# twke18/SPML

Measured on AMD Instinct MI355X. Metric: images/sec (513x513) + k-means iters/sec, higher is better.
Workload: dtype f32

## Files before the change

include/spml_hip.h:

```cpp
#ifndef SPML_HIP_H_
#define SPML_HIP_H_

#include <stddef.h>
#include <stdint.h>

#ifdef __cplusplus
extern "C" {
#endif

typedef enum spml_status {
  SPML_OK = 0,
  SPML_ERR_INVALID_ARG = -1,
  SPML_ERR_UNSUPPORTED = -2,
  SPML_ERR_WORKSPACE = -3,
  SPML_ERR_LAUNCH = -4
} spml_status;

const char* spml_status_string(int status);

#define SPML_ABI_VERSION 8
int spml_abi_version(void);

int spml_set_deterministic(int on);
int spml_get_deterministic(void);

int spml_build_experiment(void);

int spml_normalize_concat_loc_f32(const float* emb, int N, int C, int H, int W,
                                  const float* loc, const int64_t* row_map,
                                  float* out_emb, float* out_loc, void* stream);

int spml_normalize_concat_loc_bwd_f32(const float* emb, int N, int C, int H,
                                      int W, const float* loc,
                                      const int64_t* row_map,
                                      const float* d_out_emb,
                                      const float* d_out_loc, float* d_emb,
                                      void* stream);

int spml_normalize_concat_local_f32(const float* emb, int N, int C, int H, int W,
                                    const float* local, int L,
                                    const int64_t* row_map, float* out_emb,
                                    float* out_loc, void* stream);

int spml_normalize_concat_local_bwd_f32(const float* emb, int N, int C, int H,
                                        int W, const float* local, int L,
                                        const int64_t* row_map,
                                        const float* d_out_emb,
                                        const float* d_out_loc, float* d_emb,
                                        void* stream);

int spml_normalize_concat_local_nhwc_supported(int C, int L);
int spml_normalize_concat_local_nhwc_f32(const float* emb, int N, int C, int H, int W,
                                         const float* local, int L,
                                         const int64_t* row_map, float* out_emb,
                                         float* out_loc, void* stream);
int spml_normalize_concat_local_nhwc_bwd_f32(const float* emb, int N, int C, int H,
                                             int W, const float* local, int L,
                                             const int64_t* row_map,
                                             const float* d_out_emb,
                                             const float* d_out_loc, float* d_emb,
                                             void* stream);

int spml_normalize_rows_f32(const float* x, int64_t rows, int D, float* y,
                            void* stream);
int spml_normalize_rows_bwd_f32(const float* x, const float* dy, int64_t rows,
                                int D, float* dx, void* stream);

size_t spml_relabel_unique_workspace_bytes(int64_t P);
int spml_relabel_unique_i64(const int64_t* keys, int64_t P, int64_t* inv, int64_t* uniq,
                            int64_t uniq_capacity, int64_t* count, void* workspace,
                            size_t workspace_bytes, void* stream);

int spml_kmeans_init_grid_i64(int H, int W, int Ky, int Kx, int64_t* out,
                              void* stream);

#define SPML_KMEANS_DEFAULT 0
#define SPML_KMEANS_FORCE_GENERIC 1
#define SPML_KMEANS_FORCE_V2 4
#define SPML_KMEANS_SEPARATE_PRECONVERT 16
#define SPML_KMEANS_NO_PRECONVERT 8
#define SPML_KMEANS_NO_SCREEN 64
#define SPML_KMEANS_WS_PRECONVERTED 32
#define SPML_KMEANS_PASS_ONLY 256

#define SPML_KMEANS_NO_PASS64 512

#define SPML_KMEANS_TWO_KERNEL_FINALIZE 1024

#define SPML_KMEANS_NO_V4K 2048

size_t spml_kmeans_workspace_bytes(int64_t P, int D, int K, int n_img,
                                   int64_t max_seg_len);

int spml_clock_probe(uint64_t* out, int spin_us, void* stream);

int spml_maxpool3x3s2_nhwc_f32(const float* x, int n, int H, int W, int C, float* y, void* stream);

int spml_kmeans_run_f32(const float* x, int64_t P, int D,
                        const int64_t* seg_offsets, int n_img,
                        int64_t max_seg_len, int K, const int64_t* labels_init,
                        int iterations, int64_t* labels_out,
                        float* centroids_out, int flags, void* ws,
                        size_t ws_bytes, void* stream);

int spml_kmeans_assign_f32(const float* x, int64_t P, int D,
                           const int64_t* seg_offsets, int n_img,
                           int64_t max_seg_len, int K, const float* centroids,
                           int64_t* labels_out, int flags, void* ws,
                           size_t ws_bytes, void* stream);

int spml_kmeans_fused_pass_f32(const float* x, int64_t P, int D,
                               const int64_t* seg_offsets, int n_img,
                               int64_t max_seg_len, int K,
                               const float* centroids_in, int64_t* labels_out,
                               float* centroid_sums_out, int flags, void* ws,
                               size_t ws_bytes, void* stream);

int spml_kmeans_preconvert_f32(const float* x, int64_t P, int D,
                               const int64_t* seg_offsets, int n_img,
                               int64_t max_seg_len, int K, void* ws,
                               size_t ws_bytes, void* stream);

const char* spml_kmeans_path_name(int64_t P, int D, int K, int n_img,
                                  int64_t max_seg_len, int iterations,
                                  int given_centroids, int flags);

int spml_kmeans_profile_layout(int64_t P, int D, int K, int n_img,
                               int64_t max_seg_len, int iterations,
                               int* n_passes, int* workgroups_per_pass);

int spml_kmeans_run_profiled_f32(const float* x, int64_t P, int D,
                                 const int64_t* seg_offsets, int n_img,
                                 int64_t max_seg_len, int K,
                                 const int64_t* labels_init, int iterations,
                                 int64_t* labels_out, int flags, void* ws,
                                 size_t ws_bytes, uint64_t* pass_clocks,
                                 size_t pass_clocks_len, void* stream);

int spml_segment_sum_normalize_f32(const float* x, const int64_t* ids,
                                   int64_t P, int D, int64_t M, float* sums,
                                   float* protos, void* stream);

size_t spml_segment_sum_det_workspace_bytes(int64_t M, int D);
int spml_segment_sum_normalize_det_f32(const float* x, const int64_t* ids,
                                       int64_t P, int D, int64_t M,
                                       float* sums, float* protos, void* ws,
                                       size_t ws_bytes, void* stream);

int spml_segment_sum_normalize_bwd_f32(const float* d_protos,
                                       const float* sums, const int64_t* ids,
                                       int64_t P, int D, int64_t M,
                                       float* d_sums_scratch, float* dx,
                                       int accumulate, void* stream);

#define SPML_NLL_LABEL 0
#define SPML_NLL_TAGSET 1
#define SPML_NLL_PLAIN 2
#define SPML_NLL_CODE32 4

size_t spml_segsort_nll_workspace_bytes(int64_t P, int64_t M, int D);

int spml_segsort_nll_fwd_f32(const float* emb, const int64_t* own,
                             const int64_t* px_code, int64_t P,
                             const float* protos, const int64_t* pr_code,
                             int64_t M, int D, float kappa, int mode,
                             float* nll, float* stats, void* ws,
                             size_t ws_bytes, void* stream);

int spml_segsort_nll_bwd_f32(const float* emb, const int64_t* own,
                             const int64_t* px_code, int64_t P,
                             const float* protos, const int64_t* pr_code,
                             int64_t M, int D, float kappa, int mode,
                             const float* stats, const float* d_nll,
                             float* d_emb, float* d_protos, int64_t m_grad,
                             void* ws, size_t ws_bytes, void* stream);

size_t spml_topk_workspace_bytes(int64_t Q, int64_t M, int D, int k);

int spml_topk_affinity_f32(const float* q, int64_t Q, const float* protos,
                           int64_t M, int D, int k, const int64_t* q_group,
                           const int64_t* pr_group, const uint8_t* pr_valid,
                           float masked_value, int64_t* idx, float* val,
                           void* ws, size_t ws_bytes, void* stream);

int spml_window_accumulate_f32(const float* patch, int C, int h, int w,
                               float* acc, float* counts, int H, int W, int sh,
                               int sw, void* stream);

size_t spml_affinity_workspace_bytes(int B, int C, int64_t n);

int spml_affinity_transition_f32(const float* emb, int B, int C, int64_t n,
                                 float scale, int power, float* trans, void* ws,
                                 size_t ws_bytes, void* stream);

size_t spml_bn_workspace_bytes(int64_t R, int C);

int spml_bn_act_fwd_f32(const float* x, const float* residual, int64_t R, int C,
                        const float* gamma, const float* beta,
                        float* running_mean, float* running_var, float momentum,
                        float eps, int relu, float* y, float* mean, float* invstd,
                        void* ws, size_t ws_bytes, void* stream);

int spml_bn_act_bwd_f32(const float* dy, const float* y, const float* x, int64_t R,
                        int C, const float* mean, const float* invstd,
                        const float* gamma, float* d_gamma, float* d_beta,
                        float* dx, float* d_residual, void* ws, size_t ws_bytes,
                        void* stream);

int spml_bn_stats_f32(const float* x, int64_t R, int C, float* mean, float* m2,
                      void* ws, size_t ws_bytes, void* stream);

int spml_bn_act_apply_f32(const float* x, const float* residual, int64_t R, int C,
                          const float* mean, const float* invstd,
                          const float* gamma, const float* beta, int relu,
                          float* y, void* stream);

int spml_bn_act_bwd_reduce_f32(const float* dy, const float* y, const float* x,
                               int64_t R, int C, const float* mean,
                               const float* invstd, float* sum_dz,
                               float* sum_dz_xhat, void* ws, size_t ws_bytes,
                               void* stream);

int spml_bn_act_bwd_apply_f32(const float* dy, const float* y, const float* x,
                              int64_t R, int C, const float* mean,
                              const float* invstd, const float* gamma,
                              const float* sum_dz, const float* sum_dz_xhat,
                              double count, const float* count_dev, float* dx,
                              float* d_residual, void* stream);


int spml_hl8_from_f32(const float* x, int64_t rows, int C, float* bound,
                      int compute_bound, void* out, void* stream);

int spml_hl8_weight_transposed_f32(const float* w, int Cout, int taps, int Cin,
                                   const float* bound, void* out, void* stream);

int spml_conv_hl8_supported(int K, int N, int taps);

int spml_conv_hl8_f32(const void* a, const float* a_bound, const void* b,
                      const float* b_bound, const float* addend,
                      const unsigned char* addend_mask, float* out,
                      int n_img, int H, int W, int K, int N, int taps, int dilation,
                      void* stream);

int spml_conv_hl8_stats_layout(int n_img, int H, int W, int K, int N, int taps,
                               int* chunks, int* chunk_rows);
int spml_conv_hl8_stats_f32(const void* a, const float* a_bound, const void* b,
                            const float* b_bound, float* out, float* chunk_stats,
                            float* zero_me, int n_img, int H, int W, int K, int N,
                            int taps, int dilation, void* stream);

int spml_conv_wgrad_hl8_supported(int K, int N, int taps);
size_t spml_conv_wgrad_workspace_bytes(int n_img, int H, int W, int K, int N, int taps);
int spml_conv_wgrad_hl8_f32(const void* dy, const float* dy_bound, const void* x,
                            const float* x_bound, float* dw, int n_img, int H, int W,
                            int K, int N, int taps, int dilation, void* ws,
                            size_t ws_bytes, void* stream);

int spml_conv_wgrad_pyramid_hl8_supported(int K, int N, int branches);
int spml_conv_tap_gather_f32(const float* z, const float* bias, float* out, int n_img, int H,
                             int W, int N, int branches, const int* dilations, void* stream);
size_t spml_conv_wgrad_pyramid_workspace_bytes(int n_img, int H, int W, int K, int N,
                                               int branches);
int spml_conv_wgrad_pyramid_hl8_f32(const void* dy, const float* dy_bound, const void* x,
                                    const float* x_bound, float* dw, int n_img, int H, int W,
                                    int K, int N, int branches, const int* dilations,
                                    void* ws, size_t ws_bytes, void* stream);

int spml_bn_stats_ext_f32(const float* x, int64_t R, int C, float* mean, float* m2,
                          float* cmax, float* cmin, void* ws, size_t ws_bytes,
                          void* stream);

int spml_bn_stats_ext_chunks_f32(const float* chunk_stats, int chunks, int chunk_rows,
                                 int64_t R, int C, float* mean, float* m2, float* cmax,
                                 float* cmin, void* stream);

int spml_bn_finalize_f32(const float* mean, const float* m2, int C, double count,
                         float eps, float momentum, float* running_mean,
                         float* running_var, float* invstd, void* stream);

int spml_bn_act_apply_hl8_f32(const float* x, const float* residual,
                              const float* residual_bound, int64_t R, int C,
                              const float* mean, const float* invstd,
                              const float* gamma, const float* beta,
                              const float* cmax, const float* cmin, int relu,
                              float* y, void* y_hl8, float* y_bound,
                              unsigned char* relu_mask, void* stream);

int spml_bn_act_bwd_reduce_ext_f32(const float* dy, const float* y,
                                   const unsigned char* relu_mask,
                                   const float* x, int64_t R, int C, const float* mean,
                                   const float* invstd, float* sum_dz,
                                   float* sum_dz_xhat, float* max_dz, void* ws,
                                   size_t ws_bytes, void* stream);

int spml_bn_act_bwd_apply_hl8_f32(const float* dy, const float* y,
                                  const unsigned char* relu_mask,
                                  const float* x, int64_t R, int C, const float* mean,
                                  const float* invstd, const float* gamma,
                                  const float* sum_dz, const float* sum_dz_xhat,
                                  const float* max_dz, const float* cmax,
                                  const float* cmin, double count,
                                  const float* count_dev, float* dx, void* dx_hl8,
                                  float* dx_bound, float* d_residual, void* stream);

int spml_bn_fwd_hl8_f32(const float* x, const float* residual, const float* residual_bound,
                        int64_t R, int C, const float* gamma, const float* beta,
                        float* running_mean, float* running_var, float momentum, float eps,
                        int relu, float* y, void* y_hl8, float* y_bound,
                        unsigned char* relu_mask, float* mean, float* invstd, float* cmax,
                        float* cmin, void* ws, size_t ws_bytes, void* stream);

int spml_bn_fwd_hl8_chunks_f32(const float* x, const float* chunk_stats, int chunks,
                               int chunk_rows, const float* residual,
                               const float* residual_bound, int64_t R, int C,
                               const float* gamma, const float* beta, float* running_mean,
                               float* running_var, float momentum, float eps, int relu,
                               float* y, void* y_hl8, float* y_bound,
                               unsigned char* relu_mask, float* mean, float* invstd,
                               float* cmax, float* cmin, void* stream);

int spml_bn_bwd_hl8_f32(const float* dy, const float* y, const unsigned char* relu_mask,
                        const float* x, int64_t R, int C, const float* mean,
                        const float* invstd, const float* gamma, const float* cmax,
                        const float* cmin, float* d_gamma, float* d_beta, float* dx,
                        void* dx_hl8, float* dx_bound, float* d_residual, void* ws,
                        size_t ws_bytes, void* stream);

int spml_conv_hl8_pyramid_f32(const void* a, const float* a_bound, const void* b,
// ... 80 lines not shown
```

spml_amd/_ffi.py:

```python
import ctypes
import os
import threading
from ctypes import c_char_p, c_double, c_float, c_int, c_int64, c_size_t, c_void_p

import torch

_HERE = os.path.dirname(os.path.abspath(__file__))
LIB_PATH = os.environ.get('SPML_HIP_LIB') or os.path.join(_HERE, 'lib', 'libspml_hip.so')

_lib = None
_lock = threading.Lock()

_P = c_void_p
_SIGNATURES = {
    'spml_status_string': (c_char_p, [c_int]),
    'spml_abi_version': (c_int, []),
    'spml_normalize_concat_loc_f32': (c_int, [_P, c_int, c_int, c_int, c_int, _P, _P, _P, _P, _P]),
    'spml_normalize_concat_loc_bwd_f32': (c_int, [_P, c_int, c_int, c_int, c_int, _P, _P, _P, _P, _P, _P]),
    'spml_normalize_concat_local_f32': (c_int, [_P, c_int, c_int, c_int, c_int, _P, c_int, _P, _P, _P, _P]),
    'spml_normalize_concat_local_nhwc_supported': (c_int, [c_int, c_int]),
    'spml_normalize_concat_local_nhwc_f32': (c_int, [_P, c_int, c_int, c_int, c_int, _P, c_int, _P, _P, _P, _P]),
    'spml_normalize_concat_local_nhwc_bwd_f32': (c_int, [_P, c_int, c_int, c_int, c_int, _P, c_int, _P, _P, _P,
                                                         _P, _P]),
    'spml_normalize_concat_local_bwd_f32': (c_int, [_P, c_int, c_int, c_int, c_int, _P, c_int, _P, _P, _P,
                                                    _P, _P]),
    'spml_normalize_rows_f32': (c_int, [_P, c_int64, c_int, _P, _P]),
    'spml_normalize_rows_bwd_f32': (c_int, [_P, _P, c_int64, c_int, _P, _P]),
    'spml_kmeans_init_grid_i64': (c_int, [c_int, c_int, c_int, c_int, _P, _P]),
    'spml_relabel_unique_workspace_bytes': (c_size_t, [c_int64]),
    'spml_relabel_unique_i64': (c_int, [_P, c_int64, _P, _P, c_int64, _P, _P, c_size_t, _P]),
    'spml_kmeans_workspace_bytes': (c_size_t, [c_int64, c_int, c_int, c_int, c_int64]),
    'spml_kmeans_run_f32': (c_int, [_P, c_int64, c_int, _P, c_int, c_int64, c_int, _P, c_int, _P, _P,
                                    c_int, _P, c_size_t, _P]),
    'spml_kmeans_assign_f32': (c_int, [_P, c_int64, c_int, _P, c_int, c_int64, c_int, _P, _P, c_int,
                                       _P, c_size_t, _P]),
    'spml_kmeans_fused_pass_f32': (c_int, [_P, c_int64, c_int, _P, c_int, c_int64, c_int, _P, _P, _P,
                                           c_int, _P, c_size_t, _P]),
    'spml_kmeans_preconvert_f32': (c_int, [_P, c_int64, c_int, _P, c_int, c_int64, c_int, _P, c_size_t,
                                           _P]),
    'spml_kmeans_path_name': (c_char_p, [c_int64, c_int, c_int, c_int, c_int64, c_int, c_int, c_int]),
    'spml_kmeans_profile_layout': (c_int, [c_int64, c_int, c_int, c_int, c_int64, c_int, _P, _P]),
    'spml_kmeans_run_profiled_f32': (c_int, [_P, c_int64, c_int, _P, c_int, c_int64, c_int, _P, c_int,
                                             _P, c_int, _P, c_size_t, _P, c_size_t, _P]),
    'spml_segment_sum_normalize_f32': (c_int, [_P, _P, c_int64, c_int, c_int64, _P, _P, _P]),
    'spml_segment_sum_normalize_bwd_f32': (c_int, [_P, _P, _P, c_int64, c_int, c_int64, _P, _P, c_int, _P]),
    'spml_segment_sum_det_workspace_bytes': (c_size_t, [c_int64, c_int]),
    'spml_segment_sum_normalize_det_f32': (c_int, [_P, _P, c_int64, c_int, c_int64, _P, _P, _P, c_size_t, _P]),
    'spml_set_deterministic': (c_int, [c_int]),
    'spml_get_deterministic': (c_int, []),
    'spml_build_experiment': (c_int, []),
    'spml_segsort_nll_workspace_bytes': (c_size_t, [c_int64, c_int64, c_int]),
    'spml_segsort_nll_fwd_f32': (c_int, [_P, _P, _P, c_int64, _P, _P, c_int64, c_int, c_float, c_int,
                                         _P, _P, _P, c_size_t, _P]),
    'spml_segsort_nll_bwd_f32': (c_int, [_P, _P, _P, c_int64, _P, _P, c_int64, c_int, c_float, c_int,
                                         _P, _P, _P, _P, c_int64, _P, c_size_t, _P]),
    'spml_topk_workspace_bytes': (c_size_t, [c_int64, c_int64, c_int, c_int]),
    'spml_topk_affinity_f32': (c_int, [_P, c_int64, _P, c_int64, c_int, c_int, _P, _P, _P, c_float,
                                       _P, _P, _P, c_size_t, _P]),
    'spml_affinity_workspace_bytes': (c_size_t, [c_int, c_int, c_int64]),
    'spml_affinity_transition_f32': (c_int, [_P, c_int, c_int, c_int64, c_float, c_int, _P, _P, c_size_t,
                                             _P]),
    'spml_bn_workspace_bytes': (c_size_t, [c_int64, c_int]),
    'spml_bn_act_fwd_f32': (c_int, [_P, _P, c_int64, c_int, _P, _P, _P, _P, c_float, c_float, c_int, _P, _P, _P,
                                    _P, c_size_t, _P]),
    'spml_bn_act_bwd_f32': (c_int, [_P, _P, _P, c_int64, c_int, _P, _P, _P, _P, _P, _P, _P, _P, c_size_t, _P]),
    'spml_hl8_from_f32': (c_int, [_P, c_int64, c_int, _P, c_int, _P, _P]),
    'spml_hl8_weight_transposed_f32': (c_int, [_P, c_int, c_int, c_int, _P, _P, _P]),
    'spml_conv_hl8_supported': (c_int, [c_int, c_int, c_int]),
    'spml_conv_hl8_f32': (c_int, [_P, _P, _P, _P, _P, _P, _P, c_int, c_int, c_int, c_int, c_int, c_int, c_int, _P]),
    'spml_conv_hl8_stats_layout': (c_int, [c_int, c_int, c_int, c_int, c_int, c_int, _P, _P]),
    'spml_conv_hl8_stats_f32': (c_int, [_P, _P, _P, _P, _P, _P, _P, c_int, c_int, c_int, c_int, c_int, c_int, c_int, _P]),
    'spml_bn_fwd_hl8_chunks_f32': (c_int, [_P, _P, c_int, c_int, _P, _P, c_int64, c_int, _P, _P, _P, _P, c_float, c_float,
                                           c_int, _P, _P, _P, _P, _P, _P, _P, _P, _P]),
    'spml_conv_wgrad_hl8_supported': (c_int, [c_int, c_int, c_int]),
    'spml_conv_wgrad_workspace_bytes': (c_size_t, [c_int, c_int, c_int, c_int, c_int, c_int]),
    'spml_conv_wgrad_hl8_f32': (c_int, [_P, _P, _P, _P, _P, c_int, c_int, c_int, c_int, c_int, c_int, c_int, _P,
                                        c_size_t, _P]),
    'spml_conv_wgrad_pyramid_hl8_supported': (c_int, [c_int, c_int, c_int]),
    'spml_conv_tap_gather_f32': (c_int, [_P, _P, _P, c_int, c_int, c_int, c_int, c_int, _P, _P]),
    'spml_conv_wgrad_pyramid_workspace_bytes': (c_size_t, [c_int, c_int, c_int, c_int, c_int, c_int]),
    'spml_conv_wgrad_pyramid_hl8_f32': (c_int, [_P, _P, _P, _P, _P, c_int, c_int, c_int, c_int, c_int, c_int, _P, _P,
                                                c_size_t, _P]),
    'spml_bn_stats_ext_f32': (c_int, [_P, c_int64, c_int, _P, _P, _P, _P, _P, c_size_t, _P]),
    'spml_bn_stats_ext_chunks_f32': (c_int, [_P, c_int, c_int, c_int64, c_int, _P, _P, _P, _P, _P]),
    'spml_bn_finalize_f32': (c_int, [_P, _P, c_int, c_double, c_float, c_float, _P, _P, _P, _P]),
    'spml_bn_act_apply_hl8_f32': (c_int, [_P, _P, _P, c_int64, c_int, _P, _P, _P, _P, _P, _P, c_int, _P, _P, _P, _P,
                                          _P]),
    'spml_bn_act_bwd_reduce_ext_f32': (c_int, [_P, _P, _P, _P, c_int64, c_int, _P, _P, _P, _P, _P, _P, c_size_t, _P]),
    'spml_bn_act_bwd_apply_hl8_f32': (c_int, [_P, _P, _P, _P, c_int64, c_int, _P, _P, _P, _P, _P, _P, _P, _P,
                                              c_double, _P, _P, _P, _P, _P, _P]),
    'spml_bn_fwd_hl8_f32': (c_int, [_P, _P, _P, c_int64, c_int, _P, _P, _P, _P, c_float, c_float, c_int, _P, _P, _P, _P,
                                    _P, _P, _P, _P, _P, c_size_t, _P]),
    'spml_bn_bwd_hl8_f32': (c_int, [_P, _P, _P, _P, c_int64, c_int, _P, _P, _P, _P, _P, _P, _P, _P, _P, _P, _P, _P,
                                    c_size_t, _P]),
    'spml_conv_hl8_pyramid_f32': (c_int, [_P, _P, _P, _P, _P, _P, _P, c_int, c_int, c_int, c_int, c_int, c_int, _P,
                                          _P]),
    'spml_hl8_weight_transposed_into_f32': (c_int, [_P, c_int, c_int, c_int, _P, _P, c_int, c_int, _P]),
    'spml_absmax_bound_f32': (c_int, [_P, c_int64, _P, c_int, _P]),
    'spml_hl8_weight_set_f32': (c_int, [_P, _P, _P, _P, c_int, _P, _P, _P, _P]),
    'spml_bn_finalize_ranks_f32': (c_int, [_P, c_int, c_int, c_float, c_float, _P, _P, _P, _P, _P, _P]),
    'spml_conv_hl8_affine_f32': (c_int, [_P, _P, _P, _P, _P, _P, c_int, _P, _P, c_int, c_int, c_int, c_int, c_int,
                                         c_int, c_int, _P]),
    'spml_upsample_ce_supported': (c_int, [c_int]),
    'spml_upsample_ce_workspace_bytes': (c_size_t, [c_int, c_int, c_int]),
    'spml_upsample_ce_fwd_f32': (c_int, [_P, _P, c_int, c_int, c_int, c_int, c_int, c_int, c_int64, _P, _P, _P,
                                         c_size_t, _P]),
    'spml_upsample_ce_bwd_f32': (c_int, [_P, _P, _P, c_int, c_int, c_int, c_int, c_int, c_int, c_int64, _P, _P, _P]),
    'spml_upsample_ce_bwd_path_name': (c_char_p, [c_int, c_int, c_int, c_int, c_int, c_int]),
    'spml_bn_stats_f32': (c_int, [_P, c_int64, c_int, _P, _P, _P, c_size_t, _P]),
    'spml_bn_act_apply_f32': (c_int, [_P, _P, c_int64, c_int, _P, _P, _P, _P, c_int, _P, _P]),
    'spml_bn_act_bwd_reduce_f32': (c_int, [_P, _P, _P, c_int64, c_int, _P, _P, _P, _P, _P, c_size_t, _P]),
    'spml_bn_act_bwd_apply_f32': (c_int, [_P, _P, _P, c_int64, c_int, _P, _P, _P, _P, _P, c_double, _P, _P, _P,
                                          _P]),
    'spml_clock_probe': (c_int, [_P, c_int, _P]),
    'spml_maxpool3x3s2_nhwc_f32': (c_int, [_P, c_int, c_int, c_int, c_int, _P, _P]),
    'spml_window_accumulate_f32': (c_int, [_P, c_int, c_int, c_int, _P, _P, c_int, c_int, c_int, c_int,
                                           _P]),
    'spml_unit_hl8_from_nchw_f32': (c_int, [_P, c_int, c_int, c_int, c_int, _P, _P]),
    'spml_class_head_supported': (c_int, [c_int, c_int]),
    'spml_class_head_accumulate_f32': (c_int, [_P, c_int, c_int, c_int, _P, _P, c_int, _P, c_int, c_int, c_int, c_int,
                                               _P]),
    'spml_argmax_channels_i64': (c_int, [_P, c_int, c_int, c_int, c_int, c_int, _P, _P]),
    'spml_iou_counts_i64': (c_int, [_P, _P, c_int64, c_int, _P, _P]),
    'spml_resample_unit_f32': (c_int, [_P, c_int, c_int, c_int, c_int64, c_int64, c_int64, c_int, c_int, c_int, c_int,
                                       c_int, _P, c_int, c_int, _P]),
    'spml_resample_classes_accumulate_f32': (c_int, [_P, c_int, c_int, c_int, c_int64, c_int64, c_int64, c_int, c_int,
                                                     c_int, c_int, c_int, c_int, _P, _P]),
    'spml_cam_finalize_f32': (c_int, [_P, c_int, c_int64, c_int, c_int, _P, c_int, c_float, _P, _P]),
    'spml_upsample_argmax_i64': (c_int, [_P, c_int, c_int, c_int, c_int, c_int, _P, _P]),
    'spml_view_probs_accumulate_f32': (c_int, [_P, c_int, c_int, c_int, _P, _P, c_int, c_int, c_int, c_int, c_int, _P,
                                               _P]),
    'spml_view_votes_workspace_bytes': (c_size_t, [c_int, c_int]),
    'spml_view_votes_accumulate_f32': (c_int, [_P, c_int, c_int, _P, c_int, c_int, c_int, c_int, c_int, c_int, _P, _P,
                                               c_size_t, _P]),
}

EXPORTS = tuple(_SIGNATURES)


class SpmlHipError(RuntimeError):
  pass


ABI_VERSION = 8


def lib():
  global _lib
  if _lib is None:
    with _lock:
      if _lib is None:
        if not os.path.exists(LIB_PATH):
          raise SpmlHipError(
              'libspml_hip.so not found at %s -- build it with `python -m spml_amd._build` '
              '(there is no CPU fallback for the HIP path)' % LIB_PATH)
        handle = ctypes.CDLL(LIB_PATH)
        for name, (res, args) in _SIGNATURES.items():
          try:
            fn = getattr(handle, name)
          except AttributeError:
            raise SpmlHipError('libspml_hip.so does not export %s (stale build? run '
                               '`python -m spml_amd._build --force`)' % name)
          fn.restype = res
          fn.argtypes = args
        got = handle.spml_abi_version()
        if got != ABI_VERSION:
          raise SpmlHipError('libspml_hip.so has ABI version %d, this wrapper was written against %d (stale build? '
                             'run `python -m spml_amd._build --force`)' % (got, ABI_VERSION))
        exp = handle.spml_build_experiment()
        want = (int(os.environ.get('SPML_CONV_EXP') or 0) & 0xffff) | ((int(os.environ.get('SPML_P64_EXP') or 0) & 0xffff) << 16)
        if exp != want:
          raise SpmlHipError('libspml_hip.so is a profiling build (SPML_CONV_EXP=%d, SPML_P64_EXP=%d: kernels that skip work '
                             'and overwrite outputs) but this process asks for (%d, %d) -- rebuild with '
                             '`python -m spml_amd._build`' % (exp & 0xffff, exp >> 16, want & 0xffff, want >> 16))
        if os.environ.get('SPML_DETERMINISTIC', '0') not in ('', '0'):
          handle.spml_set_deterministic(1)
        _lib = handle
  return _lib


def set_deterministic(on):
  return bool(lib().spml_set_deterministic(1 if on else 0))


def deterministic():
  return bool(lib().spml_get_deterministic())


def check(rc, what):
  if rc != 0:
    raise SpmlHipError('%s failed: %s (status %d)' % (
        what, lib().spml_status_string(rc).decode(), rc))


def stream_ptr():
  return c_void_p(torch.cuda.current_stream().cuda_stream)


def ptr(t, dtype=None, allow_none=False):
  if t is None:
    if allow_none:
      return c_void_p(0)
    raise SpmlHipError('missing tensor argument')
  if not t.is_cuda:
    raise SpmlHipError('the HIP path needs GPU tensors (got %s); there is no CPU fallback'
                       % t.device)
  if t.device.index != torch.cuda.current_device():
    raise SpmlHipError('tensor lives on %s but the current device is cuda:%d -- wrap the call in '
# ... 135 lines not shown
  nbytes = lib().spml_kmeans_workspace_bytes(p, d, k, n_img, max_seg_len)
  ws = workspace(nbytes, x.device)
  check(lib().spml_kmeans_run_f32(
      ptr(x, torch.float32), p, d, ptr(seg_offsets, torch.int64), n_img, int(max_seg_len), k,
      ptr(labels_init, torch.int64), int(iterations), ptr(labels), ptr(cent, None, True),
      int(flags), ptr(ws), ws.numel(), stream_ptr()), 'spml_kmeans_run_f32')
  _note_kmeans(p, d, k, n_img, max_seg_len, iterations, 0, flags)
  return (labels, cent) if want_centroids else labels


def kmeans_run_profiled(x, seg_offsets, max_seg_len, k, labels_init, iterations, flags=0):
  import ctypes
  p, d = x.shape
  n_img = seg_offsets.shape[0] - 1
  n_pass, wgs = ctypes.c_int(0), ctypes.c_int(0)
  check(lib().spml_kmeans_profile_layout(p, d, k, n_img, int(max_seg_len), int(iterations),
                                         ctypes.byref(n_pass), ctypes.byref(wgs)),
        'spml_kmeans_profile_layout')
  clocks = torch.zeros((n_pass.value, wgs.value, 2), dtype=torch.int64, device=x.device)
  labels = torch.empty((p,), dtype=torch.int64, device=x.device)
  ws = workspace(lib().spml_kmeans_workspace_bytes(p, d, k, n_img, max_seg_len), x.device)
  check(lib().spml_kmeans_run_profiled_f32(
      ptr(x, torch.float32), p, d, ptr(seg_offsets, torch.int64), n_img, int(max_seg_len), k,
      ptr(labels_init, torch.int64), int(iterations), ptr(labels), int(flags), ptr(ws), ws.numel(),
      ptr(clocks), clocks.numel(), stream_ptr()), 'spml_kmeans_run_profiled_f32')
  _note_kmeans(p, d, k, n_img, max_seg_len, iterations, 0, flags)
  c = clocks.cpu()
  start = torch.where(c[:, :, 0] == 0, torch.full_like(c[:, :, 0], torch.iinfo(torch.int64).max), c[:, :, 0])
  dur = (c[:, :, 1].max(dim=1).values - start.min(dim=1).values).double() * 0.01
  return labels, dur


def kmeans_assign(x, seg_offsets, max_seg_len, centroids, flags=0):
  p, d = x.shape
  n_img = seg_offsets.shape[0] - 1
  k = centroids.shape[-2]
  labels = torch.empty((p,), dtype=torch.int64, device=x.device)
  nbytes = lib().spml_kmeans_workspace_bytes(p, d, k, n_img, max_seg_len)
  ws = workspace(nbytes, x.device)
  check(lib().spml_kmeans_assign_f32(
      ptr(x, torch.float32), p, d, ptr(seg_offsets, torch.int64), n_img, int(max_seg_len), k,
      ptr(centroids, torch.float32), ptr(labels), int(flags), ptr(ws), ws.numel(),
      stream_ptr()), 'spml_kmeans_assign_f32')
  _note_kmeans(p, d, k, n_img, max_seg_len, 1, 1, flags)
  return labels


def kmeans_workspace(x, seg_offsets, max_seg_len, k):
  p, d = x.shape
  return workspace(lib().spml_kmeans_workspace_bytes(p, d, k, seg_offsets.shape[0] - 1, max_seg_len),
                   x.device)


def kmeans_preconvert(x, seg_offsets, max_seg_len, k, ws):
  p, d = x.shape
  check(lib().spml_kmeans_preconvert_f32(
      ptr(x, torch.float32), p, d, ptr(seg_offsets, torch.int64), seg_offsets.shape[0] - 1,
      int(max_seg_len), int(k), ptr(ws), ws.numel(), stream_ptr()), 'spml_kmeans_preconvert_f32')


def kmeans_fused_pass(x, seg_offsets, max_seg_len, centroids, ws=None, preconverted=False, flags=0,
                      out=None):
  p, d = x.shape
  n_img = seg_offsets.shape[0] - 1
  k = centroids.shape[-2]
  if ws is None:
    ws = kmeans_workspace(x, seg_offsets, max_seg_len, k)
  if out is None:
    out = (torch.empty((p,), dtype=torch.int64, device=x.device),
           torch.empty((n_img, k, d), dtype=torch.float32, device=x.device))
  labels, sums = out
  flags = int(flags) | (32 if preconverted else 0)
  check(lib().spml_kmeans_fused_pass_f32(
      ptr(x, torch.float32), p, d, ptr(seg_offsets, torch.int64), n_img, int(max_seg_len), k,
      ptr(centroids, torch.float32), ptr(labels, torch.int64), ptr(sums, torch.float32), flags,
      ptr(ws), ws.numel(), stream_ptr()), 'spml_kmeans_fused_pass_f32')
  _note_kmeans(p, d, k, n_img, max_seg_len, 1, 1, flags)
  return labels, sums


def clock_probe(device, spin_us, stream):
  out = torch.zeros((2,), dtype=torch.int64, device=device)
  stream.wait_stream(torch.cuda.current_stream(device))
  check(lib().spml_clock_probe(ptr(out), int(spin_us), c_void_p(stream.cuda_stream)), 'spml_clock_probe')
  return out


def maxpool3x3s2_nhwc(x):
  n, c, h, w = x.shape
  oh, ow = (h - 1) // 2 + 1, (w - 1) // 2 + 1
  y = torch.empty((n, c, oh, ow), dtype=torch.float32, device=x.device, memory_format=torch.channels_last)
  check(lib().spml_maxpool3x3s2_nhwc_f32(_ptr_any(x), n, h, w, c, _ptr_any(y), stream_ptr()), 'spml_maxpool3x3s2_nhwc_f32')
  return y


def segment_sum_normalize(x, ids, m):
  p, d = x.shape
  sums = torch.empty((m, d), dtype=torch.float32, device=x.device)
  protos = torch.empty((m, d), dtype=torch.float32, device=x.device)
  if deterministic():
    nbytes = lib().spml_segment_sum_det_workspace_bytes(int(m), d)
    ws = workspace(nbytes, x.device)
    check(lib().spml_segment_sum_normalize_det_f32(ptr(x, torch.float32), ptr(ids, torch.int64), p, d, int(m),
                                                   ptr(sums), ptr(protos), ptr(ws), ws.numel(), stream_ptr()),
          'spml_segment_sum_normalize_det_f32')
    return protos, sums
  check(lib().spml_segment_sum_normalize_f32(ptr(x, torch.float32), ptr(ids, torch.int64), p, d,
                                             int(m), ptr(sums), ptr(protos), stream_ptr()),
        'spml_segment_sum_normalize_f32')
  return protos, sums


def segment_sum_normalize_bwd(d_protos, sums, ids, p, accumulate=0, dx=None):
  m, d = sums.shape
  scratch = torch.empty_like(sums)
  if accumulate:
    if dx is None or tuple(dx.shape) != (p, d):
      raise SpmlHipError('accumulate needs a dx of shape (%d, %d) to add into' % (p, d))
  else:
    dx = torch.empty((p, d), dtype=torch.float32, device=sums.device)
  check(lib().spml_segment_sum_normalize_bwd_f32(
      ptr(d_protos, torch.float32), ptr(sums, torch.float32), ptr(ids, torch.int64), p, d, m,
      ptr(scratch), ptr(dx, torch.float32), 1 if accumulate else 0, stream_ptr()), 'spml_segment_sum_normalize_bwd_f32')
  return dx


def segsort_nll_fwd(emb, own, px_code, protos, pr_code, kappa, mode):
  p, d = emb.shape
  m = protos.shape[0]
  nll = torch.empty((p,), dtype=torch.float32, device=emb.device)
  stats = torch.empty((p, 4), dtype=torch.float32, device=emb.device)
  ws = workspace(lib().spml_segsort_nll_workspace_bytes(p, m, d), emb.device)
  check(lib().spml_segsort_nll_fwd_f32(
      ptr(emb, torch.float32), ptr(own, torch.int64), ptr(px_code, torch.int64), p,
      ptr(protos, torch.float32), ptr(pr_code, torch.int64), m, d, float(kappa), int(mode),
      ptr(nll), ptr(stats), ptr(ws), ws.numel(), stream_ptr()), 'spml_segsort_nll_fwd_f32')
  return nll, stats


def segsort_nll_bwd(emb, own, px_code, protos, pr_code, kappa, mode, stats, d_nll, m_grad=-1):
  p, d = emb.shape
  m = protos.shape[0]
  d_emb = torch.empty_like(emb)
  d_protos = torch.zeros_like(protos)
  ws = workspace(lib().spml_segsort_nll_workspace_bytes(p, m, d), emb.device)
  check(lib().spml_segsort_nll_bwd_f32(
      ptr(emb, torch.float32), ptr(own, torch.int64), ptr(px_code, torch.int64), p,
      ptr(protos, torch.float32), ptr(pr_code, torch.int64), m, d, float(kappa), int(mode),
      ptr(stats, torch.float32), ptr(d_nll, torch.float32), ptr(d_emb), ptr(d_protos),
      int(m_grad), ptr(ws), ws.numel(), stream_ptr()), 'spml_segsort_nll_bwd_f32')
  return d_emb, d_protos


def topk_affinity(q, protos, k, q_group=None, pr_group=None, pr_valid=None, masked_value=-2.0):
  nq, d = q.shape
  m = protos.shape[0]
  idx = torch.empty((nq, k), dtype=torch.int64, device=q.device)
  val = torch.empty((nq, k), dtype=torch.float32, device=q.device)
  ws = workspace(lib().spml_topk_workspace_bytes(nq, m, d, k), q.device)
  check(lib().spml_topk_affinity_f32(
      ptr(q, torch.float32), nq, ptr(protos, torch.float32), m, d, int(k),
      ptr(q_group, torch.int64, True), ptr(pr_group, torch.int64, True),
      ptr(pr_valid, torch.uint8, True), float(masked_value), ptr(idx), ptr(val), ptr(ws),
      ws.numel(), stream_ptr()), 'spml_topk_affinity_f32')
  return idx, val


def window_accumulate(patch, acc, counts, sh, sw):
  c, h, w = patch.shape
  big_c, big_h, big_w = acc.shape
  if big_c != c or tuple(counts.shape) != (big_h, big_w):
    raise SpmlHipError('window_accumulate: shape mismatch')
  check(lib().spml_window_accumulate_f32(
      ptr(patch, torch.float32), c, h, w, ptr(acc, torch.float32), ptr(counts, torch.float32),
      big_h, big_w, int(sh), int(sw), stream_ptr()), 'spml_window_accumulate_f32')


def unit_hl8_from_nchw(x):
  n, c, h, w = x.shape
  out = torch.empty((n * h * w * c * 4,), dtype=torch.uint8, device=x.device)
  check(lib().spml_unit_hl8_from_nchw_f32(ptr(x, torch.float32), n, c, h, w, ptr(out), stream_ptr()),
        'spml_unit_hl8_from_nchw_f32')
  return Hl8(out, torch.ones((1,), dtype=torch.float32, device=x.device), n * h * w, c)


def class_head_supported(ch, ncls):
  return bool(lib().spml_class_head_supported(int(ch), int(ncls)))


def class_head_accumulate(hidden, weight, bias, canvas, sh, sw, h, w):
  ncls, ch = weight.shape
  if hidden.numel() != h * w * ch or canvas.dim() != 3 or canvas.shape[0] != ncls or bias.numel() != ncls:
    raise SpmlHipError('class_head_accumulate: shape mismatch')
  check(lib().spml_class_head_accumulate_f32(
      _ptr_any(hidden), ch, int(h), int(w), ptr(weight, torch.float32), ptr(bias, torch.float32), ncls,
      ptr(canvas, torch.float32), canvas.shape[1], canvas.shape[2], int(sh), int(sw), stream_ptr()),
        'spml_class_head_accumulate_f32')


def argmax_channels(canvas, h, w):
  ncls, hp, wp = canvas.shape
  out = torch.empty((h, w), dtype=torch.int64, device=canvas.device)
  check(lib().spml_argmax_channels_i64(ptr(canvas, torch.float32), ncls, hp, wp, int(h), int(w), ptr(out),
                                       stream_ptr()), 'spml_argmax_channels_i64')
  return out


def iou_counts(pred, target, ncls, counts=None):
  if pred.numel() != target.numel():
    raise SpmlHipError('iou_counts: pred and target differ in size')
  if counts is None:
    counts = torch.zeros((3, ncls), dtype=torch.int64, device=pred.device)
  elif tuple(counts.shape) != (3, ncls):
    raise SpmlHipError('iou_counts: counts must be [3, num_classes]')
  check(lib().spml_iou_counts_i64(ptr(pred, torch.int64), ptr(target, torch.int64), pred.numel(), int(ncls),
                                  ptr(counts, torch.int64), stream_ptr()), 'spml_iou_counts_i64')
  return counts


COMBINE_MODES = {'prob_mean': 0, 'logit_mean': 1}


def _combine(combine):
  if combine not in COMBINE_MODES:
    raise SpmlHipError("combine must be 'prob_mean' or 'logit_mean' (got %r)" % (combine,))
  return COMBINE_MODES[combine]


def _view_args(x, crop_hw, out_hw, what):
  if x.dim() != 3:
    raise SpmlHipError('%s: expected a [C, Hp, Wp] tensor' % what)
  c, hp, wp = x.shape
  (rh, rw), (oh, ow) = crop_hw, out_hw
  if not (0 < rh <= hp and 0 < rw <= wp and oh > 0 and ow > 0):
    raise SpmlHipError('%s: crop %r / output %r do not fit a %d x %d plane' % (what, crop_hw, out_hw, hp, wp))
  sc, sy, sx = x.stride()
  return c, hp, wp, sc, sy, sx, int(rh), int(rw), int(oh), int(ow)


def resample_unit(emb, crop_hw, flip, out_hw, out, b):
  c, hp, wp, sc, sy, sx, rh, rw, oh, ow = _view_args(emb, crop_hw, out_hw, 'resample_unit')
  if out.dim() != 3 or out.shape[1] != c or out.shape[2] != oh * ow or not 0 <= b < out.shape[0]:
    raise SpmlHipError('resample_unit: out must be [B, %d, %d] with b < B' % (c, oh * ow))
  check(lib().spml_resample_unit_f32(_ptr_any(emb), c, hp, wp, sc, sy, sx, rh, rw, int(bool(flip)), oh, ow,
                                     ptr(out, torch.float32), out.shape[0], int(b), stream_ptr()),
        'spml_resample_unit_f32')
  return out


def resample_classes_accumulate(logit, crop_hw, flip, out_hw, acc, combine='prob_mean'):
  ncls, hp, wp, sc, sy, sx, rh, rw, oh, ow = _view_args(logit, crop_hw, out_hw, 'resample_classes_accumulate')
  if acc.shape[0] != ncls or acc.numel() != ncls * oh * ow:
    raise SpmlHipError('resample_classes_accumulate: acc must hold [%d, %d] values' % (ncls, oh * ow))
  check(lib().spml_resample_classes_accumulate_f32(_ptr_any(logit), ncls, hp, wp, sc, sy, sx, rh, rw, int(bool(flip)),
                                                   oh, ow, _combine(combine), ptr(acc, torch.float32), stream_ptr()),
        'spml_resample_classes_accumulate_f32')
  return acc


def cam_finalize(acc, num_views, label_tags, combine='prob_mean', background_threshold=None):
  ncls = acc.shape[0]
  if label_tags.numel() != ncls or label_tags.dtype not in (torch.bool, torch.uint8):
    raise SpmlHipError('cam_finalize: label_tags must be a bool [%d] tensor' % ncls)
  if int(num_views) < 1:
    raise SpmlHipError('cam_finalize: no views')
  cam = torch.empty_like(acc)
  tags = label_tags.view(torch.uint8) if label_tags.dtype == torch.bool else label_tags
  check(lib().spml_cam_finalize_f32(ptr(acc, torch.float32), ncls, acc.numel() // ncls, int(num_views),
                                    _combine(combine), ptr(tags, torch.uint8), int(background_threshold is not None),
                                    float(background_threshold or 0.0), ptr(cam), stream_ptr()),
        'spml_cam_finalize_f32')
  return cam


def upsample_argmax(cam, h, w):
  if cam.dim() != 3:
    raise SpmlHipError('upsample_argmax: expected [ncls, oh, ow]')
  ncls, oh, ow = cam.shape
  out = torch.empty((int(h), int(w)), dtype=torch.int64, device=cam.device)
  check(lib().spml_upsample_argmax_i64(ptr(cam, torch.float32), ncls, oh, ow, int(h), int(w), ptr(out), stream_ptr()),
        'spml_upsample_argmax_i64')
  return out


def view_probs_accumulate(canvas, cnt_y, cnt_x, crop_hw, flip, acc):
  if canvas.dim() != 3 or acc.dim() != 3 or acc.shape[0] != canvas.shape[0]:
    raise SpmlHipError('view_probs_accumulate: canvas must be [ncls, Hp, Wp] and acc [ncls, h, w]')
  ncls, hp, wp = canvas.shape
  rh, rw = int(crop_hw[0]), int(crop_hw[1])
  if not (0 < rh <= hp and 0 < rw <= wp):
    raise SpmlHipError('view_probs_accumulate: crop %r does not fit a %d x %d plane' % (tuple(crop_hw), hp, wp))
  if tuple(cnt_y.shape) != (hp,) or tuple(cnt_x.shape) != (wp,):
    raise SpmlHipError('view_probs_accumulate: cnt_y must be [%d] and cnt_x [%d]' % (hp, wp))
  check(lib().spml_view_probs_accumulate_f32(
      ptr(canvas, torch.float32), ncls, hp, wp, ptr(cnt_y, torch.float32), ptr(cnt_x, torch.float32), rh, rw,
      int(bool(flip)), acc.shape[1], acc.shape[2], ptr(acc, torch.float32), stream_ptr()),
        'spml_view_probs_accumulate_f32')
  return acc


MAX_VIEW_VOTES_CLASSES = 64
MAX_VIEW_VOTES_SEGMENTS = 4096


def view_votes_accumulate(clu, crop_hw, topk, ncls, flip, acc):
  rh, rw = int(crop_hw[0]), int(crop_hw[1])
# ... 514 lines not shown
```

spml_amd/csrc/nll.hip:

```cpp
#include <algorithm>
#include <type_traits>

#include "nll_common.hpp"

namespace spml {
namespace {

template <bool RAW>
__global__ __launch_bounds__(256) void prep_std(const float* __restrict__ x, int64_t R, int D,
                                                int KS, float scale, _Float16* __restrict__ oh,
                                                _Float16* __restrict__ ol) {
  const int64_t f = (int64_t)blockIdx.x * 4 + (threadIdx.x >> 6);
  const int64_t nfrag = ((R + 31) / 32) * KS;
  if (f >= nfrag) return;
  const int lane = threadIdx.x & 63;
  const int64_t tile = f / KS;
  const int ks = (int)(f - tile * KS);
  const int64_t row = 32 * tile + (lane & 31);
  const int k0 = 16 * ks + 8 * (lane >> 5);
  half8 h, l;
#pragma unroll
  for (int e = 0; e < 8; ++e) {
    float v = 0.f;
    if (row < R && k0 + e < D) v = x[(size_t)row * D + k0 + e] * scale;
    _Float16 a, b;
    if constexpr (RAW) {
      a = (_Float16)v;
      b = (_Float16)(v - (float)a);
    } else {
      split_f16(v, a, b);
    }
    h[e] = a; l[e] = b;
  }
  *reinterpret_cast<half8*>(oh + ((size_t)f * 64 + lane) * 8) = h;
  *reinterpret_cast<half8*>(ol + ((size_t)f * 64 + lane) * 8) = l;
}

template <bool RAW>
__global__ __launch_bounds__(256) void prep_T(const float* __restrict__ x, int64_t R, int D,
                                              int DT, const float* __restrict__ rowscale,
                                              const float* __restrict__ gscale, float scale,
                                              _Float16* __restrict__ oh,
                                              _Float16* __restrict__ ol) {
  const int64_t f = (int64_t)blockIdx.x * 4 + (threadIdx.x >> 6);
  const int64_t nfrag = ((R + 31) / 32) * DT * 2;
  if (f >= nfrag) return;
  const int lane = threadIdx.x & 63;
  const int s = (int)(f & 1);
  const int64_t td = f >> 1;
  const int64_t tile = td / DT;
  const int dt = (int)(td - tile * DT);
  const int d = 32 * dt + (lane & 31);
  const float gs = gscale ? 1.0f / gscale[0] : 1.0f;
  half8 h, l;
#pragma unroll
  for (int e = 0; e < 8; ++e) {
    const int64_t rho = 32 * tile + tile_row(8 * s + e, lane >> 5);
    float v = 0.f;
    if (rho < R && d < D) {
      v = x[(size_t)rho * D + d] * scale;
      if (rowscale) v *= rowscale[rho] * gs;
    }
    _Float16 a, b;
    if constexpr (RAW) {
      v = fminf(fmaxf(v, -65000.f), 65000.f);
      a = (_Float16)v;
      b = (_Float16)(v - (float)a);
    } else {
      split_f16(v, a, b);
    }
    h[e] = a; l[e] = b;
  }
  *reinterpret_cast<half8*>(oh + ((size_t)f * 64 + lane) * 8) = h;
  *reinterpret_cast<half8*>(ol + ((size_t)f * 64 + lane) * 8) = l;
}

__global__ __launch_bounds__(1024) void max_abs_pow2(const float* __restrict__ g, int64_t n,
                                                     float* __restrict__ out) {
  __shared__ float red[16];
  float m = 0.f;
  for (int64_t i = threadIdx.x; i < n; i += 1024) m = fmaxf(m, fabsf(g[i]));
#pragma unroll
  for (int o = 32; o > 0; o >>= 1) m = fmaxf(m, __shfl_xor(m, o, 64));
  if ((threadIdx.x & 63) == 0) red[threadIdx.x >> 6] = m;
  __syncthreads();
  if (threadIdx.x == 0) {
    for (int i = 1; i < 16; ++i) m = fmaxf(m, red[i]);
    float p = 1.0f;
    if (m > 0.f && m < INFINITY) {
      int ex;
      frexpf(m, &ex);
      p = ldexpf(1.0f, ex);
    }
    out[0] = p;
  }
}

template <int KS>
__device__ __forceinline__ void zgemm_lds(const unsigned char* a_lds, int lane,
                                          const half8 (&bh)[KS], const half8 (&bl)[KS],
                                          float16v& zh, float16v& zx) {
#pragma unroll
  for (int r = 0; r < 16; ++r) { zh[r] = 0.f; zx[r] = 0.f; }
#pragma unroll
  for (int ks = 0; ks < KS; ++ks) {
    const half8 a_h = *reinterpret_cast<const half8*>(a_lds + ((size_t)ks * 64 + lane) * 16);
    const half8 a_l = *reinterpret_cast<const half8*>(a_lds + ((size_t)(KS + ks) * 64 + lane) * 16);
    zh = mfma32(a_h, bh[ks], zh);
    zx = mfma32(a_h, bl[ks], zx);
    zx = mfma32(a_l, bh[ks], zx);
  }
}

template <int KS>
__device__ __forceinline__ void zgemm(const _Float16* __restrict__ ah_g,
                                      const _Float16* __restrict__ al_g, int lane,
                                      const half8 (&bh)[KS], const half8 (&bl)[KS],
                                      float16v& zh, float16v& zx) {
#pragma unroll
  for (int r = 0; r < 16; ++r) { zh[r] = 0.f; zx[r] = 0.f; }
#pragma unroll
  for (int ks = 0; ks < KS; ++ks) {
    const half8 a_h = *reinterpret_cast<const half8*>(ah_g + ((size_t)ks * 64 + lane) * 8);
    const half8 a_l = *reinterpret_cast<const half8*>(al_g + ((size_t)ks * 64 + lane) * 8);
    zh = mfma32(a_h, bh[ks], zh);
    zx = mfma32(a_h, bl[ks], zx);
    zx = mfma32(a_l, bh[ks], zx);
  }
}

template <int KS, int NB, bool TAG, bool C32>
__global__ __launch_bounds__(256) void nll_fwd(NllArgs a) {
  using CodeT = code_t<C32>;
  constexpr int NBLK = 2 * KS + 1;
  constexpr int SLOT = NBLK * 1024;
  const int DEPTH = a.depth_fwd;
  extern __shared__ __attribute__((aligned(16))) unsigned char sm[];
  const int lane = threadIdx.x & 63;
  const int wv = __builtin_amdgcn_readfirstlane(threadIdx.x >> 6);
  const int half = lane >> 5, j = lane & 31;
  const int64_t wave = (int64_t)blockIdx.x * 4 + wv;
  const int64_t pt0 = wave * NB;

  half8 bh[NB][KS], bl[NB][KS];
  CodeT pcode[NB];
  int own[NB];
  float s_same[NB], s_diff[NB], s_own[NB];
#pragma unroll
  for (int nb = 0; nb < NB; ++nb) {
    const int64_t pt = min(pt0 + nb, a.n.PT - 1);
#pragma unroll
    for (int ks = 0; ks < KS; ++ks) {
      bh[nb][ks] = *reinterpret_cast<const half8*>(a.eh + (((size_t)pt * KS + ks) * 64 + lane) * 8);
      bl[nb][ks] = *reinterpret_cast<const half8*>(a.el + (((size_t)pt * KS + ks) * 64 + lane) * 8);
    }
    const int64_t p = min(32 * pt + j, a.n.P - 1);
    pcode[nb] = (CodeT)a.px_code[p];
    own[nb] = (int)a.own[p];
    s_same[nb] = 0.f; s_diff[nb] = 0.f; s_own[nb] = 0.f;
  }

  auto stage = [&](int64_t mt, int slot) {
    unsigned char* dst = sm + slot * SLOT;
    for (int b = wv; b < 2 * KS + 1; b += 4) {
      const void* src;
      if (b < KS) src = a.ph + ((size_t)(mt * KS + b) * 64 + lane) * 8;
      else if (b < 2 * KS) src = a.pl + ((size_t)(mt * KS + (b - KS)) * 64 + lane) * 8;
      else src = a.pr_code_pad + 32 * mt + 2 * min(lane, 15);
      dma_block(src, dst + (size_t)b * 1024);
    }
  };

  const int my_blocks = (NBLK - wv + 3) / 4;
  for (int64_t t0 = 0; t0 < DEPTH - 1 && t0 < a.n.MT; ++t0) stage(t0, (int)t0);
  int slot = -1;
  for (int64_t mt = 0; mt < a.n.MT; ++mt) {
    slot = slot + 1 == DEPTH ? 0 : slot + 1;
    if (DEPTH > 2) wait_vmcnt(my_blocks * (int)min((int64_t)(DEPTH - 2), a.n.MT - 1 - mt));
    else asm volatile("s_waitcnt vmcnt(0)" ::: "memory");
    wg_barrier();
    if (mt + DEPTH - 1 < a.n.MT) stage(mt + DEPTH - 1, slot == 0 ? DEPTH - 1 : slot - 1);
    const unsigned char* at = sm + slot * SLOT;
    const int64_t* codes = reinterpret_cast<const int64_t*>(at + 2 * KS * 1024);
    CodeT rc[16];
#pragma unroll
    for (int r = 0; r < 16; ++r) rc[r] = (CodeT)codes[tile_row(r, half)];
    const bool ragged = 32 * (mt + 1) > a.n.M;
#pragma unroll
    for (int nb = 0; nb < NB; ++nb) {
      float16v zh, zx;
      zgemm_lds<KS>(at, lane, bh[nb], bl[nb], zh, zx);
      float sv[16];
#pragma unroll
      for (int r = 0; r < 16; ++r) sv[r] = __builtin_amdgcn_exp2f(zh[r] + zx[r] * kSplitInv);
      if (ragged) {
        const int lim = (int)(a.n.M - 32 * mt) - 4 * half;
#pragma unroll
        for (int r = 0; r < 16; ++r) sv[r] = (tile_row(r, 0) < lim) ? sv[r] : 0.f;
      }
#pragma unroll
      for (int r = 0; r < 16; ++r) {
        const float t = code_match<TAG, CodeT>(pcode[nb], rc[r]) ? sv[r] : 0.f;
        s_same[nb] += t;
        s_diff[nb] += sv[r] - t;
      }
      if (__any((own[nb] >> 5) == (int)mt)) {
        const int own_rel = own[nb] - (int)(32 * mt) - 4 * half;
#pragma unroll
        for (int r = 0; r < 16; ++r) s_own[nb] += (tile_row(r, 0) == own_rel) ? sv[r] : 0.f;
      }
    }
  }
#pragma unroll
  for (int nb = 0; nb < NB; ++nb) {
    const float same = s_same[nb] + __shfl_xor(s_same[nb], 32, 64);
    const float diff = s_diff[nb] + __shfl_xor(s_diff[nb], 32, 64);
    const float osim = s_own[nb] + __shfl_xor(s_own[nb], 32, 64);
    const int64_t p = 32 * (pt0 + nb) + j;
    if (half == 0 && pt0 + nb < a.n.PT && p < a.n.P) {
      const float pos = same - osim;
      const bool fb = (a.mode & SPML_NLL_PLAIN) || !(pos > 0.f);
      const float num = fb ? osim : pos;
      const float den = diff + num;
      a.nll[p] = -logf(num / den);
      float4v st = {num, den, osim, fb ? 1.f : 0.f};
      *reinterpret_cast<float4v*>(a.stats + (size_t)p * 4) = st;
    }
  }
}


template <int KS, int MTB, bool TAG>
__global__ __launch_bounds__(256, 2) void nll_fwd2(NllArgs a) {
  constexpr int TILE = 2 * KS * 1024;
  constexpr int SLOT = MTB * TILE;
  constexpr int CODES = kFwd2TilesPerChunk * 32 * 4;
  static_assert((MTB & (MTB - 1)) == 0 && MTB >= 2, "MTB: even power of two");
  static_assert(kFwd2TilesPerChunk <= 128, "two 64-bit masks of uniform-tile flags");
  extern __shared__ __attribute__((aligned(16))) unsigned char sm[];
  int* const codes_lds = reinterpret_cast<int*>(sm);
  unsigned char* const ring = sm + CODES;
  const int lane = threadIdx.x & 63;
  const int wv = __builtin_amdgcn_readfirstlane(threadIdx.x >> 6);
  const int half = lane >> 5, j = lane & 31;
  const int64_t pt0 = ((int64_t)blockIdx.x * 4 + wv) * 2;
  const int64_t mt_lo = (int64_t)blockIdx.y * kFwd2TilesPerChunk;
  const int ntile = (int)(min(a.n.MT, mt_lo + kFwd2TilesPerChunk) - mt_lo);
  const int nstage = (ntile + MTB - 1) / MTB;

  auto stage = [&](int st, int slot) {
    unsigned char* dst = ring + slot * SLOT;
    for (int b = wv; b < MTB * 2 * KS; b += 4) {
      const int t = b / (2 * KS), q = b - t * (2 * KS);
      const int64_t mt = mt_lo + min(st * MTB + t, ntile - 1);
      const void* src = q < KS ? a.ph + ((size_t)(mt * KS + q) * 64 + lane) * 8
                               : a.pl + ((size_t)(mt * KS + (q - KS)) * 64 + lane) * 8;
      dma_block(src, dst + (size_t)b * 1024);
    }
  };
  stage(0, 0);
  if (nstage > 1) stage(1, 1);
  for (int i = threadIdx.x; i < 32 * ntile; i += 256) codes_lds[i] = (int)a.pr_code_pad[32 * mt_lo + i];

  half8 bh[2][KS], bl[2][KS];
  int pcode[2], own[2];
  float s_same[2], s_all[2], s_own[2];
#pragma unroll
  for (int nb = 0; nb < 2; ++nb) {
    const int64_t pt = min(pt0 + nb, a.n.PT - 1);
#pragma unroll
    for (int ks = 0; ks < KS; ++ks) {
      bh[nb][ks] = *reinterpret_cast<const half8*>(a.eh + (((size_t)pt * KS + ks) * 64 + lane) * 8);
      bl[nb][ks] = *reinterpret_cast<const half8*>(a.el + (((size_t)pt * KS + ks) * 64 + lane) * 8);
    }
    const int64_t p = min(32 * pt + j, a.n.P - 1);
    pcode[nb] = (int)a.px_code[p];
    own[nb] = (int)a.own[p] - (int)(32 * mt_lo);
    s_same[nb] = 0.f; s_all[nb] = 0.f; s_own[nb] = 0.f;
  }

  auto advance = [&](int st) {
    asm volatile("s_waitcnt vmcnt(0)" ::: "memory");
    wg_barrier();
    if (st + 1 < nstage) stage(st + 1, (st + 1) & 1);
  };
  auto tile_at = [&](int g) -> const unsigned char* {
    return ring + ((g / MTB) & 1) * SLOT + (g & (MTB - 1)) * TILE + (size_t)lane * 16;
  };
  half8 pa, pl;
  auto prefetch = [&](int g) {
    const unsigned char* at = tile_at(g);
    pa = *reinterpret_cast<const half8*>(at);
    pl = *reinterpret_cast<const half8*>(at + KS * 1024);
  };
  auto step = [&](int gn, float16v& zn0, float16v& zn1, int gp, const float16v& zp0, const float16v& zp1,
                  int g_next, auto gemm_tag, auto epi_tag, auto last_tag, auto uni_tag) {
    constexpr bool GEMM = decltype(gemm_tag)::value, EPI = decltype(epi_tag)::value;
    constexpr bool LAST = decltype(last_tag)::value;
    constexpr bool UNI = decltype(uni_tag)::value && !LAST;
    constexpr int NSLOT = 6 * KS;
    int rc[16];
    int lim = 0;
    float same[2] = {s_same[0], s_same[1]}, all[2] = {s_all[0], s_all[1]};
    float tsum[2] = {0.f, 0.f};
    if constexpr (EPI && !UNI) {
#pragma unroll
      for (int r = 0; r < 16; ++r) rc[r] = codes_lds[32 * gp + tile_row(r, half)];
      lim = (int)(a.n.M - 32 * (mt_lo + gp)) - 4 * half;
    }
    const unsigned char* at = GEMM ? tile_at(gn) : ring;
    half8 ah, al, ah_n, al_n;
    if constexpr (GEMM) { ah = pa; al = pl; }
    const float16v zero = {0.f, 0.f, 0.f, 0.f, 0.f, 0.f, 0.f, 0.f, 0.f, 0.f, 0.f, 0.f, 0.f, 0.f, 0.f, 0.f};
    auto epi_values = [&](int slot) {
      if constexpr (EPI) {
#pragma unroll
        for (int v = slot * 32 / NSLOT; v < (slot + 1) * 32 / NSLOT; ++v) {
          const int nb = v >> 4, r = v & 15;
          float sv = __builtin_amdgcn_exp2f(nb ? zp1[r] : zp0[r]);
          if constexpr (UNI) {
            tsum[nb] += sv;
          } else {
            if constexpr (LAST) sv = (tile_row(r, 0) < lim) ? sv : 0.f;
            all[nb] += sv;
            same[nb] += code_match<TAG, int>(pcode[nb], rc[r]) ? sv : 0.f;
          }
        }
      }
    };
#pragma unroll
    for (int ks = 0; ks < KS; ++ks) {
      if constexpr (GEMM) {
        if (ks + 1 < KS) {
          ah_n = *reinterpret_cast<const half8*>(at + (ks + 1) * 1024);
          al_n = *reinterpret_cast<const half8*>(at + (KS + ks + 1) * 1024);
        }
        zn0 = mfma32(ah, bh[0][ks], ks == 0 ? zero : zn0);
      }
      epi_values(6 * ks + 0);
      if constexpr (GEMM) zn1 = mfma32(ah, bh[1][ks], ks == 0 ? zero : zn1);
      epi_values(6 * ks + 1);
      if constexpr (GEMM) zn0 = mfma32(ah, bl[0][ks], zn0);
      epi_values(6 * ks + 2);
      if constexpr (GEMM) zn1 = mfma32(ah, bl[1][ks], zn1);
      epi_values(6 * ks + 3);
      if constexpr (GEMM) zn0 = mfma32(al, bh[0][ks], zn0);
      epi_values(6 * ks + 4);
      if constexpr (GEMM) zn1 = mfma32(al, bh[1][ks], zn1);
      epi_values(6 * ks + 5);
      if constexpr (GEMM) { ah = ah_n; al = al_n; }
    }
    if constexpr (EPI && UNI) {
      const int code = codes_lds[32 * gp];
#pragma unroll
      for (int nb = 0; nb < 2; ++nb) {
        all[nb] += tsum[nb];
        same[nb] += code_match<TAG, int>(pcode[nb], code) ? tsum[nb] : 0.f;
      }
    }
    if constexpr (GEMM && EPI) {
      constexpr int kValu = ((UNI ? 2 : TAG ? 6 : 5) * 32 + 8) / NSLOT + 1;
#pragma unroll
      for (int i = 0; i < NSLOT; ++i) {
        __builtin_amdgcn_sched_group_barrier(0x008, 1, 0);
        __builtin_amdgcn_sched_group_barrier(0x002, kValu, 0);
      }
    }
    if constexpr (EPI) {
      asm volatile("" : "+v"(same[0]), "+v"(same[1]), "+v"(all[0]), "+v"(all[1]));
      s_same[0] = same[0]; s_same[1] = same[1]; s_all[0] = all[0]; s_all[1] = all[1];
    }
    if (g_next >= 0) prefetch(g_next);
  };
  auto own_check = [&](int g, const float16v& z0, const float16v& z1) {
#pragma unroll
    for (int nb = 0; nb < 2; ++nb) {
      if (__any((own[nb] >> 5) == g)) {
        const float16v& z = nb ? z1 : z0;
        const int own_rel = own[nb] - 32 * g - 4 * half;
#pragma unroll
        for (int r = 0; r < 16; ++r) {
          float zz = z[r];
          asm volatile("" : "+v"(zz));
          s_own[nb] += (tile_row(r, 0) == own_rel) ? __builtin_amdgcn_exp2f(zz) : 0.f;
        }
      }
    }
  };
  using Y = std::true_type;
  using N = std::false_type;

  const int my_blocks = (MTB * 2 * KS - wv + 3) / 4;
  if (nstage > 1) wait_vmcnt(my_blocks); else asm volatile("s_waitcnt vmcnt(0)" ::: "memory");
  __syncthreads();
  unsigned long long uni_lo, uni_hi;
  {
    bool u0 = lane < ntile && 32 * (mt_lo + lane + 1) <= a.n.M;
    bool u1 = lane + 64 < ntile && 32 * (mt_lo + lane + 65) <= a.n.M;
    for (int i = 1; i < 32; ++i) {
      u0 &= codes_lds[32 * min(lane, ntile - 1) + i] == codes_lds[32 * min(lane, ntile - 1)];
      u1 &= codes_lds[32 * min(lane + 64, ntile - 1) + i] == codes_lds[32 * min(lane + 64, ntile - 1)];
    }
    uni_lo = __ballot(u0);
    uni_hi = __ballot(u1);
  }
  auto is_uniform = [&](int g) -> bool { return ((g < 64 ? uni_lo >> g : uni_hi >> (g - 64)) & 1ull) != 0; };

  float16v zA0, zA1, zB0, zB1;
  prefetch(0);
  step(0, zA0, zA1, 0, zA0, zA1, 1, Y{}, N{}, N{}, N{});
  int g = 0;
  for (; g + 2 < ntile; g += 2) {
    own_check(g, zA0, zA1);
    const bool turn = ((g + 2) & (MTB - 1)) == 0;
    if (is_uniform(g)) step(g + 1, zB0, zB1, g, zA0, zA1, turn ? -1 : g + 2, Y{}, Y{}, N{}, Y{});
    else step(g + 1, zB0, zB1, g, zA0, zA1, turn ? -1 : g + 2, Y{}, Y{}, N{}, N{});
    own_check(g + 1, zB0, zB1);
    if (turn) { advance((g + 2) / MTB); prefetch(g + 2); }
    if (is_uniform(g + 1)) step(g + 2, zA0, zA1, g + 1, zB0, zB1, g + 3, Y{}, Y{}, N{}, Y{});
    else step(g + 2, zA0, zA1, g + 1, zB0, zB1, g + 3, Y{}, Y{}, N{}, N{});
  }
  own_check(g, zA0, zA1);
  if (g + 1 < ntile) {
    step(g + 1, zB0, zB1, g, zA0, zA1, -1, Y{}, Y{}, N{}, N{});
    own_check(g + 1, zB0, zB1);
    step(0, zA0, zA1, g + 1, zB0, zB1, -1, N{}, Y{}, Y{}, N{});
  } else {
    step(0, zB0, zB1, g, zA0, zA1, -1, N{}, Y{}, Y{}, N{});
  }

#pragma unroll
  for (int nb = 0; nb < 2; ++nb) {
    const float same = s_same[nb] + __shfl_xor(s_same[nb], 32, 64);
    const float all = s_all[nb] + __shfl_xor(s_all[nb], 32, 64);
    const float osim = s_own[nb] + __shfl_xor(s_own[nb], 32, 64);
    const int64_t p = 32 * (pt0 + nb) + j;
    if (half == 0 && pt0 + nb < a.n.PT) {
      const float4v st = {same, all, osim, 0.f};
      *reinterpret_cast<float4v*>(a.partial + ((size_t)blockIdx.y * a.n.PT * 32 + p) * 4) = st;
    }
  }
}

__global__ __launch_bounds__(256) void nll_finalize(const float* __restrict__ partial, int chunks,
                                                    int64_t P, int64_t P_pad, int plain,
                                                    float* __restrict__ nll, float* __restrict__ stats) {
  const int64_t p = (int64_t)blockIdx.x * 256 + threadIdx.x;
  if (p >= P) return;
  float same = 0.f, all = 0.f, osim = 0.f;
  for (int c = 0; c < chunks; ++c) {
    const float4v v = *reinterpret_cast<const float4v*>(partial + ((size_t)c * P_pad + p) * 4);
    same += v[0]; all += v[1]; osim += v[2];
  }
  const float pos = same - osim;
  const bool fb = plain || !(pos > 0.f);
  const float num = fb ? osim : pos;
  const float den = fb ? (all - same) + osim : all - osim;
  nll[p] = -logf(num / den);
  const float4v st = {num, den, osim, fb ? 1.f : 0.f};
  *reinterpret_cast<float4v*>(stats + (size_t)p * 4) = st;
}

template <bool TAG>
__global__ void coef_kernel(const float* __restrict__ stats, const int64_t* __restrict__ own,
                            const int64_t* __restrict__ px_code, const int64_t* __restrict__ pr_code, int64_t M,
                            int64_t P, int64_t P_pad, PixelCoef* __restrict__ out) {
  const int64_t i = (int64_t)blockIdx.x * 256 + threadIdx.x;
  if (i >= P_pad) return;
  PixelCoef c{0.f, 0.f, -1, 0.f};
  if (i < P) {
    const float4v st = *reinterpret_cast<const float4v*>(stats + (size_t)i * 4);
    const float inv_num = 1.0f / st[0], inv_den = 1.0f / st[1];
    c.wa = st[3] != 0.f ? 0.f : inv_den - inv_num;
    c.wb = inv_den;
    c.own = (int)own[i];
    const int64_t m = own[i];
    const bool own_same = m >= 0 && m < M && code_match<TAG, int64_t>(px_code[i], pr_code[m]);
    c.tscale = nll_t_scale(st[0], st[1], st[2], st[3] != 0.f, own_same);
  }
  out[i] = c;
}

__global__ void rowscale_ts_kernel(const float* g, float kappa, const PixelCoef* __restrict__ coef, int64_t n, float* out) {
  const int64_t i = (int64_t)blockIdx.x * 256 + threadIdx.x;
  if (i < n) out[i] = g[i] * kappa * (kTScale / coef[i].tscale);
}

template <bool TAG>
__global__ void own_term_kernel(const float* __restrict__ stats, const int64_t* __restrict__ own,
                                const int64_t* __restrict__ px_code, const int64_t* __restrict__ pr_code,
                                const float* __restrict__ emb, const float* __restrict__ protos, int64_t P,
                                int64_t P_pad, int64_t M, int D, float kappa_log2e, float* __restrict__ out) {
  const int64_t i = (int64_t)blockIdx.x * 256 + threadIdx.x;
  if (i >= P_pad) return;
  float v = 0.f;
  if (i < P) {
    const int64_t m = own[i];
    if (m >= 0 && m < M) {
      const float4v st = *reinterpret_cast<const float4v*>(stats + (size_t)i * 4);
      const float inv_num = 1.0f / st[0], inv_den = 1.0f / st[1];
      const bool fb = st[3] != 0.f;
      const bool same = code_match<TAG, int64_t>(px_code[i], pr_code[m]);
      const float c1 = inv_den - inv_num;
      const float w = same ? (fb ? c1 : 0.f) : (fb ? c1 + inv_den : inv_num);
      if (w != 0.f) {
        double dot = 0.0;
        for (int d = 0; d < D; ++d) dot += (double)emb[(size_t)i * D + d] * (double)protos[(size_t)m * D + d];
        v = w * __builtin_amdgcn_exp2f((float)(dot * (double)kappa_log2e));
      }
    }
  }
  out[i] = v;
}

__device__ __forceinline__ float own_weight(bool same, float wa, float wb) {
  return same ? 0.f : wb - wa;
}

__device__ __forceinline__ void split_regs(const float (&t)[16], int s2, half8& th, half8& tl) {
  float v[8];
#pragma unroll
  for (int e = 0; e < 8; ++e) v[e] = t[8 * s2 + e];
  split8(v, th, tl);
}

constexpr int kLoResident = 3;
template <int DT>
struct LoAcc {
  float16v v[DT <= kLoResident ? DT : 1];
};
template <int DT>
__device__ __forceinline__ void zero_lo(LoAcc<DT>& lo) {
#pragma unroll
  for (int dt = 0; dt < (DT <= kLoResident ? DT : 1); ++dt)
#pragma unroll
    for (int r = 0; r < 16; ++r) lo.v[dt][r] = 0.f;
}
template <int DT>
__device__ __forceinline__ void fold_lo(const LoAcc<DT>& lo, float16v (&dacc)[DT]) {
  if constexpr (DT <= kLoResident) {
#pragma unroll
    for (int dt = 0; dt < DT; ++dt)
#pragma unroll
      for (int r = 0; r < 16; ++r) dacc[dt][r] += lo.v[dt][r] * kSplitInv;
  }
}

template <int DT>
__device__ __forceinline__ void second_gemm(const unsigned char* at_lds, int lane,
                                            const float (&t)[16], float16v (&dacc)[DT],
                                            LoAcc<DT>& dlo) {
#pragma unroll
  for (int s2 = 0; s2 < 2; ++s2) {
    half8 th, tl;
    split_regs(t, s2, th, tl);
#pragma unroll
    for (int dt = 0; dt < DT; ++dt) {
      const unsigned char* blk = at_lds + (size_t)((dt * 2 + s2) * 2) * 1024;
      const half8 a_h = *reinterpret_cast<const half8*>(blk + (size_t)lane * 16);
      const half8 a_l = *reinterpret_cast<const half8*>(blk + 1024 + (size_t)lane * 16);
      if constexpr (DT <= kLoResident) {
        dlo.v[dt] = mfma32(a_h, tl, dlo.v[dt]);
        dlo.v[dt] = mfma32(a_l, th, dlo.v[dt]);
      } else {
        float16v lo;
#pragma unroll
        for (int r = 0; r < 16; ++r) lo[r] = 0.f;
        lo = mfma32(a_h, tl, lo);
        lo = mfma32(a_l, th, lo);
#pragma unroll
        for (int r = 0; r < 16; ++r) dacc[dt][r] += lo[r] * kSplitInv;
      }
      dacc[dt] = mfma32(a_h, th, dacc[dt]);
    }
  }
}

__device__ __forceinline__ void tcache_store(float* base, int64_t tile, int lane, const float (&t)[16]) {
  float4v* p = reinterpret_cast<float4v*>(base + ((size_t)tile * 64 + lane) * 16);
#pragma unroll
  for (int q = 0; q < 4; ++q) {
    const float4v v = {t[4 * q], t[4 * q + 1], t[4 * q + 2], t[4 * q + 3]};
    p[q] = v;
  }
}
__device__ __forceinline__ void tcache_load(const float* base, int64_t tile, int lane, float (&t)[16]) {
  const float4v* p = reinterpret_cast<const float4v*>(base + ((size_t)tile * 64 + lane) * 16);
#pragma unroll
  for (int q = 0; q < 4; ++q) {
    const float4v v = p[q];
    t[4 * q] = v[0]; t[4 * q + 1] = v[1]; t[4 * q + 2] = v[2]; t[4 * q + 3] = v[3];
  }
}

template <int KS, int DT, bool TAG, bool C32, int TM = 0>
__global__ __launch_bounds__(256) void nll_bwd_de(NllArgs a) {
  using CodeT = code_t<C32>;
  constexpr int kStd = TM == 2 ? 0 : 2 * KS + 1;
  constexpr int NBLK = kStd + 4 * DT;
  constexpr int SLOT = NBLK * 1024;
  const int DEPTH = a.depth;
  extern __shared__ __attribute__((aligned(16))) unsigned char sm[];
  const int lane = threadIdx.x & 63;
  const int wv = __builtin_amdgcn_readfirstlane(threadIdx.x >> 6);
  const int half = lane >> 5, j = lane & 31;
  const int64_t pt = min(a.spt0 + (int64_t)blockIdx.x * 4 + wv, a.spt1 - 1);
  const bool active = a.spt0 + (int64_t)blockIdx.x * 4 + wv < a.spt1;

  half8 bh[TM == 2 ? 1 : KS], bl[TM == 2 ? 1 : KS];
  if constexpr (TM != 2) {
#pragma unroll
    for (int ks = 0; ks < KS; ++ks) {
      bh[ks] = *reinterpret_cast<const half8*>(a.eh + (((size_t)pt * KS + ks) * 64 + lane) * 8);
      bl[ks] = *reinterpret_cast<const half8*>(a.el + (((size_t)pt * KS + ks) * 64 + lane) * 8);
    }
  }
  const int64_t p = min(32 * pt + j, a.n.P - 1);
  const CodeT pcode = (CodeT)a.px_code[p];
  const PixelCoef cf = a.coef[32 * pt + j];
  const float inv_num = 1.0f / a.stats[(size_t)p * 4];

  float16v dacc[DT];
  LoAcc<DT> dlo;
  zero_lo<DT>(dlo);
#pragma unroll
  for (int dt = 0; dt < DT; ++dt)
#pragma unroll
    for (int r = 0; r < 16; ++r) dacc[dt][r] = 0.f;

  auto stage = [&](int64_t mt, int slot) {
    unsigned char* dst = sm + slot * SLOT;
    for (int b = wv; b < NBLK; b += 4) {
      const void* src;
      if (b < kStd && b < KS) src = a.ph + ((size_t)(mt * KS + b) * 64 + lane) * 8;
      else if (b < kStd && b < 2 * KS) src = a.pl + ((size_t)(mt * KS + (b - KS)) * 64 + lane) * 8;
      else if (b < kStd) src = a.pr_code_pad + 32 * mt + 2 * min(lane, 15);
      else {
        const int q = b - kStd;
        const size_t f = ((size_t)mt * a.dt_all + a.dt0) * 2 + (q >> 1);
        src = ((q & 1) ? a.ptl : a.pth) + (f * 64 + lane) * 8;
      }
      dma_block(src, dst + (size_t)b * 1024);
    }
  };
  const int my_blocks = (NBLK - wv + 3) / 4;
  for (int64_t t0 = 0; t0 < DEPTH - 1 && t0 < a.n.MT; ++t0) stage(t0, (int)t0);
  int slot = -1;
  for (int64_t mt = 0; mt < a.n.MT; ++mt) {
    slot = slot + 1 == DEPTH ? 0 : slot + 1;
    if (mt + 1 < a.n.MT && DEPTH > 2) wait_vmcnt(my_blocks * (int)min((int64_t)(DEPTH - 2), a.n.MT - 1 - mt));
    else asm volatile("s_waitcnt vmcnt(0)" ::: "memory");
    wg_barrier();
    if (mt + DEPTH - 1 < a.n.MT) stage(mt + DEPTH - 1, slot == 0 ? DEPTH - 1 : slot - 1);
    const unsigned char* at = sm + slot * SLOT;
    const int64_t* codes = reinterpret_cast<const int64_t*>(at + 2 * KS * 1024);
    float t[16];
    if constexpr (TM == 2) {
      tcache_load(a.tcache_de, (pt - a.spt0) * a.n.MT + mt, lane, t);
    } else {
      float16v zh, zx;
      zgemm_lds<KS>(at, lane, bh, bl, zh, zx);
      const bool ragged = 32 * (mt + 1) > a.n.M;
  #pragma unroll
      for (int r = 0; r < 16; ++r) {
        const float s = __builtin_amdgcn_exp2f(zh[r] + zx[r] * kSplitInv);
        const bool same = code_match<TAG, CodeT>(pcode, (CodeT)codes[tile_row(r, half)]);
        t[r] = s * (same ? cf.wa : cf.wb);
      }
      if (__any((cf.own >> 5) == (int)mt)) {
        const int own_rel = cf.own - (int)(32 * mt) - 4 * half;
  #pragma unroll
        for (int r = 0; r < 16; ++r) {
          if (tile_row(r, 0) == own_rel) {
            const float s = __builtin_amdgcn_exp2f(zh[r] + zx[r] * kSplitInv);
            const bool same = code_match<TAG, CodeT>(pcode, (CodeT)codes[tile_row(r, half)]);
            const bool fb = cf.wa == 0.f && a.stats[(size_t)p * 4 + 3] != 0.f;
            const float c1 = cf.wb - inv_num;
            const float w = fb ? (c1 + (same ? 0.f : cf.wb)) : (same ? 0.f : inv_num);
            t[r] = s * w;
          }
        }
      }
      if (ragged) {
        const int lim = (int)(a.n.M - 32 * mt) - 4 * half;
  #pragma unroll
        for (int r = 0; r < 16; ++r) t[r] = (tile_row(r, 0) < lim) ? t[r] : 0.f;
      }
      if (TM == 1) tcache_store(a.tcache_de, (pt - a.spt0) * a.n.MT + mt, lane, t);
    }
    second_gemm<DT>(at + kStd * 1024, lane, t, dacc, dlo);
  }
  fold_lo<DT>(dlo, dacc);
  const int64_t pp = 32 * pt + j;
  if (active && pp < a.n.P) {
    const float gk = a.d_nll[pp] * a.kappa;
#pragma unroll
    for (int dt = 0; dt < DT; ++dt)
#pragma unroll
      for (int r = 0; r < 16; ++r) {
        const int d = 32 * (a.dt0 + dt) + tile_row(r, half);
        if (d < a.n.D) a.d_emb[(size_t)pp * a.n.D + d] = gk * dacc[dt][r];
      }
  }
}

template <int KS, int DT, int MTB, bool TAG>
__global__ __launch_bounds__(256, 2) void nll_bwd_de2(NllArgs a) {
  constexpr int TSTD = 2 * KS * 1024;
  constexpr int TILE = TSTD + 4 * DT * 1024;
  constexpr int SLOT = MTB * TILE;
  constexpr int CODES = kFwd2TilesPerChunk * 32 * 4;
  static_assert((MTB & (MTB - 1)) == 0 && MTB >= 2, "MTB: even power of two");
  extern __shared__ __attribute__((aligned(16))) unsigned char sm[];
  int* const codes_lds = reinterpret_cast<int*>(sm);
  unsigned char* const ring = sm + CODES;
  const int lane = threadIdx.x & 63;
  const int wv = __builtin_amdgcn_readfirstlane(threadIdx.x >> 6);
  const int half = lane >> 5, j = lane & 31;
  const int64_t pt0 = ((int64_t)blockIdx.x * 4 + wv) * 2;
  const int nchunk = (int)((a.n.MT + kFwd2TilesPerChunk - 1) / kFwd2TilesPerChunk);

  half8 bh[2][KS], bl[2][KS];
  int pcode[2], own[2];
  float wa[2], wb[2];
#pragma unroll
  for (int nb = 0; nb < 2; ++nb) {
    const int64_t pt = min(pt0 + nb, a.n.PT - 1);
#pragma unroll
    for (int ks = 0; ks < KS; ++ks) {
      bh[nb][ks] = *reinterpret_cast<const half8*>(a.eh + (((size_t)pt * KS + ks) * 64 + lane) * 8);
      bl[nb][ks] = *reinterpret_cast<const half8*>(a.el + (((size_t)pt * KS + ks) * 64 + lane) * 8);
    }
    const int64_t p = min(32 * pt + j, a.n.P - 1);
    pcode[nb] = (int)a.px_code[p];
    const PixelCoef cf = a.coef[32 * pt + j];
    wa[nb] = cf.wa * cf.tscale; wb[nb] = cf.wb * cf.tscale; own[nb] = cf.own;
  }
  float16v dacc[2][DT];
#pragma unroll
  for (int nb = 0; nb < 2; ++nb)
#pragma unroll
    for (int dt = 0; dt < DT; ++dt)
#pragma unroll
      for (int r = 0; r < 16; ++r) dacc[nb][dt][r] = 0.f;

  for (int c = blockIdx.y; c < nchunk; c += gridDim.y) {
    const int64_t mt_lo = (int64_t)c * kFwd2TilesPerChunk;
    const int ntile = (int)(min(a.n.MT, mt_lo + kFwd2TilesPerChunk) - mt_lo);
    const int nstage = (ntile + MTB - 1) / MTB;
    __syncthreads();
    auto stage = [&](int st, int slot) {
      unsigned char* dst = ring + slot * SLOT;
      for (int b = wv; b < MTB * (2 * KS + 4 * DT); b += 4) {
        const int t = b / (2 * KS + 4 * DT), q = b - t * (2 * KS + 4 * DT);
        const int64_t mt = mt_lo + min(st * MTB + t, ntile - 1);
        const void* src;
        if (q < KS) src = a.ph + ((size_t)(mt * KS + q) * 64 + lane) * 8;
        else if (q < 2 * KS) src = a.pl + ((size_t)(mt * KS + (q - KS)) * 64 + lane) * 8;
        else {
          const int u = q - 2 * KS;
          src = ((u & 1) ? a.ptl : a.pth) + (((size_t)mt * DT * 2 + (u >> 1)) * 64 + lane) * 8;
        }
        dma_block(src, dst + (size_t)b * 1024);
      }
    };
    stage(0, 0);
    if (nstage > 1) stage(1, 1);
    for (int i = threadIdx.x; i < 32 * ntile; i += 256) codes_lds[i] = (int)a.pr_code_pad[32 * mt_lo + i];
    const int my_blocks = (MTB * (2 * KS + 4 * DT) - wv + 3) / 4;
    if (nstage > 1) wait_vmcnt(my_blocks); else asm volatile("s_waitcnt vmcnt(0)" ::: "memory");
    __syncthreads();
    unsigned long long uni_lo, uni_hi;
    {
      bool u0 = lane < ntile && 32 * (mt_lo + lane + 1) <= a.n.M;
      bool u1 = lane + 64 < ntile && 32 * (mt_lo + lane + 65) <= a.n.M;
      for (int i = 1; i < 32; ++i) {
        u0 &= codes_lds[32 * min(lane, ntile - 1) + i] == codes_lds[32 * min(lane, ntile - 1)];
        u1 &= codes_lds[32 * min(lane + 64, ntile - 1) + i] == codes_lds[32 * min(lane + 64, ntile - 1)];
      }
      uni_lo = __ballot(u0);
      uni_hi = __ballot(u1);
    }
    const int own_c0 = own[0] - (int)(32 * mt_lo), own_c1 = own[1] - (int)(32 * mt_lo);

    auto tile = [&](int g, auto uni_tag) {
      constexpr bool UNI = decltype(uni_tag)::value;
      const unsigned char* at = ring + ((g / MTB) & 1) * SLOT + (g & (MTB - 1)) * TILE + (size_t)lane * 16;
      const float16v zero = {0.f, 0.f, 0.f, 0.f, 0.f, 0.f, 0.f, 0.f, 0.f, 0.f, 0.f, 0.f, 0.f, 0.f, 0.f, 0.f};
      const int code0 = codes_lds[32 * g];
      const bool ragged = mt_lo + g + 1 == a.n.MT && 32 * a.n.MT > a.n.M;
      const int lim = (int)(a.n.M - 32 * (mt_lo + g)) - 4 * half;
#pragma unroll
      for (int nb = 0; nb < 2; ++nb) {
        float16v z;
#pragma unroll
        for (int ks = 0; ks < KS; ++ks) {
          const half8 ah = *reinterpret_cast<const half8*>(at + ks * 1024);
          const half8 al = *reinterpret_cast<const half8*>(at + (KS + ks) * 1024);
          z = mfma32(ah, bh[nb][ks], ks == 0 ? zero : z);
          z = mfma32(ah, bl[nb][ks], z);
          z = mfma32(al, bh[nb][ks], z);
        }
        float t[16];
        const float wu = code_match<TAG, int>(pcode[nb], code0) ? wa[nb] : wb[nb];
#pragma unroll
        for (int r = 0; r < 16; ++r) {
          const float sv = __builtin_amdgcn_exp2f(z[r]);
          if constexpr (UNI) t[r] = sv * wu;
          else t[r] = sv * (code_match<TAG, int>(pcode[nb], codes_lds[32 * g + tile_row(r, half)]) ? wa[nb] : wb[nb]);
        }
        const int own_c = nb ? own_c1 : own_c0;
        if (__any((own_c >> 5) == g)) {
          const int own_rel = own_c - 32 * g - 4 * half;
#pragma unroll
          for (int r = 0; r < 16; ++r)
            if (tile_row(r, 0) == own_rel) t[r] = 0.f;
        }
        if (ragged) {
#pragma unroll
          for (int r = 0; r < 16; ++r) t[r] = (tile_row(r, 0) < lim) ? t[r] : 0.f;
        }
#pragma unroll
        for (int s2 = 0; s2 < 2; ++s2) {
          half8 th, tl;
#pragma unroll
          for (int e = 0; e < 8; e += 2) {
            const float t0 = t[8 * s2 + e], t1 = t[8 * s2 + e + 1];
            const half2v hh = __builtin_bit_cast(half2v, __builtin_amdgcn_cvt_pkrtz(t0, t1));
            float r0, r1;
            asm("v_fma_mix_f32 %0, %1, -1.0, %2 op_sel_hi:[1,0,0]" : "=v"(r0) : "v"(hh), "v"(t0));
            asm("v_fma_mix_f32 %0, %1, -1.0, %2 op_sel:[1,0,0] op_sel_hi:[1,0,0]" : "=v"(r1) : "v"(hh), "v"(t1));
            const half2v ll = __builtin_bit_cast(half2v, __builtin_amdgcn_cvt_pkrtz(r0, r1));
            th[e] = hh[0]; th[e + 1] = hh[1];
            tl[e] = ll[0]; tl[e + 1] = ll[1];
          }
#pragma unroll
          for (int dt = 0; dt < DT; ++dt) {
            const unsigned char* blk = at + TSTD + (size_t)((dt * 2 + s2) * 2) * 1024;
            const half8 qh = *reinterpret_cast<const half8*>(blk);
            const half8 ql = *reinterpret_cast<const half8*>(blk + 1024);
            dacc[nb][dt] = mfma32(qh, th, dacc[nb][dt]);
            dacc[nb][dt] = mfma32(qh, tl, dacc[nb][dt]);
            dacc[nb][dt] = mfma32(ql, th, dacc[nb][dt]);
          }
        }
        __builtin_amdgcn_sched_barrier(0);
      }
    };

    for (int g = 0; g < ntile; ++g) {
      if (g > 0 && (g & (MTB - 1)) == 0) {
        const int st = g / MTB;
        asm volatile("s_waitcnt vmcnt(0)" ::: "memory");
        wg_barrier();
        if (st + 1 < nstage) stage(st + 1, (st + 1) & 1);
      }
      if (((g < 64 ? uni_lo >> g : uni_hi >> (g - 64)) & 1ull) != 0) tile(g, std::true_type{});
      else tile(g, std::false_type{});
    }
  }

#pragma unroll
  for (int nb = 0; nb < 2; ++nb) {
    if (pt0 + nb < a.n.PT) {
#pragma unroll
      for (int dt = 0; dt < DT; ++dt)
#pragma unroll
        for (int r = 0; r < 16; ++r)
          a.partial_de[((((size_t)blockIdx.y * a.n.PT + pt0 + nb) * DT + dt) * 16 + r) * 64 + lane] = dacc[nb][dt][r];
    }
  }
}

__global__ __launch_bounds__(256) void nll_de_finalize(const float* __restrict__ partial, int ny, int64_t P,
                                                       int64_t PT, int D, int DT, const float* __restrict__ d_nll,
                                                       float factor, float* __restrict__ d_emb,
                                                       const float* __restrict__ own_term,
                                                       const int64_t* __restrict__ own,
                                                       const float* __restrict__ protos, float own_scale,
                                                       const PixelCoef* __restrict__ coef) {
  extern __shared__ float tile[];
  const int64_t pt = blockIdx.x;
  const int width = DT * 32, pitch = width + 1;
  const int n4 = DT * 256;
  for (int u = threadIdx.x; u < n4; u += 256) {
    float4v acc = {0.f, 0.f, 0.f, 0.f};
    for (int y = 0; y < ny; ++y)
      acc += *reinterpret_cast<const float4v*>(partial + (((size_t)y * PT + pt) * DT) * 1024 + 4 * (size_t)u);
    const int e = 4 * u;
    const int dt = e >> 10, r = (e >> 6) & 15, hf = (e >> 5) & 1, i = e & 31;
    const int d = 32 * dt + (r & 3) + 8 * (r >> 2) + 4 * hf;
#pragma unroll
    for (int q = 0; q < 4; ++q) tile[(i + q) * pitch + d] = acc[q];
  }
  __syncthreads();
  for (int o = threadIdx.x; o < 32 * D; o += 256) {
    const int i = o / D, d = o - i * D;
    const int64_t p = 32 * pt + i;
    if (p >= P) continue;
    float acc = tile[i * pitch + d];
    const float ts = coef[p].tscale;
    if (own_term) {
      const float ot = own_term[p];
      if (ot != 0.f) acc += ot * own_scale * ts * protos[(size_t)own[p] * D + d];
    }
    d_emb[(size_t)p * D + d] = acc * d_nll[p] * (factor / ts);
  }
}

template <int KS, int DT, bool TAG, bool C32, int TM = 0>
__global__ __launch_bounds__(256) void nll_bwd_dp(NllArgs a) {
  using CodeT = code_t<C32>;
  constexpr int kStd = TM == 2 ? 0 : 2 * KS + 2;
  constexpr int NBLK = kStd + 4 * DT;
  constexpr int SLOT = NBLK * 1024;
  const int DEPTH = a.depth;
  extern __shared__ __attribute__((aligned(16))) unsigned char sm[];
  const int lane = threadIdx.x & 63;
  const int wv = __builtin_amdgcn_readfirstlane(threadIdx.x >> 6);
  const int half = lane >> 5, j = lane & 31;
  const int64_t mt = min((int64_t)blockIdx.x * 4 + wv, a.n.MT - 1);
  const bool active = (int64_t)blockIdx.x * 4 + wv < a.mt_grad;
  const int64_t per = (a.spt1 - a.spt0 + a.chunks - 1) / a.chunks;
  const int64_t pt_lo = a.spt0 + (int64_t)blockIdx.y * per;
  const int64_t pt_hi = min(a.spt1, pt_lo + per);

  half8 bh[TM == 2 ? 1 : KS], bl[TM == 2 ? 1 : KS];
  if constexpr (TM != 2) {
#pragma unroll
    for (int ks = 0; ks < KS; ++ks) {
      bh[ks] = *reinterpret_cast<const half8*>(a.ph + (((size_t)mt * KS + ks) * 64 + lane) * 8);
      bl[ks] = *reinterpret_cast<const half8*>(a.pl + (((size_t)mt * KS + ks) * 64 + lane) * 8);
    }
  }
  const int col = (int)(32 * mt) + j;
  const bool col_ok = col < a.n.M;
  const CodeT ccode = (CodeT)a.pr_code_pad[col];

  float16v dacc[DT];
  LoAcc<DT> dlo;
  zero_lo<DT>(dlo);
#pragma unroll
  for (int dt = 0; dt < DT; ++dt)
#pragma unroll
    for (int r = 0; r < 16; ++r) dacc[dt][r] = 0.f;

  auto stage = [&](int64_t pt, int slot) {
    unsigned char* dst = sm + slot * SLOT;
    for (int b = wv; b < NBLK; b += 4) {
      const void* src;
      if (b < kStd && b < KS) src = a.eh + ((size_t)(pt * KS + b) * 64 + lane) * 8;
      else if (b < kStd && b < 2 * KS) src = a.el + ((size_t)(pt * KS + (b - KS)) * 64 + lane) * 8;
      else if (b < kStd && b == 2 * KS) src = a.coef + 32 * pt + min(lane, 31);
      else if (b < kStd) src = a.px_code_pad + 32 * pt + 2 * min(lane, 15);
      else {
        const int q = b - kStd;
        const size_t f = ((size_t)pt * a.dt_all + a.dt0) * 2 + (q >> 1);
        src = ((q & 1) ? a.etl : a.eth) + (f * 64 + lane) * 8;
      }
      dma_block(src, dst + (size_t)b * 1024);
    }
  };
  const int my_blocks = (NBLK - wv + 3) / 4;
  const int64_t ntile = pt_hi - pt_lo;
  for (int64_t t0 = 0; t0 < DEPTH - 1 && t0 < ntile; ++t0) stage(pt_lo + t0, (int)t0);
  int slot = -1;
  for (int64_t it = 0; it < ntile; ++it) {
    const int64_t pt = pt_lo + it;
    slot = slot + 1 == DEPTH ? 0 : slot + 1;
    if (it + 1 < ntile && DEPTH > 2) wait_vmcnt(my_blocks * (int)min((int64_t)(DEPTH - 2), ntile - 1 - it));
    else asm volatile("s_waitcnt vmcnt(0)" ::: "memory");
    wg_barrier();
    if (it + DEPTH - 1 < ntile) stage(pt + DEPTH - 1, slot == 0 ? DEPTH - 1 : slot - 1);
    const unsigned char* at = sm + slot * SLOT;
    const PixelCoef* coef = reinterpret_cast<const PixelCoef*>(at + 2 * KS * 1024);
    const int64_t* codes = reinterpret_cast<const int64_t*>(at + (2 * KS + 1) * 1024);
    float t[16];
    if constexpr (TM == 2) {
      tcache_load(a.tcache_dp, mt * (a.spt1 - a.spt0) + (pt - a.spt0), lane, t);
    } else {
      float16v zh, zx;
      zgemm_lds<KS>(at, lane, bh, bl, zh, zx);
      bool own_here = false;
  #pragma unroll
      for (int r = 0; r < 16; ++r) {
        const PixelCoef c = coef[tile_row(r, half)];
        const float s = __builtin_amdgcn_exp2f(zh[r] + zx[r] * kSplitInv);
        const bool same = code_match<TAG, CodeT>((CodeT)codes[tile_row(r, half)], ccode);
        float w = same ? c.wa : c.wb;
        w = c.tscale != 0.f ? w : 0.f;
        own_here |= (c.own == col);
        t[r] = s * w;
      }
      if (__any(own_here)) {
  #pragma unroll
        for (int r = 0; r < 16; ++r) {
          const PixelCoef c = coef[tile_row(r, half)];
          if (c.tscale != 0.f && c.own == col) {
            const int64_t pr = 32 * pt + tile_row(r, half);
            const float4v st = *reinterpret_cast<const float4v*>(a.stats + (size_t)pr * 4);
            const float s = __builtin_amdgcn_exp2f(zh[r] + zx[r] * kSplitInv);
            const bool same = code_match<TAG, CodeT>((CodeT)codes[tile_row(r, half)], ccode);
            const float inv_num = 1.0f / st[0];
            const float w = st[3] != 0.f ? ((c.wb - inv_num) + (same ? 0.f : c.wb))
                                         : (same ? 0.f : inv_num);
            t[r] = s * w;
          }
        }
      }
      if (!col_ok) {
  #pragma unroll
        for (int r = 0; r < 16; ++r) t[r] = 0.f;
      }
      if (TM == 1) tcache_store(a.tcache_dp, mt * (a.spt1 - a.spt0) + (pt - a.spt0), lane, t);
    }
    second_gemm<DT>(at + kStd * 1024, lane, t, dacc, dlo);
  }
  fold_lo<DT>(dlo, dacc);
  if (active && col_ok) {
    const float gs = a.gscale[0], igs = 1.0f / gs;
#pragma unroll
    for (int dt = 0; dt < DT; ++dt)
#pragma unroll
      for (int r = 0; r < 16; ++r) {
        const int d = 32 * (a.dt0 + dt) + tile_row(r, half);
        if (d < a.n.D) dpr_add(a, (size_t)col * a.n.D + d, dacc[dt][r] * gs, igs);
      }
  }
}

__global__ void pad_codes_kernel(const int64_t* in, int64_t n, int64_t n_pad, int64_t* out) {
  const int64_t i = (int64_t)blockIdx.x * 256 + threadIdx.x;
  if (i < n_pad) out[i] = i < n ? in[i] : 0;
}

__global__ void rowscale_kernel(const float* g, float kappa, int64_t n, float* out) {
  const int64_t i = (int64_t)blockIdx.x * 256 + threadIdx.x;
  if (i < n) out[i] = g[i] * kappa;
}

struct NllWs {
  size_t eh, el, ph, pl, pth, ptl, eth, etl, gscale, rowscale, codes, pxcodes, coef, ownterm, dprows, tde, tdp, partial, partial_de, dp64, total;
};

inline int64_t tcache_strip_tiles(const NllDims& n) {
  int64_t mb = 8192;
  if (const char* e = getenv("SPML_NLL_TCACHE_MB")) { const long long v = atoll(e); if (v > 0) mb = v; }
  int64_t tiles = (mb << 20) / (n.MT * 4096);
  tiles = tiles / 8 * 8;
  if (tiles < 8) tiles = 8;
  return tiles < n.PT ? tiles : n.PT;
}

inline int64_t fwd2_chunks(const NllDims& n) { return (n.MT + kFwd2TilesPerChunk - 1) / kFwd2TilesPerChunk; }
inline int bwd2_rows(const NllDims& n) { return (int)std::min<int64_t>(fwd2_chunks(n), 8); }

NllWs nll_ws(const NllDims& n) {
  NllWs w{};
  size_t o = 0;
  const size_t e_std = (size_t)n.PT * n.KS * 512 * 2, p_std = (size_t)n.MT * n.KS * 512 * 2;
  const size_t e_t = (size_t)n.PT * n.DT * 2 * 512 * 2, p_t = (size_t)n.MT * n.DT * 2 * 512 * 2;
  w.eh = o; o = align_up(o + e_std, 256);
  w.el = o; o = align_up(o + e_std, 256);
  w.ph = o; o = align_up(o + p_std, 256);
  w.pl = o; o = align_up(o + p_std, 256);
  w.pth = o; o = align_up(o + p_t, 256);
  w.ptl = o; o = align_up(o + p_t, 256);
  w.eth = o; o = align_up(o + e_t, 256);
  w.etl = o; o = align_up(o + e_t, 256);
  w.gscale = o; o = align_up(o + 16, 256);
  w.rowscale = o; o = align_up(o + (size_t)n.P * 4, 256);
  w.codes = o; o = align_up(o + (size_t)n.MT * 32 * 8, 256);
  w.pxcodes = o; o = align_up(o + (size_t)n.PT * 32 * 8, 256);
  w.coef = o; o = align_up(o + (size_t)n.PT * 32 * 16, 256);
  w.ownterm = o; o = align_up(o + (size_t)n.PT * 32 * 4, 256);
  w.dprows = o; o = align_up(o + nll_dp3_rows_bytes(n.PT), 256);
  w.tde = w.tdp = 0;
  if (n.KS > 17) {
    const size_t tiles = (size_t)tcache_strip_tiles(n) * n.MT * 4096;
    w.tde = o; o = align_up(o + tiles, 256);
    w.tdp = o; o = align_up(o + tiles, 256);
  }
  w.partial = 0;
  w.partial_de = 0;
  if (n.KS <= 5) {
    w.partial = o; o = align_up(o + (size_t)fwd2_chunks(n) * n.PT * 32 * 16, 256);
  }
  if (n.KS <= 4) {
    const size_t need = (size_t)bwd2_rows(n) * n.PT * n.DT * 4096;
    w.partial_de = w.partial;
    o = align_up(std::max(o, w.partial + need), 256);
  }
  w.dp64 = 0;
  if (deterministic_mode()) { w.dp64 = o; o = align_up(o + (size_t)n.MT * 32 * n.D * 8, 256); }
  w.total = o;
  return w;
}

__global__ void nll_dpr_from_fix(long long* __restrict__ acc, int64_t n, const float* __restrict__ gscale,
                                 float* __restrict__ d_protos) {
  const int64_t i = (int64_t)blockIdx.x * 256 + threadIdx.x;
  if (i >= n) return;
  const long long q = acc[i];
  if (q != 0) d_protos[i] += (float)((double)q * kDetFixInv) * gscale[0];
}

int ks_bucket(int ks) {
  if (ks <= 2) return 2;
  if (ks <= 3) return 3;
  if (ks <= 4) return 4;
  if (ks <= 5) return 5;
  if (ks <= 9) return 9;
  if (ks <= 17) return 17;
  if (ks <= 33) return 33;
  return 0;
}

int dt_per_launch(int ks) { return ks <= 17 ? (ks + 1) / 2 : 3; }

void launch_prep_std(const float* x, int64_t R, int D, int KS, float scale, _Float16* h,
                     _Float16* l, hipStream_t s) {
  const int64_t nfrag = ((R + 31) / 32) * KS;
  hipLaunchKernelGGL(prep_std<false>, dim3((unsigned)((nfrag + 3) / 4)), dim3(256), 0, s, x, R, D, KS,
                     scale, h, l);
}
void launch_prep_raw(const float* x, int64_t R, int D, int KS, float scale, _Float16* h,
                     _Float16* l, hipStream_t s) {
  const int64_t nfrag = ((R + 31) / 32) * KS;
  hipLaunchKernelGGL(prep_std<true>, dim3((unsigned)((nfrag + 3) / 4)), dim3(256), 0, s, x, R, D, KS,
                     scale, h, l);
}
void launch_prep_T(const float* x, int64_t R, int D, int DT, const float* rowscale,
                   const float* gscale, _Float16* h, _Float16* l, hipStream_t s) {
  const int64_t nfrag = ((R + 31) / 32) * DT * 2;
  hipLaunchKernelGGL(prep_T<false>, dim3((unsigned)((nfrag + 3) / 4)), dim3(256), 0, s, x, R, D, DT,
                     rowscale, gscale, 1.0f, h, l);
}
void launch_prep_T_raw(const float* x, int64_t R, int D, int DT, const float* rowscale,
                       const float* gscale, float scale, _Float16* h, _Float16* l, hipStream_t s) {
  const int64_t nfrag = ((R + 31) / 32) * DT * 2;
  hipLaunchKernelGGL(prep_T<true>, dim3((unsigned)((nfrag + 3) / 4)), dim3(256), 0, s, x, R, D, DT,
                     rowscale, gscale, scale, h, l);
}

}
}

using namespace spml;

extern "C" size_t spml_segsort_nll_workspace_bytes(int64_t P, int64_t M, int D) {
  if (P < 0 || M <= 0 || D <= 0) return 0;
  NllDims n = nll_dims(P, M, D);
  if (ks_bucket(n.KS)) {
    n.KS = ks_bucket(n.KS);
    const int per = dt_per_launch(n.KS);
    n.DT = ((n.KS + 1) / 2 + per - 1) / per * per;
  }
  return nll_ws(n).total;
}

static int nll_common(bool backward, const float* emb, const int64_t* own,
                      const int64_t* px_code, int64_t P, const float* protos,
                      const int64_t* pr_code, int64_t M, int D, float kappa, int mode,
                      float* nll, float* stats, const float* d_nll, float* d_emb,
                      float* d_protos, int64_t m_grad, void* ws, size_t ws_bytes, hipStream_t s) {
  if (!emb || !own || !px_code || !protos || !pr_code || P < 0 || M <= 0 || D <= 0 || !stats)
    return SPML_ERR_INVALID_ARG;
  if (mode < 0 || mode > (SPML_NLL_TAGSET | SPML_NLL_PLAIN | SPML_NLL_CODE32)) return SPML_ERR_INVALID_ARG;
  if (backward ? (!d_nll || !d_emb || !d_protos) : !nll) return SPML_ERR_INVALID_ARG;
  NllDims n = nll_dims(P, M, D);
  const int ksb = ks_bucket(n.KS);
  if (!ksb) return SPML_ERR_UNSUPPORTED;
  n.KS = ksb;
  const int dt_launch = dt_per_launch(ksb);
  n.DT = ((ksb + 1) / 2 + dt_launch - 1) / dt_launch * dt_launch;
  const NllWs w = nll_ws(n);
  if (!ws || ws_bytes < w.total) return SPML_ERR_WORKSPACE;
  if (P == 0) return SPML_OK;
  unsigned char* b = static_cast<unsigned char*>(ws);
  NllArgs a{};
  a.n = n;
  _Float16* eh = reinterpret_cast<_Float16*>(b + w.eh);
  _Float16* el = reinterpret_cast<_Float16*>(b + w.el);
  _Float16* ph = reinterpret_cast<_Float16*>(b + w.ph);
  _Float16* pl = reinterpret_cast<_Float16*>(b + w.pl);
  a.eh = eh; a.el = el; a.ph = ph; a.pl = pl;
  a.own = own; a.px_code = px_code; a.pr_code = pr_code;
  a.kappa = kappa;
  a.kappa_log2e = kappa * 1.4426950408889634f;
  a.mode = mode; a.nll = nll; a.stats = stats; a.d_nll = d_nll; a.d_emb = d_emb;
  a.d_protos = d_protos;
  int64_t* codes = reinterpret_cast<int64_t*>(b + w.codes);
  a.pr_code_pad = codes;
  hipLaunchKernelGGL(pad_codes_kernel, dim3((unsigned)((n.MT * 32 + 255) / 256)), dim3(256), 0, s,
                     pr_code, M, n.MT * 32, codes);
  const char* env2 = getenv("SPML_NLL_FWD2");
  const bool fwd2 = !backward && n.KS <= 5 && (mode & SPML_NLL_CODE32) && !(env2 && env2[0] == '0');
  if (fwd2) {
    launch_prep_raw(emb, P, D, n.KS, 8.0f, eh, el, s);
    launch_prep_raw(protos, M, D, n.KS, a.kappa_log2e * 0.125f, ph, pl, s);
    a.partial = reinterpret_cast<float*>(b + w.partial);
    const int64_t chunks = fwd2_chunks(n);
    const unsigned groups = (unsigned)((n.PT + 7) / 8);
#define SPML_FWD2(KS_, MTB_)                                                                        \
    {                                                                                               \
      constexpr int LDS2 = kFwd2TilesPerChunk * 128 + 2 * MTB_ * 2 * KS_ * 1024;                                         \
      if (mode & SPML_NLL_TAGSET) {                                                                 \
        (void)hipFuncSetAttribute(reinterpret_cast<const void*>(&nll_fwd2<KS_, MTB_, true>),        \
                                  hipFuncAttributeMaxDynamicSharedMemorySize, LDS2);                \
        hipLaunchKernelGGL((nll_fwd2<KS_, MTB_, true>), dim3(groups, (unsigned)chunks), dim3(256), LDS2, s, a); \
      } else {                                                                                      \
        (void)hipFuncSetAttribute(reinterpret_cast<const void*>(&nll_fwd2<KS_, MTB_, false>),       \
                                  hipFuncAttributeMaxDynamicSharedMemorySize, LDS2);                \
        hipLaunchKernelGGL((nll_fwd2<KS_, MTB_, false>), dim3(groups, (unsigned)chunks), dim3(256), LDS2, s, a); \
      }                                                                                             \
    }
    switch (n.KS) {
      case 2: SPML_FWD2(2, 4); break;
      case 3: SPML_FWD2(3, 4); break;
      case 4: SPML_FWD2(4, 4); break;
      default: SPML_FWD2(5, 2); break;
    }
#undef SPML_FWD2
    hipLaunchKernelGGL(nll_finalize, dim3((unsigned)((P + 255) / 256)), dim3(256), 0, s, a.partial, (int)chunks, P,
                       n.PT * 32, (mode & SPML_NLL_PLAIN) ? 1 : 0, nll, stats);
    return launch_status();
  }
  launch_prep_std(emb, P, D, n.KS, 1.0f, eh, el, s);
  launch_prep_std(protos, M, D, n.KS, a.kappa_log2e, ph, pl, s);

#define SPML_KS_SWITCH(MACRO)             \
  switch (n.KS) {                         \
    case 2: MACRO(2); break;              \
    case 3: MACRO(3); break;              \
    case 4: MACRO(4); break;              \
    case 5: MACRO(5); break;              \
    case 9: MACRO(9); break;              \
    case 17: MACRO(17); break;            \
    case 33: MACRO(33); break;            \
    default: return SPML_ERR_UNSUPPORTED; \
  }
  if (!backward) {
#define SPML_FWD_ONE(KS_, TAG_, C32_)                                                      \
    if (((mode & SPML_NLL_TAGSET) != 0) == TAG_ && ((mode & SPML_NLL_CODE32) != 0) == C32_) { \
      (void)hipFuncSetAttribute(reinterpret_cast<const void*>(&nll_fwd<KS_, NB, TAG_, C32_>), \
                                hipFuncAttributeMaxDynamicSharedMemorySize, lds_f);        \
      hipLaunchKernelGGL((nll_fwd<KS_, NB, TAG_, C32_>), dim3((unsigned)((waves + 3) / 4)), dim3(256), lds_f, s, a); \
    }
#define SPML_FWD(KS_)                                                                      \
  {                                                                                        \
    constexpr int NB = 1;                                                                  \
    constexpr int SLOT_F = (2 * KS_ + 1) * 1024;                                           \
     \
    a.depth_fwd = KS_ <= 5 ? 2 : (4 * SLOT_F <= 160 * 1024 ? 4 : 2);                       \
    if (const char* e_ = getenv("SPML_NLL_DEPTH_FWD")) { const int v_ = atoi(e_); if (v_ >= 2 && v_ <= 4) a.depth_fwd = v_; } \
    const int lds_f = a.depth_fwd * SLOT_F;                                                \
    const int64_t waves = (n.PT + NB - 1) / NB;                                            \
    SPML_FWD_ONE(KS_, true, true) SPML_FWD_ONE(KS_, true, false)                           \
    SPML_FWD_ONE(KS_, false, true) SPML_FWD_ONE(KS_, false, false)                         \
  }
    SPML_KS_SWITCH(SPML_FWD)
#undef SPML_FWD
#undef SPML_FWD_ONE
    return launch_status();
  }

  _Float16* pth = reinterpret_cast<_Float16*>(b + w.pth);
  _Float16* ptl = reinterpret_cast<_Float16*>(b + w.ptl);
  _Float16* eth = reinterpret_cast<_Float16*>(b + w.eth);
  _Float16* etl = reinterpret_cast<_Float16*>(b + w.etl);
  float* gscale = reinterpret_cast<float*>(b + w.gscale);
  float* rowscale = reinterpret_cast<float*>(b + w.rowscale);
  a.pth = pth; a.ptl = ptl; a.eth = eth; a.etl = etl; a.gscale = gscale;
  a.d_protos64 = nullptr;
  if (w.dp64) {
    a.d_protos64 = reinterpret_cast<long long*>(b + w.dp64);
    if (hipMemsetAsync(a.d_protos64, 0, (size_t)M * D * 8, s) != hipSuccess) return SPML_ERR_LAUNCH;
  }
  auto finish = [&](int rc) -> int {
    if (rc != SPML_OK) return rc;
    if (a.d_protos64)
      hipLaunchKernelGGL(nll_dpr_from_fix, dim3((unsigned)(((int64_t)M * D + 255) / 256)), dim3(256), 0, s,
                         a.d_protos64, (int64_t)M * D, (const float*)gscale, d_protos);
    return launch_status();
  };
  hipLaunchKernelGGL(max_abs_pow2, dim3(1), dim3(1024), 0, s, d_nll, P, gscale);
  hipLaunchKernelGGL(rowscale_kernel, dim3((unsigned)((P + 255) / 256)), dim3(256), 0, s, d_nll,
                     kappa, P, rowscale);
  launch_prep_T(protos, M, D, n.DT, nullptr, nullptr, pth, ptl, s);
  const auto env_off = [](const char* name) { const char* e = getenv(name); return e && e[0] == '0'; };
  const bool v3 = n.KS == 4 && (mode & SPML_NLL_CODE32) && !env_off("SPML_NLL_BWD2") && !env_off("SPML_NLL_DE3");
  const bool dp3 = v3 && !env_off("SPML_NLL_DP3");
  if (!dp3) launch_prep_T(emb, P, D, n.DT, rowscale, gscale, eth, etl, s);
  int64_t* pxcodes = reinterpret_cast<int64_t*>(b + w.pxcodes);
  PixelCoef* coef = reinterpret_cast<PixelCoef*>(b + w.coef);
  a.px_code_pad = pxcodes;
  a.coef = coef;
  a.tcache_de = w.tde ? reinterpret_cast<float*>(b + w.tde) : nullptr;
  a.tcache_dp = w.tdp ? reinterpret_cast<float*>(b + w.tdp) : nullptr;
  hipLaunchKernelGGL(pad_codes_kernel, dim3((unsigned)((n.PT * 32 + 255) / 256)), dim3(256), 0, s,
                     px_code, P, n.PT * 32, pxcodes);
  if (mode & SPML_NLL_TAGSET)
    hipLaunchKernelGGL(coef_kernel<true>, dim3((unsigned)((n.PT * 32 + 255) / 256)), dim3(256), 0, s, stats, own, px_code,
                       pr_code, M, P, n.PT * 32, coef);
  else
    hipLaunchKernelGGL(coef_kernel<false>, dim3((unsigned)((n.PT * 32 + 255) / 256)), dim3(256), 0, s, stats, own, px_code,
                       pr_code, M, P, n.PT * 32, coef);
  const int64_t mg = m_grad < 0 || m_grad > M ? M : m_grad;
  a.mt_grad = (mg + 31) / 32;
  const int64_t mgroups = (a.mt_grad + 3) / 4;
  int64_t chunks = mgroups > 0 ? (2048 + mgroups - 1) / mgroups : 1;
  if (chunks > (n.PT + 7) / 8) chunks = (n.PT + 7) / 8;
  if (chunks < 1) chunks = 1;
  if (chunks > 65535) chunks = 65535;
  a.chunks = (int)chunks;
  a.spt0 = 0;
  a.spt1 = n.PT;

  const char* envb = getenv("SPML_NLL_BWD2");
  const bool de2 = n.KS <= 4 && (mode & SPML_NLL_CODE32) && !(envb && envb[0] == '0');
  if (de2) {
    launch_prep_raw(emb, P, D, n.KS, 8.0f, eh, el, s);
    launch_prep_raw(protos, M, D, n.KS, a.kappa_log2e * 0.125f, ph, pl, s);
    launch_prep_T_raw(protos, M, D, n.DT, nullptr, nullptr, 8.0f, pth, ptl, s);
    a.partial_de = reinterpret_cast<float*>(b + w.partial_de);
    const int rows = bwd2_rows(n);
    const unsigned groups = (unsigned)((n.PT + 7) / 8);
#define SPML_DE2(KS_, DT_)                                                                          \
    {                                                                                               \
      constexpr int LDSB = kFwd2TilesPerChunk * 128 + 2 * 2 * (2 * KS_ + 4 * DT_) * 1024;           \
      if (mode & SPML_NLL_TAGSET) {                                                                 \
        (void)hipFuncSetAttribute(reinterpret_cast<const void*>(&nll_bwd_de2<KS_, DT_, 2, true>),   \
                                  hipFuncAttributeMaxDynamicSharedMemorySize, LDSB);                \
        hipLaunchKernelGGL((nll_bwd_de2<KS_, DT_, 2, true>), dim3(groups, (unsigned)rows), dim3(256), LDSB, s, a); \
      } else {                                                                                      \
        (void)hipFuncSetAttribute(reinterpret_cast<const void*>(&nll_bwd_de2<KS_, DT_, 2, false>),  \
                                  hipFuncAttributeMaxDynamicSharedMemorySize, LDSB);                \
        hipLaunchKernelGGL((nll_bwd_de2<KS_, DT_, 2, false>), dim3(groups, (unsigned)rows), dim3(256), LDSB, s, a); \
      }                                                                                             \
    }
    const bool use3 = v3;
    float* own_term = reinterpret_cast<float*>(b + w.ownterm);
    if (mode & SPML_NLL_TAGSET)
      hipLaunchKernelGGL(own_term_kernel<true>, dim3((unsigned)((n.PT * 32 + 255) / 256)), dim3(256), 0, s, stats, own,
                         px_code, pr_code, emb, protos, P, n.PT * 32, M, D, a.kappa_log2e, own_term);
    else
      hipLaunchKernelGGL(own_term_kernel<false>, dim3((unsigned)((n.PT * 32 + 255) / 256)), dim3(256), 0, s, stats, own,
                         px_code, pr_code, emb, protos, P, n.PT * 32, M, D, a.kappa_log2e, own_term);
    if (use3) {
      const int rc3 = nll_launch_bwd_de3(a, rows, s);
      if (rc3 != SPML_OK) return rc3;
    } else {
      switch (n.KS) {
        case 2: SPML_DE2(2, 1); break;
        case 3: SPML_DE2(3, 2); break;
        default: SPML_DE2(4, 2); break;
      }
    }
#undef SPML_DE2
    hipLaunchKernelGGL(nll_de_finalize, dim3((unsigned)n.PT), dim3(256), (size_t)32 * (n.DT * 32 + 1) * sizeof(float), s, a.partial_de, rows, P, n.PT, D, n.DT,
                       d_nll, kappa * 0.125f, d_emb, (const float*)own_term, own, protos, 8.0f, (const PixelCoef*)coef);
    if (dp3) {
      hipLaunchKernelGGL(rowscale_ts_kernel, dim3((unsigned)((P + 255) / 256)), dim3(256), 0, s, d_nll, kappa,
                         (const PixelCoef*)coef, P, rowscale);
      launch_prep_T_raw(emb, P, D, n.DT, rowscale, gscale, 16.0f, eth, etl, s);
      return finish(nll_launch_bwd_dp3(a, own_term, emb, reinterpret_cast<float*>(b + w.dprows), s));
    }
    launch_prep_std(emb, P, D, n.KS, 1.0f, eh, el, s);
    launch_prep_std(protos, M, D, n.KS, a.kappa_log2e, ph, pl, s);
  }
  a.skip_de = de2 ? 1 : 0;

#define SPML_BWD_LAUNCH(KS_, DT_, TAG_, C32_, TM_)                                                    \
  {                                                                                              \
    constexpr int STD_DE = TM_ == 2 ? 0 : 2 * KS_ + 1, STD_DP = TM_ == 2 ? 0 : 2 * KS_ + 2;      \
    constexpr int SLOT_DE = (STD_DE + 4 * DT_) * 1024, SLOT_DP = (STD_DP + 4 * DT_) * 1024;      \
                                          \
    a.depth = KS_ <= 5 ? 2 : (3 * SLOT_DP <= 80 * 1024 ? 3 : 2);                                 \
    if (const char* e_ = getenv("SPML_NLL_DEPTH_BWD")) { const int v_ = atoi(e_); if (v_ >= 2 && v_ <= 3) a.depth = v_; } \
    if (2 * SLOT_DP > 160 * 1024) return SPML_ERR_UNSUPPORTED;                                   \
    (void)hipFuncSetAttribute(reinterpret_cast<const void*>(&nll_bwd_de<KS_, DT_, TAG_, C32_, TM_>),   \
                              hipFuncAttributeMaxDynamicSharedMemorySize, a.depth * SLOT_DE);    \
    (void)hipFuncSetAttribute(reinterpret_cast<const void*>(&nll_bwd_dp<KS_, DT_, TAG_, C32_, TM_>),   \
                              hipFuncAttributeMaxDynamicSharedMemorySize, a.depth * SLOT_DP);    \
    if (!a.skip_de)                                                                              \
      hipLaunchKernelGGL((nll_bwd_de<KS_, DT_, TAG_, C32_, TM_>), dim3((unsigned)((a.spt1 - a.spt0 + 3) / 4)), \
                         dim3(256), a.depth * SLOT_DE, s, a);                                    \
    if (mgroups > 0)                                                                             \
      hipLaunchKernelGGL((nll_bwd_dp<KS_, DT_, TAG_, C32_, TM_>), dim3((unsigned)mgroups, (unsigned)a.chunks), \
                         dim3(256), a.depth * SLOT_DP, s, a);                                    \
  }
#define SPML_BWD_DT(KS_, DT_, TAG_, C32_)                                                              \
  {                                                                                              \
    a.dt_all = n.DT;                                                                             \
    if constexpr (KS_ > 17) {                                                                    \
                                     \
      if (a.tcache_de != nullptr && 32 * DT_ < D) {                                              \
        const int64_t strip = tcache_strip_tiles(n);                                             \
        for (int64_t t0 = 0; t0 < n.PT; t0 += strip) {        \
          a.spt0 = t0;                                                                           \
          a.spt1 = t0 + strip < n.PT ? t0 + strip : n.PT;                                        \
          int64_t ch = chunks;                                                                   \
          if (ch > (a.spt1 - a.spt0 + 7) / 8) ch = (a.spt1 - a.spt0 + 7) / 8;                    \
          a.chunks = (int)(ch < 1 ? 1 : ch);                                                     \
          a.dt0 = 0;                                                                             \
          SPML_BWD_LAUNCH(KS_, DT_, TAG_, C32_, 1)                                               \
          for (int dt0 = DT_; 32 * dt0 < D; dt0 += 7) {                                          \
            a.dt0 = dt0;                                                                         \
            SPML_BWD_LAUNCH(KS_, 7, TAG_, C32_, 2)                                               \
          }                                                                                      \
        }                                                                                        \
      } else {                                                                                   \
        for (int dt0 = 0; dt0 < n.DT && 32 * dt0 < D; dt0 += DT_) {                              \
          a.dt0 = dt0;                                                                           \
          SPML_BWD_LAUNCH(KS_, DT_, TAG_, C32_, 0)                                               \
        }                                                                                        \
      }                                                                                          \
    } else {                                                                                     \
      for (int dt0 = 0; dt0 < n.DT && 32 * dt0 < D; dt0 += DT_) {     \
        a.dt0 = dt0;                                                                             \
        SPML_BWD_LAUNCH(KS_, DT_, TAG_, C32_, 0)                                                 \
      }                                                                                          \
    }                                                                                            \
  }
#define SPML_BWD(KS_)                                          \
  {                                                            \
    constexpr int DTM = KS_ <= 17 ? (KS_ + 1) / 2 : 3;         \
     \
    if (mode & SPML_NLL_TAGSET) SPML_BWD_DT(KS_, DTM, true, false)   \
    else SPML_BWD_DT(KS_, DTM, false, false)                   \
  }
  SPML_KS_SWITCH(SPML_BWD)
#undef SPML_BWD
#undef SPML_BWD_DT
#undef SPML_BWD_LAUNCH
#undef SPML_KS_SWITCH
  return finish(SPML_OK);
}

extern "C" int spml_segsort_nll_fwd_f32(const float* emb, const int64_t* own,
                                        const int64_t* px_code, int64_t P, const float* protos,
                                        const int64_t* pr_code, int64_t M, int D, float kappa,
                                        int mode, float* nll, float* stats, void* ws,
                                        size_t ws_bytes, void* stream) {
  return nll_common(false, emb, own, px_code, P, protos, pr_code, M, D, kappa, mode, nll, stats,
                    nullptr, nullptr, nullptr, -1, ws, ws_bytes, (hipStream_t)stream);
}

extern "C" int spml_segsort_nll_bwd_f32(const float* emb, const int64_t* own,
                                        const int64_t* px_code, int64_t P, const float* protos,
                                        const int64_t* pr_code, int64_t M, int D, float kappa,
                                        int mode, const float* stats, const float* d_nll,
                                        float* d_emb, float* d_protos, int64_t m_grad, void* ws,
                                        size_t ws_bytes, void* stream) {
  return nll_common(true, emb, own, px_code, P, protos, pr_code, M, D, kappa, mode, nullptr,
                    const_cast<float*>(stats), d_nll, d_emb, d_protos, m_grad, ws, ws_bytes,
                    (hipStream_t)stream);
}
```

spml_amd/csrc/nll_common.hpp:

```cpp
#pragma once

#include <type_traits>

#include "common.hpp"

namespace spml {

struct NllDims {
  int64_t P, M;
  int D, KS, DT;
  int64_t PT, MT;
};

__host__ __device__ inline NllDims nll_dims(int64_t P, int64_t M, int D) {
  NllDims n;
  n.P = P; n.M = M; n.D = D;
  n.KS = (D + 15) / 16;
  n.DT = (D + 31) / 32;
  n.PT = (P + 31) / 32;
  n.MT = (M + 31) / 32;
  return n;
}

__device__ __forceinline__ int tile_row(int r, int h) { return (r & 3) + 8 * (r >> 2) + 4 * h; }

constexpr int kFwd2TilesPerChunk = 96;

constexpr float kTScale = 16384.0f;

__host__ __device__ inline float nll_t_scale(float num, float den, float own_sim, bool fallback, bool own_is_same) {
  if (fallback || own_is_same) return kTScale;
  const float b = (num + own_sim) * fabsf(1.0f / den - 1.0f / num);
  if (!(b > 1.0f) || !(b < 3.0e38f)) return kTScale;
  int ex = 0;
  frexpf(b, &ex);
  return ldexpf(kTScale, -(ex > 40 ? 40 : ex));
}

struct PixelCoef {
  float wa, wb;
  int own;
  float tscale;
};

struct NllArgs {
  NllDims n;
  const _Float16 *eh, *el;
  const _Float16 *ph, *pl;
  const _Float16 *pth, *ptl;
  const _Float16 *eth, *etl;
  const int64_t* own;
  const int64_t* px_code;
  const int64_t* pr_code;
  const int64_t* pr_code_pad;
  const int64_t* px_code_pad;
  const struct PixelCoef* coef;
  int64_t mt_grad;
  int depth;
  int depth_fwd;
  int dt0, dt_all;
  float kappa_log2e, kappa;
  int mode;
  float* nll;
  float* stats;
  const float* d_nll;
  const float* gscale;
  float* d_emb;
  float* d_protos;
  long long* d_protos64;
  int chunks;
  float* tcache_de;
  float* tcache_dp;
  int64_t spt0, spt1;
  float* partial;
  int skip_de;
  float* partial_de;
};

__device__ __forceinline__ void dpr_add(const NllArgs& a, size_t idx, float v, float inv_gscale) {
  if (a.d_protos64) det_atomic_add(a.d_protos64 + idx, v * inv_gscale);
  else unsafeAtomicAdd(a.d_protos + idx, v);
}

template <bool TAG, typename T>
__device__ __forceinline__ bool code_match(T a, T b) {
  if constexpr (sizeof(T) == 4) return TAG ? ((unsigned)(a & b) != 0u) : ((unsigned)a == (unsigned)b);
  else return TAG ? ((a & b) != 0) : (a == b);
}
template <bool C32>
using code_t = typename std::conditional<C32, int, int64_t>::type;

typedef const __attribute__((address_space(1))) void* gptr_t;
typedef __attribute__((address_space(3))) void* lptr_t;

__device__ __forceinline__ void dma_block(const void* src_lane, void* dst_wave_uniform) {
  __builtin_amdgcn_global_load_lds((gptr_t)src_lane, (lptr_t)dst_wave_uniform, 16, 0, 0);
}
__device__ __forceinline__ void dma_wait_and_sync() {
  asm volatile("s_waitcnt vmcnt(0) lgkmcnt(0)\n\ts_barrier" ::: "memory");
}

int nll_launch_bwd_de3(const NllArgs& a, int rows, hipStream_t s);

size_t nll_dp3_rows_bytes(int64_t PT);
int nll_launch_bwd_dp3(const NllArgs& a, const float* own_term, const float* emb, float* rows, hipStream_t s);

}
```

spml_amd/models/predictions/segsort.py:

```python
import os

import torch
import torch.nn as nn

import spml_amd.utils.segsort.common as segsort_common
import spml_amd.utils.segsort.eval as segsort_eval
from spml_amd import parallel
import spml_amd.utils.segsort.loss as segsort_loss


_streams = {}


def _side_streams(device, n):
  if n <= 1:
    return []
  key = (torch.device(device).index, n)
  if key not in _streams:
    _streams[key] = [torch.cuda.Stream(device=device) for _ in range(n)]
  return _streams[key]


def _nonzero_pair(mask_a, mask_b, extra=None):
  head = torch.stack([mask_a.sum(), mask_b.sum()])
  vals = (torch.cat([head, extra.reshape(-1).to(head.dtype)]) if extra is not None else head).tolist()
  counts, tail = vals[:2], vals[2:]
  out = []
  for mask, n in zip((mask_a, mask_b), counts):
    mask = mask.reshape(-1)
    dst = torch.where(mask, torch.cumsum(mask, 0) - 1, torch.full_like(mask, n, dtype=torch.long))
    src = torch.arange(mask.shape[0], device=mask.device)
    out.append(src.new_empty((n + 1,)).scatter_(0, dst, src)[:n])
  return (out[0], out[1], tail) if extra is not None else out


class Segsort(nn.Module):

  def __init__(self, config):
    super().__init__()
    t = config.train
    self.sem_ann_loss = self._construct_loss(t.sem_ann_loss_types,
                                             concentration=t.sem_ann_concentration)
    self.sem_ann_loss_weight = t.sem_ann_loss_weight
    occ_type = 'set_segsort' if t.sem_occ_loss_types == 'segsort' else 'none'
    self.sem_occ_loss = self._construct_loss(occ_type, concentration=t.sem_occ_concentration)
    self.sem_occ_loss_weight = t.sem_occ_loss_weight
    self.img_sim_loss = self._construct_loss(t.img_sim_loss_types,
                                             concentration=t.img_sim_concentration)
    self.img_sim_loss_weight = t.img_sim_loss_weight
    self.feat_aff_loss = self._construct_loss(t.feat_aff_loss_types,
                                              concentration=t.feat_aff_concentration)
    enabled = bool(t.get('evaluate_feat_aff', False)) and t.feat_aff_loss_types == 'segsort'
    self.feat_aff_set_loss = self._construct_loss(
        'set_segsort' if enabled else 'none', concentration=t.feat_aff_concentration)
    self.feat_aff_loss_weight = t.feat_aff_loss_weight
    self.semantic_ignore_index = config.dataset.semantic_ignore_index
    self.num_classes = config.dataset.num_classes
    self.label_divisor = config.network.label_divisor

  def _construct_loss(self, loss_types, **kwargs):
    if loss_types == 'segsort':
      return segsort_loss.SegSortLoss(kwargs['concentration'], group_mode='segsort+',
                                      reduction='mean')
    if loss_types == 'set_segsort':
      return segsort_loss.SetSegSortLoss(kwargs['concentration'], group_mode='segsort+',
                                         reduction='mean')
    if loss_types == 'none':
      return None
    raise KeyError('Unsupported loss types: {:s}'.format(loss_types))

  def segment_predictions(self, datas, targets={}):
    memory = targets.get('semantic_memory_prototype', None)
    memory_labels = targets.get('semantic_memory_prototype_label', None)
    emb = datas.get('cluster_embedding', None)
    clu = datas.get('cluster_index', None)
    if memory is None or memory_labels is None or emb is None or clu is None:
      return None, None
    _, clu = torch.unique(clu, return_inverse=True)
    m = int(clu.max()) + 1
    protos = segsort_common.calculate_prototypes_from_labels(emb, clu, m)
    dummy = torch.zeros(m, dtype=torch.long, device=protos.device)
    _, topk = segsort_eval.top_k_ranking(protos, dummy, memory, memory_labels, 20)
    return topk, clu

  def predictions(self, datas, targets={}):
    topk, clu = self.segment_predictions(datas, targets)
    if topk is None:
      return None, None
    pred = segsort_eval.majority_label_from_topk(topk)
    return pred[clu], topk[clu]

  img_sim_embedding_key = 'cluster_embedding_with_loc'

  def _memory_bank_ready(self, targets):
    return all(targets.get(k, []) for k in (
        'memory_prototype', 'memory_prototype_semantic_label',
        'memory_prototype_semantic_tag', 'memory_prototype_batch_index'))

  def _occurrence_sets(self, targets, use_memory, clu, bat, p_sem, p_bat):
    nc = self.num_classes
    p_tags = targets['prototype_semantic_tag'][:, 1:nc]
    if use_memory:
      p_tags = torch.cat([p_tags] + [t[:, 1:nc] for t in targets['memory_prototype_semantic_tag']])
    img_sets, p_sets = segsort_loss.pack_tag_set_pair(targets['semantic_tag'][:, 1:nc], p_tags)
    return img_sets[bat], p_sets

  def _contrastive_losses(self, datas, targets):
    sem_ann = sem_occ = img_sim = acc = None
    nc = self.num_classes

    sim = None
    if self.img_sim_loss is not None:
      clu = datas['cluster_index']
      ins = datas['cluster_instance_label']
      bat = datas['cluster_batch_index']
      sizes = datas.get('cluster_image_sizes', None)
      if sizes is None:
        sizes = torch.unique_consecutive(bat, return_counts=True)[1].tolist()
      sizes = [int(v) for v in sizes if int(v) > 0]
      n_img, total = len(sizes), int(clu.shape[0])
      img_of_px = torch.zeros_like(bat)
      if total > 1:
        img_of_px[1:] = torch.cumsum(bat[1:] != bat[:-1], 0)
      off = ins.max() + 1
      stride = (clu.max() + 1) * off
      uniq, pair = segsort_common._unique_inverse((img_of_px * (clu.max() + 1) + clu) * off + ins,
                                                  with_uniq=False, padded=True)
      bounds = torch.arange(1, n_img + 1, device=uniq.device) * stride
      sim = (sizes, off, uniq, pair, torch.searchsorted(uniq, bounds) - 1)
    last = None

    if self.sem_ann_loss is not None or self.sem_occ_loss is not None:
      clu = datas['cluster_index']
      emb = datas['cluster_embedding']
      sem = datas['cluster_semantic_label']
      bat = datas['cluster_batch_index']
      protos = targets['prototype']
      live = protos.shape[0]
      p_sem = targets['prototype_semantic_label']
      p_bat = targets['prototype_batch_index']

      mem_p = targets.get('memory_prototype', [])
      mem_sem = targets.get('memory_prototype_semantic_label', [])
      mem_bat = targets.get('memory_prototype_batch_index', [])
      use_memory = self._memory_bank_ready(targets)
      if use_memory:
        protos = torch.cat([protos] + list(mem_p), dim=0)
        p_sem = torch.cat([p_sem] + list(mem_sem), dim=0)
        p_bat = torch.cat([p_bat] + list(mem_bat), dim=0)
      px_sets, p_sets = self._occurrence_sets(targets, use_memory, clu, bat, p_sem, p_bat)

      labelled = p_sem < nc
      if sim is not None:
        px, pr, last = _nonzero_pair(sem < nc, labelled, extra=sim[4])
      else:
        px, pr = _nonzero_pair(sem < nc, labelled)
      remap = torch.cumsum(labelled, 0) - 1
      remap = torch.where(labelled, remap, torch.full_like(remap, pr.shape[0]))
      new_clu = remap[clu]

      if self.sem_ann_loss is not None:
        sem_ann = self.sem_ann_loss(emb[px], sem[px], new_clu[px], protos[pr], p_sem[pr],
                                    codes32=True)
        sem_ann = sem_ann * self.sem_ann_loss_weight
      if self.sem_occ_loss is not None:
        sem_occ = self.sem_occ_loss(emb, px_sets, clu, protos, p_sets,
                                    prototype_grad_rows=live, codes32=self.num_classes <= 32)
        sem_occ = sem_occ * self.sem_occ_loss_weight
      acc = parallel.sharded_retrieval_accuracy(segsort_eval.top_k_ranking, protos, p_sem, 5)

    if sim is not None:
      sizes, off, uniq, pair, last_dev = sim
      emb = datas[self.img_sim_embedding_key]
      ins = datas['cluster_instance_label']
      if last is None:
        last = last_dev.tolist()
      last = [int(v) for v in last]
      pair_lab = uniq[:last[-1] + 1] % off
      terms, lo, first = [], 0, 0
      pr_all = e_all = None
      if os.environ.get('SPML_IMG_SIM_BATCHED_PROTOS') != '0' and sum(sizes) == int(emb.shape[0]):
        counts = [end + 1 - (last[i - 1] + 1 if i else 0) for i, end in enumerate(last)]
        pr_all = torch.split(segsort_common.calculate_prototypes_from_labels(emb, pair, last[-1] + 1), counts)
        e_all = torch.split(emb, sizes)
      streams = _side_streams(emb.device, int(os.environ.get('SPML_IMG_SIM_STREAMS', '4'))) if emb.is_cuda else []
      cur = torch.cuda.current_stream(emb.device) if streams else None
      for st in streams:
        st.wait_stream(cur)
      for i, (n_px, end) in enumerate(zip(sizes, last)):
        lab, c_abs, first_i = ins[lo:lo + n_px], pair[lo:lo + n_px], first
        e = e_all[i] if e_all is not None else emb[lo:lo + n_px]
        p_lab = pair_lab[first:end + 1]
        lo, first = lo + n_px, end + 1
        if streams:
          side = streams[i % len(streams)]
          if os.environ.get('SPML_IMG_SIM_RECORD_STREAM') != '0':
            for t_ in (e, lab, c_abs, p_lab) + ((pr_all[i],) if pr_all is not None else ()):
              t_.record_stream(side)
          with torch.cuda.stream(side):
            c = c_abs - first_i
            pr_img = pr_all[i] if pr_all is not None else \
                segsort_common.calculate_prototypes_from_labels(e, c, p_lab.shape[0])
            term = self.img_sim_loss(e, lab, c, pr_img, p_lab, codes32=True)
            term.record_stream(cur)
          terms.append(term)
          continue
        c = c_abs - first_i
        pr_img = pr_all[i] if pr_all is not None else \
            segsort_common.calculate_prototypes_from_labels(e, c, p_lab.shape[0])
        terms.append(self.img_sim_loss(e, lab, c, pr_img, p_lab, codes32=True))
      for st in streams:
        cur.wait_stream(st)
      img_sim = sum(terms) / len(terms) * self.img_sim_loss_weight

    return sem_ann, sem_occ, img_sim, acc

  def feature_affinity_loss(self, datas, targets):
    import spml_amd.models.utils as model_utils
    protos = targets['prototype']
    protos_loc = targets['prototype_with_loc']
    p_sem = targets['prototype_semantic_label']
    p_bat = targets['prototype_batch_index']
    live = protos.shape[0]
    mem_p = targets.get('memory_prototype', [])
    mem_pl = targets.get('memory_prototype_with_loc', [])
    mem_sem = targets.get('memory_prototype_semantic_label', [])
    mem_bat = targets.get('memory_prototype_batch_index', [])
    if mem_p and mem_sem and mem_bat:
      protos = torch.cat([protos] + list(mem_p), dim=0)
      protos_loc = torch.cat([protos_loc] + list(mem_pl), dim=0)
      p_sem = torch.cat([p_sem] + list(mem_sem), dim=0)
      p_bat = torch.cat([p_bat] + list(mem_bat), dim=0)
    tags = model_utils.gather_multiset_labels_per_batch_by_nearest_neighbor(
        protos_loc, protos_loc, p_sem, p_bat, p_bat, num_classes=self.num_classes, top_k=1,
        threshold=0.95, label_divisor=self.label_divisor)
    untagged = tags.max(dim=1, keepdim=True)[0] == 0
    tags = tags.masked_fill(untagged.expand(-1, self.num_classes), 1)
    clu = datas['cluster_index']
    loss = self.feat_aff_set_loss(datas['cluster_embedding'], tags[clu], clu, protos, tags,
                                  prototype_grad_rows=live, codes32=self.num_classes <= 32)
    return loss * self.feat_aff_loss_weight

  def losses(self, datas, targets={}):
    return self._contrastive_losses(datas, targets)

  def forward(self, datas, targets=None, with_loss=True, with_prediction=False):
    targets = targets if targets is not None else {}
    outputs = {}
    if with_prediction:
      pred, score = self.predictions(datas, targets)
      outputs.update({'semantic_prediction': pred, 'semantic_score': score})
    if with_loss:
      sem_ann, sem_occ, img_sim, acc = self.losses(datas, targets)
      outputs.update({'sem_ann_loss': sem_ann, 'sem_occ_loss': sem_occ,
                      'img_sim_loss': img_sim, 'accuracy': acc})
      if self.feat_aff_set_loss is not None:
        outputs['feat_aff_loss'] = self.feature_affinity_loss(datas, targets)
    return outputs

  def get_params_lr(self):
    return []


def segsort(config):
  return Segsort(config)
```

spml_amd/ops.py:

```python
import torch
import torch.nn.functional as F

from . import _ffi

NLL_LABEL, NLL_TAGSET, NLL_PLAIN, NLL_CODE32 = 0, 1, 2, 4


def _f32c(t):
  t = t if t.dtype == torch.float32 else t.float()
  return t if t.is_contiguous() else t.contiguous()


def _i64c(t):
  t = t if t.dtype == torch.int64 else t.long()
  return t if t.is_contiguous() else t.contiguous()


class _NormalizeRows(torch.autograd.Function):

  @staticmethod
  def forward(ctx, x):
    x = _f32c(x)
    ctx.save_for_backward(x)
    return _ffi.normalize_rows(x)

  @staticmethod
  def backward(ctx, dy):
    (x,) = ctx.saved_tensors
    return _ffi.normalize_rows_bwd(x, _f32c(dy))


def normalize_rows(x):
  return _NormalizeRows.apply(x)


class _NormalizeConcatLoc(torch.autograd.Function):

  @staticmethod
  def forward(ctx, emb, loc, row_map, num_rows):
    if not (emb.is_cuda and _ffi.k1_channels_last(emb, 2 if loc is None else int(loc.shape[-1]))):
      emb = _f32c(emb)
    loc = None if loc is None else _f32c(loc)
    ctx.save_for_backward(emb, loc, row_map)
    out_emb, out_loc = _ffi.normalize_concat_loc(emb, loc, row_map, num_rows)
    return out_emb, out_loc

  @staticmethod
  def backward(ctx, d_emb_rows, d_loc_rows):
    emb, loc, row_map = ctx.saved_tensors
    d_emb_rows = None if d_emb_rows is None else _f32c(d_emb_rows)
    d_loc_rows = None if d_loc_rows is None else _f32c(d_loc_rows)
    return _ffi.normalize_concat_loc_bwd(emb, loc, row_map, d_emb_rows, d_loc_rows), None, None, None


K1_MAX_GRAD_CHANNELS = 512


def normalize_concat_loc(emb_nchw, loc=None, row_map=None, num_rows=None):
  if emb_nchw.requires_grad and torch.is_grad_enabled() and emb_nchw.shape[1] > K1_MAX_GRAD_CHANNELS:
    raise _ffi.SpmlHipError('the K1 backward kernels take at most %d channels (got %d)' % (
        K1_MAX_GRAD_CHANNELS, emb_nchw.shape[1]))
  return _NormalizeConcatLoc.apply(emb_nchw, loc, row_map, num_rows)


class _SegmentPrototypes(torch.autograd.Function):

  @staticmethod
  def forward(ctx, x, ids, m):
    x, ids = _f32c(x), _i64c(ids)
    protos, sums = _ffi.segment_sum_normalize(x, ids, m)
    ctx.save_for_backward(sums, ids)
    ctx.p = x.shape[0]
    return protos

  @staticmethod
  def backward(ctx, d_protos):
    sums, ids = ctx.saved_tensors
    return _ffi.segment_sum_normalize_bwd(_f32c(d_protos), sums, ids, ctx.p), None, None


def segment_prototypes(x, ids, m):
  return _SegmentPrototypes.apply(x, ids, int(m))


class _SegSortNLL(torch.autograd.Function):

  @staticmethod
  def forward(ctx, emb, own, px_code, protos, pr_code, kappa, mode, m_grad):
    emb, protos = _f32c(emb), _f32c(protos)
    own, px_code, pr_code = _i64c(own), _i64c(px_code), _i64c(pr_code)
    nll, stats = _ffi.segsort_nll_fwd(emb, own, px_code, protos, pr_code, kappa, mode)
    ctx.save_for_backward(emb, own, px_code, protos, pr_code, stats)
    ctx.kappa, ctx.mode, ctx.m_grad = kappa, mode, m_grad
    return nll

  @staticmethod
  def backward(ctx, d_nll):
    emb, own, px_code, protos, pr_code, stats = ctx.saved_tensors
    d_emb, d_protos = _ffi.segsort_nll_bwd(emb, own, px_code, protos, pr_code, ctx.kappa,
                                           ctx.mode, stats, _f32c(d_nll), ctx.m_grad)
    return d_emb, None, None, d_protos, None, None, None, None


def segsort_nll(emb, own, px_code, protos, pr_code, kappa, mode=NLL_LABEL, proto_grad_rows=None):
  if emb.shape[0] == 0:
    return emb.new_zeros((0,))
  m_grad = -1 if proto_grad_rows is None else int(proto_grad_rows)
  return _SegSortNLL.apply(emb, own, px_code, protos, pr_code, float(kappa), int(mode), m_grad)


def kmeans(x, seg_offsets, max_seg_len, k, labels_init, iterations, want_centroids=False):
  with torch.no_grad():
    return _ffi.kmeans_run(_f32c(x.detach()), _i64c(seg_offsets), int(max_seg_len), int(k),
                           _i64c(labels_init), int(iterations), want_centroids)


def kmeans_assign(x, seg_offsets, max_seg_len, centroids):
  with torch.no_grad():
    return _ffi.kmeans_assign(_f32c(x.detach()), _i64c(seg_offsets), int(max_seg_len),
                              _f32c(centroids.detach()))


def topk_affinity(q, protos, k, q_group=None, pr_group=None, pr_valid=None, masked_value=-2.0):
  with torch.no_grad():
    return _ffi.topk_affinity(
        _f32c(q.detach()), _f32c(protos.detach()), int(k),
        None if q_group is None else _i64c(q_group),
        None if pr_group is None else _i64c(pr_group),
        None if pr_valid is None else pr_valid.to(torch.uint8).contiguous(), masked_value)


def kmeans_init_grid(h, w, ky, kx, device):
  return _ffi.kmeans_init_grid(int(h), int(w), int(ky), int(kx), device)


def merge_bn_statistics(counts, means, m2s):
  total = counts.sum(0)
  mean = (means * counts).sum(0) / total
  m2 = (m2s + counts * (means - mean) ** 2).sum(0)
  return total, mean, m2


class _BatchNormAct(torch.autograd.Function):

  @staticmethod
  def forward(ctx, x, residual, weight, bias, running_mean, running_var, momentum, eps, relu, group):
    import torch.distributed as dist
    n, c, h, w = x.shape
    count = n * h * w
    world = dist.get_world_size(group) if group is not None else 1
    ctx.count, ctx.group, ctx.world = count * world, group, world
    ctx.has_res = residual is not None
    if world == 1:
      y, mean, invstd = _ffi.bn_act_fwd(x, residual, weight, bias, running_mean, running_var, momentum,
                                        eps, relu)
      ctx.save_for_backward(x, y if relu else None, mean, invstd, weight)
      return y
    mean, m2 = _ffi.bn_stats(x)
    stats = torch.stack([torch.full_like(mean, float(count)), mean, m2])
    allst = torch.empty((world * 3, stats.shape[1]), dtype=stats.dtype, device=stats.device)
    dist.all_gather_into_tensor(allst, stats, group=group)
    allst = allst.view(world, 3, stats.shape[1])
    mean, invstd, ctx.count = _ffi.bn_finalize_ranks(allst, eps, momentum if running_mean is not None else 0.0,
                                                     running_mean, running_var)
    y = _ffi.bn_act_apply(x, residual, mean, invstd, weight, bias, relu)
    ctx.save_for_backward(x, y if relu else None, mean, invstd, weight)
    return y

  @staticmethod
  def backward(ctx, dy):
    import torch.distributed as dist
    x, y, mean, invstd, weight = ctx.saved_tensors
    dy = dy if dy.is_contiguous(memory_format=torch.channels_last) else \
        dy.contiguous(memory_format=torch.channels_last)
    need_x, need_res = ctx.needs_input_grad[0], ctx.has_res and ctx.needs_input_grad[1]
    if ctx.world == 1:
      dx, dres, d_weight, d_bias = _ffi.bn_act_bwd(dy, y, x, mean, invstd, weight, want_dx=need_x,
                                                   want_dres=need_res)
      return dx, dres, d_weight, d_bias, None, None, None, None, None, None
    s0, s1 = _ffi.bn_act_bwd_reduce(dy, y, x, mean, invstd)
    d_weight, d_bias = s1.clone(), s0.clone()
    if ctx.world > 1:
      both = torch.stack([s0, s1])
      dist.all_reduce(both, group=ctx.group)
      s0, s1 = both[0].contiguous(), both[1].contiguous()
    dx, dres = _ffi.bn_act_bwd_apply(dy, y, x, mean, invstd, weight, s0, s1, ctx.count, want_dx=need_x,
                                     want_dres=need_res)
    return dx, dres, d_weight, d_bias, None, None, None, None, None, None


def fused_bn_act_available(x, bn):
  import os
  if os.environ.get('SPML_NO_FUSED_BN') == '1':
    return False
  return (x.is_cuda and x.dtype == torch.float32 and x.dim() == 4 and bn.training and bn.affine and
          bn.track_running_stats and x.shape[1] % 4 == 0 and
          x.is_contiguous(memory_format=torch.channels_last) and x.shape[0] * x.shape[2] * x.shape[3] > 1)


def batch_norm_act(x, bn, relu=True, residual=None):
  if fused_bn_act_available(x, bn) and (residual is None or
                                        residual.is_contiguous(memory_format=torch.channels_last)):
    group = None
    if isinstance(bn, torch.nn.SyncBatchNorm):
      import torch.distributed as dist
      if dist.is_available() and dist.is_initialized():
        group = bn.process_group if bn.process_group is not None else dist.group.WORLD
    if bn.num_batches_tracked is not None:
      bn.num_batches_tracked.add_(1)
    momentum = bn.momentum if bn.momentum is not None else 1.0 / float(bn.num_batches_tracked)
    y = _BatchNormAct.apply(x, residual, bn.weight, bn.bias, bn.running_mean, bn.running_var,
                            momentum, bn.eps, bool(relu), group)
    torch.autograd.graph.increment_version((bn.running_mean, bn.running_var))
    return y
  from spml_amd.nn.batchnorm import native_batch_norm
  y = native_batch_norm(bn, x)
  if residual is not None:
    y = y + residual
  return torch.relu(y) if relu else y


class _UpsampleCrossEntropy(torch.autograd.Function):

  @staticmethod
  def forward(ctx, logits, labels, ignore_index):
    nhwc = logits.permute(0, 2, 3, 1).contiguous()
    labels = _i64c(labels)
    result, lse = _ffi.upsample_ce_fwd(nhwc, labels, ignore_index)
    ctx.save_for_backward(nhwc, labels, lse, result)
    ctx.ignore_index = ignore_index
    return result[2]

  @staticmethod
  def backward(ctx, d_loss):
    nhwc, labels, lse, result = ctx.saved_tensors
    scale = (d_loss.to(torch.float32) / result[1]).reshape(1).contiguous()
    d = _ffi.upsample_ce_bwd(nhwc, labels, lse, ctx.ignore_index, scale)
    return d.permute(0, 3, 1, 2), None, None


def upsample_cross_entropy_available(logits, labels):
  return (logits.is_cuda and logits.dtype == torch.float32 and logits.dim() == 4 and labels.dim() == 3 and
          labels.shape[0] == logits.shape[0] and _ffi.upsample_ce_supported(logits.shape[1]))


def upsample_cross_entropy(logits, labels, ignore_index):
  return _UpsampleCrossEntropy.apply(logits, labels, int(ignore_index))


_interp_cache = {}


def _interp_matrix(n_in, n_out, device, dtype=torch.float32):
  key = (n_in, n_out, str(device), dtype)
  m = _interp_cache.get(key)
  if m is None:
    eye = torch.eye(n_in, device=device, dtype=dtype).view(1, 1, n_in, n_in)
    m = F.interpolate(eye, size=(n_out, n_in), mode='bilinear')[0, 0].contiguous()
    _interp_cache[key] = m
  return m

# ... 24 lines not shown
```

spml_amd/utils/segsort/loss.py:

```python
import torch
from torch.nn.modules.loss import _Loss

from spml_amd import ops


def _mode(group_mode, base, codes32=False):
  return (base | (0 if group_mode == 'segsort+' else ops.NLL_PLAIN) |
          (ops.NLL_CODE32 if codes32 else 0))


def _bit_weights(num, device):
  return torch.bitwise_left_shift(torch.ones((num,), dtype=torch.long, device=device),
                                  torch.arange(num, dtype=torch.long, device=device))


def pack_tag_sets(tags):
  if tags.dim() == 1:
    return tags
  if tags.shape[1] > 63:
    raise ValueError('tag sets wider than 63 classes need pack_tag_set_pair (pixel and prototype tags together)')
  return ((tags != 0).long() * _bit_weights(tags.shape[1], tags.device).view(1, -1)).sum(1)


def pack_tag_set_pair(pixel_tags, prototype_tags):
  t = pixel_tags.shape[1]
  if t <= 63:
    return pack_tag_sets(pixel_tags), pack_tag_sets(prototype_tags)
  active = (pixel_tags != 0).any(0) & (prototype_tags != 0).any(0)
  rank = torch.cumsum(active.long(), 0) - 1
  n_active = int(rank[-1]) + 1
  if n_active > 63:
    raise ValueError('%d classes are shared between pixels and prototypes in this call; the packed '
                     'tag-set kernels take at most 63' % n_active)
  weights = torch.where(active, torch.bitwise_left_shift(torch.ones_like(rank), rank.clamp(min=0)),
                        torch.zeros_like(rank))
  pack = lambda tags: ((tags != 0).long() * weights.view(1, -1)).sum(1)
  return pack(pixel_tags), pack(prototype_tags)


def _calculate_log_likelihood(embeddings, semantic_labels, instance_labels, prototypes,
                              prototype_semantic_labels, concentration, group_mode,
                              prototype_grad_rows=None, codes32=False):
  embeddings = embeddings.reshape(-1, embeddings.shape[-1])
  prototypes = prototypes.reshape(-1, prototypes.shape[-1])
  nll = ops.segsort_nll(embeddings, instance_labels.reshape(-1), semantic_labels.reshape(-1),
                        prototypes, prototype_semantic_labels.reshape(-1), concentration,
                        _mode(group_mode, ops.NLL_LABEL, codes32), prototype_grad_rows)
  return nll.view(-1, 1)


def _one_hot_calculate_log_likelihood(embeddings, semantic_labels, instance_labels, prototypes,
                                      prototype_semantic_labels, concentration, group_mode,
                                      prototype_grad_rows=None, codes32=False):
  embeddings = embeddings.reshape(-1, embeddings.shape[-1])
  prototypes = prototypes.reshape(-1, prototypes.shape[-1])
  codes32 = codes32 or (semantic_labels.dim() == 2 and semantic_labels.shape[1] <= 32 and
                        prototype_semantic_labels.dim() == 2 and
                        prototype_semantic_labels.shape[1] <= 32)
  if semantic_labels.dim() == 2 and prototype_semantic_labels.dim() == 2:
    px_sets, pr_sets = pack_tag_set_pair(semantic_labels, prototype_semantic_labels)
  else:
    px_sets, pr_sets = pack_tag_sets(semantic_labels), pack_tag_sets(prototype_semantic_labels)
  nll = ops.segsort_nll(embeddings, instance_labels.reshape(-1), px_sets, prototypes, pr_sets, concentration,
                        _mode(group_mode, ops.NLL_TAGSET, codes32), prototype_grad_rows)
  return nll.view(-1, 1)


class _NcaLoss(_Loss):
  _kernel = None
  _name = ''

  def __init__(self, concentration=10, group_mode='segsort+', size_average=None, reduce=None,
               reduction='mean'):
    super().__init__(size_average, reduce, reduction)
    self.concentration = concentration
    self.group_mode = group_mode

  def __repr__(self):
    return '{}(concentration={:.2f}, group_mode={})'.format(
        self._name, self.concentration, self.group_mode)

  def forward(self, embeddings, semantic_labels, instance_labels, prototypes,
              prototype_semantic_labels, prototype_weights=None, prototype_grad_rows=None,
              codes32=False):
    nll = type(self)._kernel(embeddings, semantic_labels, instance_labels, prototypes,
                             prototype_semantic_labels, self.concentration, self.group_mode,
                             prototype_grad_rows, codes32)
    if self.reduction == 'mean':
      return torch.mean(nll)
    if self.reduction == 'sum':
      return torch.sum(nll)
    return nll


class SegSortLoss(_NcaLoss):
  _kernel = staticmethod(_calculate_log_likelihood)
  _name = 'SegSortLoss'


class SetSegSortLoss(_NcaLoss):
  _kernel = staticmethod(_one_hot_calculate_log_likelihood)
  _name = 'SetSegSortLoss'
```

Baseline: 133.8.

## Batch per-image segsort NLL into single grouped-launch kernels

Adds batched forward and backward segsort NLL entry points. Each takes per-problem pixel and prototype offsets, so all images' image-similarity losses are computed in one set of kernel launches instead of a per-image loop spread over side streams. The existing kernels are split into device bodies plus thin wrappers, and an own_base offset lets absolute prototype indices be reused. This aims to cut launch and stream-sync overhead for many small per-image problems, at the cost of a batch cap of 32, packing offsets on the host for every call, and a different per-image mean reduction path.

After: 137.0 (median of 6 runs). +2.4%, better.

```diff
diff --git a/include/spml_hip.h b/include/spml_hip.h
--- a/include/spml_hip.h
+++ b/include/spml_hip.h
@@ -175,6 +175,26 @@
                              float* d_emb, float* d_protos, int64_t m_grad,
                              void* ws, size_t ws_bytes, void* stream);
 
+int spml_segsort_nll_batched_supported(int D, int mode);
+
+size_t spml_segsort_nll_batched_workspace_bytes(int n_problems, const int64_t* p_off,
+                                                const int64_t* m_off, int D);
+
+int spml_segsort_nll_batched_fwd_f32(const float* emb, const int64_t* own,
+                                     const int64_t* px_code, const int64_t* p_off,
+                                     const float* protos, const int64_t* pr_code,
+                                     const int64_t* m_off, int n_problems, int D,
+                                     float kappa, int mode, float* nll, float* stats,
+                                     void* ws, size_t ws_bytes, void* stream);
+
+int spml_segsort_nll_batched_bwd_f32(const float* emb, const int64_t* own,
+                                     const int64_t* px_code, const int64_t* p_off,
+                                     const float* protos, const int64_t* pr_code,
+                                     const int64_t* m_off, int n_problems, int D,
+                                     float kappa, int mode, const float* stats,
+                                     const float* d_nll, float* d_emb, float* d_protos,
+                                     void* ws, size_t ws_bytes, void* stream);
+
 size_t spml_topk_workspace_bytes(int64_t Q, int64_t M, int D, int k);
 
 int spml_topk_affinity_f32(const float* q, int64_t Q, const float* protos,
diff --git a/spml_amd/_ffi.py b/spml_amd/_ffi.py
--- a/spml_amd/_ffi.py
+++ b/spml_amd/_ffi.py
@@ -54,6 +54,12 @@
                                          _P, _P, _P, c_size_t, _P]),
     'spml_segsort_nll_bwd_f32': (c_int, [_P, _P, _P, c_int64, _P, _P, c_int64, c_int, c_float, c_int,
                                          _P, _P, _P, _P, c_int64, _P, c_size_t, _P]),
+    'spml_segsort_nll_batched_supported': (c_int, [c_int, c_int]),
+    'spml_segsort_nll_batched_workspace_bytes': (c_size_t, [c_int, _P, _P, c_int]),
+    'spml_segsort_nll_batched_fwd_f32': (c_int, [_P, _P, _P, _P, _P, _P, _P, c_int, c_int, c_float, c_int,
+                                                 _P, _P, _P, c_size_t, _P]),
+    'spml_segsort_nll_batched_bwd_f32': (c_int, [_P, _P, _P, _P, _P, _P, _P, c_int, c_int, c_float, c_int,
+                                                 _P, _P, _P, _P, _P, c_size_t, _P]),
     'spml_topk_workspace_bytes': (c_size_t, [c_int64, c_int64, c_int, c_int]),
     'spml_topk_affinity_f32': (c_int, [_P, c_int64, _P, c_int64, c_int, c_int, _P, _P, _P, c_float,
                                        _P, _P, _P, c_size_t, _P]),
@@ -495,6 +501,58 @@
   return d_emb, d_protos
 
 
+def segsort_nll_batched_supported(d, mode):
+  return bool(lib().spml_segsort_nll_batched_supported(int(d), int(mode)))
+
+
+def _host_offsets(sizes):
+  off = (c_int64 * (len(sizes) + 1))()
+  for i, v in enumerate(sizes):
+    off[i + 1] = off[i] + int(v)
+  return off
+
+
+def _nll_batched_workspace(p_off, m_off, n, d, device):
+  nbytes = lib().spml_segsort_nll_batched_workspace_bytes(n, p_off, m_off, d)
+  if nbytes == 0 and n > 0:
+    raise SpmlHipError('spml_segsort_nll_batched_workspace_bytes refused the sizes (D = %d)' % d)
+  return workspace(nbytes, device)
+
+
+def segsort_nll_batched_fwd(emb, own_abs, px_code, p_sizes, protos, pr_code, m_sizes, kappa, mode):
+  p, d = emb.shape
+  n = len(p_sizes)
+  p_off, m_off = _host_offsets(p_sizes), _host_offsets(m_sizes)
+  if len(m_sizes) != n or p_off[n] != p or m_off[n] != protos.shape[0]:
+    raise SpmlHipError('the problem sizes do not add up to the rows given')
+  nll = torch.empty((p,), dtype=torch.float32, device=emb.device)
+  stats = torch.empty((p, 4), dtype=torch.float32, device=emb.device)
+  ws = _nll_batched_workspace(p_off, m_off, n, d, emb.device)
+  check(lib().spml_segsort_nll_batched_fwd_f32(
+      ptr(emb, torch.float32), ptr(own_abs, torch.int64), ptr(px_code, torch.int64), p_off,
+      ptr(protos, torch.float32), ptr(pr_code, torch.int64), m_off, n, d, float(kappa), int(mode),
+      ptr(nll), ptr(stats), ptr(ws), ws.numel(), stream_ptr()), 'spml_segsort_nll_batched_fwd_f32')
+  return nll, stats
+
+
+def segsort_nll_batched_bwd(emb, own_abs, px_code, p_sizes, protos, pr_code, m_sizes, kappa, mode, stats, d_nll):
+  p, d = emb.shape
+  n = len(p_sizes)
+  p_off, m_off = _host_offsets(p_sizes), _host_offsets(m_sizes)
+  if len(m_sizes) != n or p_off[n] != p or m_off[n] != protos.shape[0] or \
+      stats.shape[0] != p or d_nll.shape[0] != p:
+    raise SpmlHipError('the problem sizes do not add up to the rows given')
+  d_emb = torch.empty_like(emb)
+  d_protos = torch.zeros_like(protos)
+  ws = _nll_batched_workspace(p_off, m_off, n, d, emb.device)
+  check(lib().spml_segsort_nll_batched_bwd_f32(
+      ptr(emb, torch.float32), ptr(own_abs, torch.int64), ptr(px_code, torch.int64), p_off,
+      ptr(protos, torch.float32), ptr(pr_code, torch.int64), m_off, n, d, float(kappa), int(mode),
+      ptr(stats, torch.float32), ptr(d_nll, torch.float32), ptr(d_emb), ptr(d_protos),
+      ptr(ws), ws.numel(), stream_ptr()), 'spml_segsort_nll_batched_bwd_f32')
+  return d_emb, d_protos
+
+
 def topk_affinity(q, protos, k, q_group=None, pr_group=None, pr_valid=None, masked_value=-2.0):
   nq, d = q.shape
   m = protos.shape[0]
diff --git a/spml_amd/csrc/nll.hip b/spml_amd/csrc/nll.hip
--- a/spml_amd/csrc/nll.hip
+++ b/spml_amd/csrc/nll.hip
@@ -7,9 +7,9 @@
 namespace {
 
 template <bool RAW>
-__global__ __launch_bounds__(256) void prep_std(const float* __restrict__ x, int64_t R, int D,
-                                                int KS, float scale, _Float16* __restrict__ oh,
-                                                _Float16* __restrict__ ol) {
+__device__ __forceinline__ void prep_std_body(const float* __restrict__ x, int64_t R, int D,
+                                              int KS, float scale, _Float16* __restrict__ oh,
+                                              _Float16* __restrict__ ol) {
   const int64_t f = (int64_t)blockIdx.x * 4 + (threadIdx.x >> 6);
   const int64_t nfrag = ((R + 31) / 32) * KS;
   if (f >= nfrag) return;
@@ -35,13 +35,19 @@
   *reinterpret_cast<half8*>(oh + ((size_t)f * 64 + lane) * 8) = h;
   *reinterpret_cast<half8*>(ol + ((size_t)f * 64 + lane) * 8) = l;
 }
-
 template <bool RAW>
-__global__ __launch_bounds__(256) void prep_T(const float* __restrict__ x, int64_t R, int D,
-                                              int DT, const float* __restrict__ rowscale,
-                                              const float* __restrict__ gscale, float scale,
-                                              _Float16* __restrict__ oh,
-                                              _Float16* __restrict__ ol) {
+__global__ __launch_bounds__(256) void prep_std(const float* __restrict__ x, int64_t R, int D,
+                                                int KS, float scale, _Float16* __restrict__ oh,
+                                                _Float16* __restrict__ ol) {
+  prep_std_body<RAW>(x, R, D, KS, scale, oh, ol);
+}
+
+template <bool RAW>
+__device__ __forceinline__ void prep_T_body(const float* __restrict__ x, int64_t R, int D,
+                                            int DT, const float* __restrict__ rowscale,
+                                            const float* __restrict__ gscale, float scale,
+                                            _Float16* __restrict__ oh,
+                                            _Float16* __restrict__ ol) {
   const int64_t f = (int64_t)blockIdx.x * 4 + (threadIdx.x >> 6);
   const int64_t nfrag = ((R + 31) / 32) * DT * 2;
   if (f >= nfrag) return;
@@ -74,9 +80,17 @@
   *reinterpret_cast<half8*>(oh + ((size_t)f * 64 + lane) * 8) = h;
   *reinterpret_cast<half8*>(ol + ((size_t)f * 64 + lane) * 8) = l;
 }
-
-__global__ __launch_bounds__(1024) void max_abs_pow2(const float* __restrict__ g, int64_t n,
-                                                     float* __restrict__ out) {
+template <bool RAW>
+__global__ __launch_bounds__(256) void prep_T(const float* __restrict__ x, int64_t R, int D,
+                                              int DT, const float* __restrict__ rowscale,
+                                              const float* __restrict__ gscale, float scale,
+                                              _Float16* __restrict__ oh,
+                                              _Float16* __restrict__ ol) {
+  prep_T_body<RAW>(x, R, D, DT, rowscale, gscale, scale, oh, ol);
+}
+
+__device__ __forceinline__ void max_abs_pow2_body(const float* __restrict__ g, int64_t n,
+                                                  float* __restrict__ out) {
   __shared__ float red[16];
   float m = 0.f;
   for (int64_t i = threadIdx.x; i < n; i += 1024) m = fmaxf(m, fabsf(g[i]));
@@ -94,6 +108,10 @@
     }
     out[0] = p;
   }
+}
+__global__ __launch_bounds__(1024) void max_abs_pow2(const float* __restrict__ g, int64_t n,
+                                                     float* __restrict__ out) {
+  max_abs_pow2_body(g, n, out);
 }
 
 template <int KS>
@@ -231,7 +249,7 @@
 
 
 template <int KS, int MTB, bool TAG>
-__global__ __launch_bounds__(256, 2) void nll_fwd2(NllArgs a) {
+__device__ __forceinline__ void nll_fwd2_body(const NllArgs& a) {
   constexpr int TILE = 2 * KS * 1024;
   constexpr int SLOT = MTB * TILE;
   constexpr int CODES = kFwd2TilesPerChunk * 32 * 4;
@@ -275,7 +293,7 @@
     }
     const int64_t p = min(32 * pt + j, a.n.P - 1);
     pcode[nb] = (int)a.px_code[p];
-    own[nb] = (int)a.own[p] - (int)(32 * mt_lo);
+    own[nb] = (int)(a.own[p] - a.own_base) - (int)(32 * mt_lo);
     s_same[nb] = 0.f; s_all[nb] = 0.f; s_own[nb] = 0.f;
   }
 
@@ -441,10 +459,14 @@
     }
   }
 }
-
-__global__ __launch_bounds__(256) void nll_finalize(const float* __restrict__ partial, int chunks,
-                                                    int64_t P, int64_t P_pad, int plain,
-                                                    float* __restrict__ nll, float* __restrict__ stats) {
+template <int KS, int MTB, bool TAG>
+__global__ __launch_bounds__(256, 2) void nll_fwd2(NllArgs a) {
+  nll_fwd2_body<KS, MTB, TAG>(a);
+}
+
+__device__ __forceinline__ void nll_finalize_body(const float* __restrict__ partial, int chunks,
+                                                  int64_t P, int64_t P_pad, int plain,
+                                                  float* __restrict__ nll, float* __restrict__ stats) {
   const int64_t p = (int64_t)blockIdx.x * 256 + threadIdx.x;
   if (p >= P) return;
   float same = 0.f, all = 0.f, osim = 0.f;
@@ -460,11 +482,17 @@
   const float4v st = {num, den, osim, fb ? 1.f : 0.f};
   *reinterpret_cast<float4v*>(stats + (size_t)p * 4) = st;
 }
+__global__ __launch_bounds__(256) void nll_finalize(const float* __restrict__ partial, int chunks,
+                                                    int64_t P, int64_t P_pad, int plain,
+                                                    float* __restrict__ nll, float* __restrict__ stats) {
+  nll_finalize_body(partial, chunks, P, P_pad, plain, nll, stats);
+}
 
 template <bool TAG>
-__global__ void coef_kernel(const float* __restrict__ stats, const int64_t* __restrict__ own,
-                            const int64_t* __restrict__ px_code, const int64_t* __restrict__ pr_code, int64_t M,
-                            int64_t P, int64_t P_pad, PixelCoef* __restrict__ out) {
+__device__ __forceinline__ void coef_body(const float* __restrict__ stats, const int64_t* __restrict__ own,
+                                          const int64_t* __restrict__ px_code, const int64_t* __restrict__ pr_code,
+                                          int64_t M, int64_t P, int64_t P_pad, int64_t own_base,
+                                          PixelCoef* __restrict__ out) {
   const int64_t i = (int64_t)blockIdx.x * 256 + threadIdx.x;
   if (i >= P_pad) return;
   PixelCoef c{0.f, 0.f, -1, 0.f};
@@ -473,12 +501,18 @@
     const float inv_num = 1.0f / st[0], inv_den = 1.0f / st[1];
     c.wa = st[3] != 0.f ? 0.f : inv_den - inv_num;
     c.wb = inv_den;
-    c.own = (int)own[i];
-    const int64_t m = own[i];
+    const int64_t m = own[i] - own_base;
+    c.own = (int)m;
     const bool own_same = m >= 0 && m < M && code_match<TAG, int64_t>(px_code[i], pr_code[m]);
     c.tscale = nll_t_scale(st[0], st[1], st[2], st[3] != 0.f, own_same);
   }
   out[i] = c;
+}
+template <bool TAG>
+__global__ void coef_kernel(const float* __restrict__ stats, const int64_t* __restrict__ own,
+                            const int64_t* __restrict__ px_code, const int64_t* __restrict__ pr_code, int64_t M,
+                            int64_t P, int64_t P_pad, PixelCoef* __restrict__ out) {
+  coef_body<TAG>(stats, own, px_code, pr_code, M, P, P_pad, 0, out);
 }
 
 __global__ void rowscale_ts_kernel(const float* g, float kappa, const PixelCoef* __restrict__ coef, int64_t n, float* out) {
@@ -594,7 +628,7 @@
 }
 
 template <int KS, int DT, bool TAG, bool C32, int TM = 0>
-__global__ __launch_bounds__(256) void nll_bwd_de(NllArgs a) {
+__device__ __forceinline__ void nll_bwd_de_body(const NllArgs& a) {
   using CodeT = code_t<C32>;
   constexpr int kStd = TM == 2 ? 0 : 2 * KS + 1;
   constexpr int NBLK = kStd + 4 * DT;
@@ -703,6 +737,10 @@
       }
   }
 }
+template <int KS, int DT, bool TAG, bool C32, int TM = 0>
+__global__ __launch_bounds__(256) void nll_bwd_de(NllArgs a) {
+  nll_bwd_de_body<KS, DT, TAG, C32, TM>(a);
+}
 
 template <int KS, int DT, int MTB, bool TAG>
 __global__ __launch_bounds__(256, 2) void nll_bwd_de2(NllArgs a) {
@@ -909,7 +947,7 @@
 }
 
 template <int KS, int DT, bool TAG, bool C32, int TM = 0>
-__global__ __launch_bounds__(256) void nll_bwd_dp(NllArgs a) {
+__device__ __forceinline__ void nll_bwd_dp_body(const NllArgs& a) {
   using CodeT = code_t<C32>;
   constexpr int kStd = TM == 2 ? 0 : 2 * KS + 2;
   constexpr int NBLK = kStd + 4 * DT;
@@ -1028,10 +1066,17 @@
       }
   }
 }
-
-__global__ void pad_codes_kernel(const int64_t* in, int64_t n, int64_t n_pad, int64_t* out) {
+template <int KS, int DT, bool TAG, bool C32, int TM = 0>
+__global__ __launch_bounds__(256) void nll_bwd_dp(NllArgs a) {
+  nll_bwd_dp_body<KS, DT, TAG, C32, TM>(a);
+}
+
+__device__ __forceinline__ void pad_codes_body(const int64_t* in, int64_t n, int64_t n_pad, int64_t* out) {
   const int64_t i = (int64_t)blockIdx.x * 256 + threadIdx.x;
   if (i < n_pad) out[i] = i < n ? in[i] : 0;
+}
+__global__ void pad_codes_kernel(const int64_t* in, int64_t n, int64_t n_pad, int64_t* out) {
+  pad_codes_body(in, n, n_pad, out);
 }
 
 __global__ void rowscale_kernel(const float* g, float kappa, int64_t n, float* out) {
@@ -1052,8 +1097,16 @@
   return tiles < n.PT ? tiles : n.PT;
 }
 
-inline int64_t fwd2_chunks(const NllDims& n) { return (n.MT + kFwd2TilesPerChunk - 1) / kFwd2TilesPerChunk; }
+__host__ __device__ inline int64_t fwd2_chunks(const NllDims& n) { return (n.MT + kFwd2TilesPerChunk - 1) / kFwd2TilesPerChunk; }
 inline int bwd2_rows(const NllDims& n) { return (int)std::min<int64_t>(fwd2_chunks(n), 8); }
+
+__host__ __device__ inline int64_t dp_chunks(int64_t mgroups, int64_t PT) {
+  int64_t chunks = mgroups > 0 ? (2048 + mgroups - 1) / mgroups : 1;
+  if (chunks > (PT + 7) / 8) chunks = (PT + 7) / 8;
+  if (chunks < 1) chunks = 1;
+  if (chunks > 65535) chunks = 65535;
+  return chunks;
+}
 
 NllWs nll_ws(const NllDims& n) {
   NllWs w{};
@@ -1097,12 +1150,16 @@
   return w;
 }
 
-__global__ void nll_dpr_from_fix(long long* __restrict__ acc, int64_t n, const float* __restrict__ gscale,
-                                 float* __restrict__ d_protos) {
+__device__ __forceinline__ void nll_dpr_from_fix_body(long long* __restrict__ acc, int64_t n,
+                                                      const float* __restrict__ gscale, float* __restrict__ d_protos) {
   const int64_t i = (int64_t)blockIdx.x * 256 + threadIdx.x;
   if (i >= n) return;
   const long long q = acc[i];
   if (q != 0) d_protos[i] += (float)((double)q * kDetFixInv) * gscale[0];
+}
+__global__ void nll_dpr_from_fix(long long* __restrict__ acc, int64_t n, const float* __restrict__ gscale,
+                                 float* __restrict__ d_protos) {
+  nll_dpr_from_fix_body(acc, n, gscale, d_protos);
 }
 
 int ks_bucket(int ks) {
@@ -1141,6 +1198,295 @@
   const int64_t nfrag = ((R + 31) / 32) * DT * 2;
   hipLaunchKernelGGL(prep_T<true>, dim3((unsigned)((nfrag + 3) / 4)), dim3(256), 0, s, x, R, D, DT,
                      rowscale, gscale, scale, h, l);
+}
+
+
+constexpr int kNllBatchMax = 32;
+struct NllBatch {
+  NllArgs a;
+  int count, first;
+  int64_t p_off[kNllBatchMax + 1], m_off[kNllBatchMax + 1];
+  int64_t pt_off[kNllBatchMax + 1], mt_off[kNllBatchMax + 1];
+  int64_t part_off[kNllBatchMax + 1];
+  const float* emb;
+  const float* protos;
+  float* rowscale;
+};
+static_assert(sizeof(NllBatch) <= 2048, "a kernel argument");
+
+__device__ __forceinline__ bool batch_problem(const NllBatch& b, int z, NllArgs& a) {
+  const int64_t p0 = b.p_off[z], m0 = b.m_off[z], pt0 = b.pt_off[z], mt0 = b.mt_off[z];
+  const int64_t P = b.p_off[z + 1] - p0;
+  if (P <= 0) return false;
+  a = b.a;
+  a.n.P = P;
+  a.n.M = b.m_off[z + 1] - m0;
+  a.n.PT = b.pt_off[z + 1] - pt0;
+  a.n.MT = b.mt_off[z + 1] - mt0;
+  const size_t ks = (size_t)a.n.KS * 512, dt = (size_t)a.n.DT * 1024, D = (size_t)a.n.D;
+  a.eh += pt0 * ks; a.el += pt0 * ks; a.ph += mt0 * ks; a.pl += mt0 * ks;
+  a.pth += mt0 * dt; a.ptl += mt0 * dt; a.eth += pt0 * dt; a.etl += pt0 * dt;
+  a.own += p0; a.own_base = m0;
+  a.px_code += p0; a.pr_code += m0;
+  a.pr_code_pad += mt0 * 32; a.px_code_pad += pt0 * 32; a.coef += pt0 * 32;
+  a.mt_grad = a.n.MT;
+  a.nll += p0; a.stats += p0 * 4; a.d_nll += p0;
+  a.gscale += b.first + z;
+  a.d_emb += p0 * D; a.d_protos += m0 * D;
+  if (a.d_protos64) a.d_protos64 += m0 * D;
+  a.chunks = (int)dp_chunks((a.n.MT + 3) / 4, a.n.PT);
+  a.spt0 = 0; a.spt1 = a.n.PT;
+  a.partial += b.part_off[z] * 4;
+  return true;
+}
+
+template <int KS, int MTB, bool TAG>
+__global__ __launch_bounds__(256, 2) void nll_fwd2_batched(NllBatch b) {
+  NllArgs a;
+  if (!batch_problem(b, blockIdx.z, a)) return;
+  if (blockIdx.x >= (a.n.PT + 7) / 8 || blockIdx.y >= fwd2_chunks(a.n)) return;
+  nll_fwd2_body<KS, MTB, TAG>(a);
+}
+template <int KS, int DT, bool TAG>
+__global__ __launch_bounds__(256) void nll_bwd_de_batched(NllBatch b) {
+  NllArgs a;
+  if (!batch_problem(b, blockIdx.z, a)) return;
+  if (blockIdx.x >= (a.n.PT + 3) / 4) return;
+  nll_bwd_de_body<KS, DT, TAG, false, 0>(a);
+}
+template <int KS, int DT, bool TAG>
+__global__ __launch_bounds__(256) void nll_bwd_dp_batched(NllBatch b) {
+  NllArgs a;
+  if (!batch_problem(b, blockIdx.z, a)) return;
+  if (blockIdx.x >= (a.mt_grad + 3) / 4 || (int)blockIdx.y >= a.chunks) return;
+  nll_bwd_dp_body<KS, DT, TAG, false, 0>(a);
+}
+__global__ void pad_codes_batched(NllBatch b, int px) {
+  NllArgs a;
+  if (!batch_problem(b, blockIdx.z, a)) return;
+  if (px) pad_codes_body(a.px_code, a.n.P, a.n.PT * 32, const_cast<int64_t*>(a.px_code_pad));
+  else pad_codes_body(a.pr_code, a.n.M, a.n.MT * 32, const_cast<int64_t*>(a.pr_code_pad));
+}
+template <bool RAW>
+__global__ __launch_bounds__(256) void prep_std_batched(NllBatch b, int px, float scale) {
+  NllArgs a;
+  if (!batch_problem(b, blockIdx.z, a)) return;
+  if (px)
+    prep_std_body<RAW>(b.emb + (size_t)b.p_off[blockIdx.z] * a.n.D, a.n.P, a.n.D, a.n.KS, scale,
+                       const_cast<_Float16*>(a.eh), const_cast<_Float16*>(a.el));
+  else
+    prep_std_body<RAW>(b.protos + (size_t)b.m_off[blockIdx.z] * a.n.D, a.n.M, a.n.D, a.n.KS, scale,
+                       const_cast<_Float16*>(a.ph), const_cast<_Float16*>(a.pl));
+}
+__global__ __launch_bounds__(256) void prep_T_batched(NllBatch b, int px) {
+  NllArgs a;
+  if (!batch_problem(b, blockIdx.z, a)) return;
+  if (px)
+    prep_T_body<false>(b.emb + (size_t)b.p_off[blockIdx.z] * a.n.D, a.n.P, a.n.D, a.n.DT,
+                       b.rowscale + b.p_off[blockIdx.z], a.gscale, 1.0f, const_cast<_Float16*>(a.eth),
+                       const_cast<_Float16*>(a.etl));
+  else
+    prep_T_body<false>(b.protos + (size_t)b.m_off[blockIdx.z] * a.n.D, a.n.M, a.n.D, a.n.DT, nullptr, nullptr,
+                       1.0f, const_cast<_Float16*>(a.pth), const_cast<_Float16*>(a.ptl));
+}
+__global__ __launch_bounds__(256) void nll_finalize_batched(NllBatch b) {
+  NllArgs a;
+  if (!batch_problem(b, blockIdx.z, a)) return;
+  nll_finalize_body(a.partial, (int)fwd2_chunks(a.n), a.n.P, a.n.PT * 32, (a.mode & SPML_NLL_PLAIN) ? 1 : 0, a.nll,
+                    a.stats);
+}
+__global__ __launch_bounds__(1024) void max_abs_pow2_batched(NllBatch b) {
+  NllArgs a;
+  if (!batch_problem(b, blockIdx.z, a)) return;
+  max_abs_pow2_body(a.d_nll, a.n.P, const_cast<float*>(a.gscale));
+}
+template <bool TAG>
+__global__ void coef_batched(NllBatch b) {
+  NllArgs a;
+  if (!batch_problem(b, blockIdx.z, a)) return;
+  coef_body<TAG>(a.stats, a.own, a.px_code, a.pr_code, a.n.M, a.n.P, a.n.PT * 32, a.own_base,
+                 const_cast<PixelCoef*>(a.coef));
+}
+__global__ void nll_dpr_from_fix_batched(NllBatch b) {
+  NllArgs a;
+  if (!batch_problem(b, blockIdx.z, a)) return;
+  nll_dpr_from_fix_body(a.d_protos64, a.n.M * a.n.D, a.gscale, a.d_protos);
+}
+
+struct NllBatchWs {
+  size_t eh, el, ph, pl, pth, ptl, eth, etl, gscale, rowscale, codes, pxcodes, coef, partial, dp64, total;
+};
+struct NllBatchTotals {
+  int64_t P, M, PT, MT, part;
+};
+bool batch_totals(int n_problems, const int64_t* p_off, const int64_t* m_off, int D, NllBatchTotals& t) {
+  t = NllBatchTotals{0, 0, 0, 0, 0};
+  if (n_problems < 0 || D <= 0 || (n_problems > 0 && (!p_off || !m_off))) return false;
+  if (n_problems == 0) return true;
+  if (p_off[0] != 0 || m_off[0] != 0) return false;
+  for (int i = 0; i < n_problems; ++i) {
+    const int64_t P = p_off[i + 1] - p_off[i], M = m_off[i + 1] - m_off[i];
+    if (P < 0 || M < 0 || (P > 0 && M <= 0)) return false;
+    if (P > (int64_t)1 << 30 || M > (int64_t)1 << 30) return false;
+    const NllDims n = nll_dims(P, M, D);
+    t.PT += n.PT;
+    t.MT += n.MT;
+    t.part += fwd2_chunks(n) * n.PT * 32;
+  }
+  t.P = p_off[n_problems];
+  t.M = m_off[n_problems];
+  return true;
+}
+NllBatchWs nll_batch_ws(const NllBatchTotals& t, int n_problems, int D, int KS, int DT) {
+  NllBatchWs w{};
+  size_t o = 0;
+  const size_t e_std = (size_t)t.PT * KS * 1024, p_std = (size_t)t.MT * KS * 1024;
+  const size_t e_t = (size_t)t.PT * DT * 2048, p_t = (size_t)t.MT * DT * 2048;
+  w.eh = o; o = align_up(o + e_std, 256);
+  w.el = o; o = align_up(o + e_std, 256);
+  w.ph = o; o = align_up(o + p_std, 256);
+  w.pl = o; o = align_up(o + p_std, 256);
+  w.pth = o; o = align_up(o + p_t, 256);
+  w.ptl = o; o = align_up(o + p_t, 256);
+  w.eth = o; o = align_up(o + e_t, 256);
+  w.etl = o; o = align_up(o + e_t, 256);
+  w.gscale = o; o = align_up(o + (size_t)n_problems * 4 + 16, 256);
+  w.rowscale = o; o = align_up(o + (size_t)t.P * 4, 256);
+  w.codes = o; o = align_up(o + (size_t)t.MT * 32 * 8, 256);
+  w.pxcodes = o; o = align_up(o + (size_t)t.PT * 32 * 8, 256);
+  w.coef = o; o = align_up(o + (size_t)t.PT * 32 * 16, 256);
+  w.partial = o; o = align_up(o + (size_t)t.part * 16, 256);
+  w.dp64 = 0;
+  if (deterministic_mode()) { w.dp64 = o; o = align_up(o + (size_t)t.M * D * 8, 256); }
+  w.total = o;
+  return w;
+}
+
+bool batched_supported(int D, int mode) {
+  if (D <= 0 || mode < 0 || mode > (SPML_NLL_TAGSET | SPML_NLL_PLAIN | SPML_NLL_CODE32)) return false;
+  if (!(mode & SPML_NLL_CODE32) || ks_bucket((D + 15) / 16) != 5) return false;
+  const char* env2 = getenv("SPML_NLL_FWD2");
+  return !(env2 && env2[0] == '0');
+}
+
+int nll_batched(bool backward, const float* emb, const int64_t* own, const int64_t* px_code, const int64_t* p_off,
+                const float* protos, const int64_t* pr_code, const int64_t* m_off, int n_problems, int D, float kappa,
+                int mode, float* nll, float* stats, const float* d_nll, float* d_emb, float* d_protos, void* ws,
+                size_t ws_bytes, hipStream_t s) {
+  if (n_problems < 0 || D <= 0) return SPML_ERR_INVALID_ARG;
+  if (mode < 0 || mode > (SPML_NLL_TAGSET | SPML_NLL_PLAIN | SPML_NLL_CODE32)) return SPML_ERR_INVALID_ARG;
+  NllBatchTotals t;
+  if (!batch_totals(n_problems, p_off, m_off, D, t)) return SPML_ERR_INVALID_ARG;
+  if (!batched_supported(D, mode)) return SPML_ERR_UNSUPPORTED;
+  if (n_problems == 0 || t.P == 0) return SPML_OK;
+  if (!emb || !own || !px_code || !protos || !pr_code || !stats) return SPML_ERR_INVALID_ARG;
+  if (backward ? (!d_nll || !d_emb || !d_protos) : !nll) return SPML_ERR_INVALID_ARG;
+  constexpr int KS = 5, DT = 3;
+  const NllBatchWs w = nll_batch_ws(t, n_problems, D, KS, DT);
+  if (!ws || ws_bytes < w.total) return SPML_ERR_WORKSPACE;
+  unsigned char* base = static_cast<unsigned char*>(ws);
+  const bool tag = (mode & SPML_NLL_TAGSET) != 0;
+
+  NllBatch b{};
+  NllArgs& a = b.a;
+  a.n = nll_dims(0, 0, D);
+  a.n.KS = KS; a.n.DT = DT;
+  a.eh = reinterpret_cast<_Float16*>(base + w.eh); a.el = reinterpret_cast<_Float16*>(base + w.el);
+  a.ph = reinterpret_cast<_Float16*>(base + w.ph); a.pl = reinterpret_cast<_Float16*>(base + w.pl);
+  a.pth = reinterpret_cast<_Float16*>(base + w.pth); a.ptl = reinterpret_cast<_Float16*>(base + w.ptl);
+  a.eth = reinterpret_cast<_Float16*>(base + w.eth); a.etl = reinterpret_cast<_Float16*>(base + w.etl);
+  a.own = own; a.px_code = px_code; a.pr_code = pr_code;
+  a.pr_code_pad = reinterpret_cast<int64_t*>(base + w.codes);
+  a.px_code_pad = reinterpret_cast<int64_t*>(base + w.pxcodes);
+  a.coef = reinterpret_cast<PixelCoef*>(base + w.coef);
+  a.kappa = kappa;
+  a.kappa_log2e = kappa * 1.4426950408889634f;
+  a.mode = mode; a.nll = nll; a.stats = stats; a.d_nll = d_nll; a.d_emb = d_emb; a.d_protos = d_protos;
+  a.gscale = reinterpret_cast<float*>(base + w.gscale);
+  a.partial = reinterpret_cast<float*>(base + w.partial);
+  a.d_protos64 = backward && w.dp64 ? reinterpret_cast<long long*>(base + w.dp64) : nullptr;
+  a.depth = 2;
+  if (const char* e_ = getenv("SPML_NLL_DEPTH_BWD")) { const int v_ = atoi(e_); if (v_ >= 2 && v_ <= 3) a.depth = v_; }
+  a.dt0 = 0; a.dt_all = DT;
+  b.emb = emb; b.protos = protos;
+  b.rowscale = reinterpret_cast<float*>(base + w.rowscale);
+  if (a.d_protos64 &&
+      hipMemsetAsync(base + w.dp64, 0, (size_t)t.M * D * 8, s) != hipSuccess) return SPML_ERR_LAUNCH;
+
+  constexpr int LDS_F = kFwd2TilesPerChunk * 128 + 2 * 2 * 2 * KS * 1024;
+  constexpr int SLOT_DE = (2 * KS + 1 + 4 * DT) * 1024, SLOT_DP = (2 * KS + 2 + 4 * DT) * 1024;
+  int64_t pt_run = 0, mt_run = 0, part_run = 0;
+  for (int g0 = 0; g0 < n_problems; g0 += kNllBatchMax) {
+    const int cnt = std::min(kNllBatchMax, n_problems - g0);
+    b.count = cnt; b.first = g0;
+    int64_t max_p = 0, max_m = 0, max_chunks = 1, max_dpc = 1;
+    for (int i = 0; i <= cnt; ++i) {
+      b.p_off[i] = p_off[g0 + i]; b.m_off[i] = m_off[g0 + i];
+      b.pt_off[i] = pt_run; b.mt_off[i] = mt_run; b.part_off[i] = part_run;
+      if (i == cnt) break;
+      const int64_t P = p_off[g0 + i + 1] - p_off[g0 + i], M = m_off[g0 + i + 1] - m_off[g0 + i];
+      const NllDims n = nll_dims(P, M, D);
+      pt_run += n.PT; mt_run += n.MT; part_run += fwd2_chunks(n) * n.PT * 32;
+      if (P <= 0) continue;
+      max_p = std::max(max_p, P); max_m = std::max(max_m, M);
+      max_chunks = std::max(max_chunks, fwd2_chunks(n));
+      max_dpc = std::max(max_dpc, dp_chunks((n.MT + 3) / 4, n.PT));
+    }
+    if (max_p == 0) continue;
+    const unsigned z = (unsigned)cnt;
+    const int64_t PT = (max_p + 31) / 32, MT = (max_m + 31) / 32;
+    const auto blocks = [](int64_t n, int64_t per) { return (unsigned)((n + per - 1) / per); };
+    hipLaunchKernelGGL(pad_codes_batched, dim3(blocks(MT * 32, 256), 1, z), dim3(256), 0, s, b, 0);
+    if (!backward) {
+      hipLaunchKernelGGL(prep_std_batched<true>, dim3(blocks(PT * KS, 4), 1, z), dim3(256), 0, s, b, 1, 8.0f);
+      hipLaunchKernelGGL(prep_std_batched<true>, dim3(blocks(MT * KS, 4), 1, z), dim3(256), 0, s, b, 0,
+                         a.kappa_log2e * 0.125f);
+      const dim3 grid(blocks(PT, 8), (unsigned)max_chunks, z);
+      if (tag) {
+        (void)hipFuncSetAttribute(reinterpret_cast<const void*>(&nll_fwd2_batched<KS, 2, true>),
+                                  hipFuncAttributeMaxDynamicSharedMemorySize, LDS_F);
+        hipLaunchKernelGGL((nll_fwd2_batched<KS, 2, true>), grid, dim3(256), LDS_F, s, b);
+      } else {
+        (void)hipFuncSetAttribute(reinterpret_cast<const void*>(&nll_fwd2_batched<KS, 2, false>),
+                                  hipFuncAttributeMaxDynamicSharedMemorySize, LDS_F);
+        hipLaunchKernelGGL((nll_fwd2_batched<KS, 2, false>), grid, dim3(256), LDS_F, s, b);
+      }
+      hipLaunchKernelGGL(nll_finalize_batched, dim3(blocks(max_p, 256), 1, z), dim3(256), 0, s, b);
+      continue;
+    }
+    hipLaunchKernelGGL((prep_std_batched<false>), dim3(blocks(PT * KS, 4), 1, z), dim3(256), 0, s, b, 1, 1.0f);
+    hipLaunchKernelGGL((prep_std_batched<false>), dim3(blocks(MT * KS, 4), 1, z), dim3(256), 0, s, b, 0, a.kappa_log2e);
+    hipLaunchKernelGGL(max_abs_pow2_batched, dim3(1, 1, z), dim3(1024), 0, s, b);
+    {
+      const int64_t lo = p_off[g0], np = p_off[g0 + cnt] - lo;
+      hipLaunchKernelGGL(rowscale_kernel, dim3(blocks(np, 256)), dim3(256), 0, s, d_nll + lo, kappa, np,
+                         b.rowscale + lo);
+    }
+    hipLaunchKernelGGL(prep_T_batched, dim3(blocks(MT * DT * 2, 4), 1, z), dim3(256), 0, s, b, 0);
+    hipLaunchKernelGGL(prep_T_batched, dim3(blocks(PT * DT * 2, 4), 1, z), dim3(256), 0, s, b, 1);
+    hipLaunchKernelGGL(pad_codes_batched, dim3(blocks(PT * 32, 256), 1, z), dim3(256), 0, s, b, 1);
+    if (tag) hipLaunchKernelGGL(coef_batched<true>, dim3(blocks(PT * 32, 256), 1, z), dim3(256), 0, s, b);
+    else hipLaunchKernelGGL(coef_batched<false>, dim3(blocks(PT * 32, 256), 1, z), dim3(256), 0, s, b);
+    const dim3 grid_de(blocks(PT, 4), 1, z), grid_dp(blocks(MT, 4), (unsigned)max_dpc, z);
+    if (tag) {
+      (void)hipFuncSetAttribute(reinterpret_cast<const void*>(&nll_bwd_de_batched<KS, DT, true>),
+                                hipFuncAttributeMaxDynamicSharedMemorySize, a.depth * SLOT_DE);
+      (void)hipFuncSetAttribute(reinterpret_cast<const void*>(&nll_bwd_dp_batched<KS, DT, true>),
+                                hipFuncAttributeMaxDynamicSharedMemorySize, a.depth * SLOT_DP);
+      hipLaunchKernelGGL((nll_bwd_de_batched<KS, DT, true>), grid_de, dim3(256), a.depth * SLOT_DE, s, b);
+      hipLaunchKernelGGL((nll_bwd_dp_batched<KS, DT, true>), grid_dp, dim3(256), a.depth * SLOT_DP, s, b);
+    } else {
+      (void)hipFuncSetAttribute(reinterpret_cast<const void*>(&nll_bwd_de_batched<KS, DT, false>),
+                                hipFuncAttributeMaxDynamicSharedMemorySize, a.depth * SLOT_DE);
+      (void)hipFuncSetAttribute(reinterpret_cast<const void*>(&nll_bwd_dp_batched<KS, DT, false>),
+                                hipFuncAttributeMaxDynamicSharedMemorySize, a.depth * SLOT_DP);
+      hipLaunchKernelGGL((nll_bwd_de_batched<KS, DT, false>), grid_de, dim3(256), a.depth * SLOT_DE, s, b);
+      hipLaunchKernelGGL((nll_bwd_dp_batched<KS, DT, false>), grid_dp, dim3(256), a.depth * SLOT_DP, s, b);
+    }
+    if (a.d_protos64)
+      hipLaunchKernelGGL(nll_dpr_from_fix_batched, dim3(blocks(max_m * D, 256), 1, z), dim3(256), 0, s, b);
+  }
+  return launch_status();
 }
 
 }
@@ -1309,10 +1655,7 @@
   const int64_t mg = m_grad < 0 || m_grad > M ? M : m_grad;
   a.mt_grad = (mg + 31) / 32;
   const int64_t mgroups = (a.mt_grad + 3) / 4;
-  int64_t chunks = mgroups > 0 ? (2048 + mgroups - 1) / mgroups : 1;
-  if (chunks > (n.PT + 7) / 8) chunks = (n.PT + 7) / 8;
-  if (chunks < 1) chunks = 1;
-  if (chunks > 65535) chunks = 65535;
+  const int64_t chunks = dp_chunks(mgroups, n.PT);
   a.chunks = (int)chunks;
   a.spt0 = 0;
   a.spt1 = n.PT;
@@ -1457,3 +1800,29 @@
                     const_cast<float*>(stats), d_nll, d_emb, d_protos, m_grad, ws, ws_bytes,
                     (hipStream_t)stream);
 }
+
+extern "C" int spml_segsort_nll_batched_supported(int D, int mode) { return batched_supported(D, mode) ? 1 : 0; }
+
+extern "C" size_t spml_segsort_nll_batched_workspace_bytes(int n_problems, const int64_t* p_off,
+                                                           const int64_t* m_off, int D) {
+  NllBatchTotals t;
+  if (!batch_totals(n_problems, p_off, m_off, D, t) || ks_bucket((D + 15) / 16) != 5) return 0;
+  return nll_batch_ws(t, n_problems, D, 5, 3).total;
+}
+
+extern "C" int spml_segsort_nll_batched_fwd_f32(const float* emb, const int64_t* own, const int64_t* px_code,
+                                                const int64_t* p_off, const float* protos, const int64_t* pr_code,
+                                                const int64_t* m_off, int n_problems, int D, float kappa, int mode,
+                                                float* nll, float* stats, void* ws, size_t ws_bytes, void* stream) {
+  return nll_batched(false, emb, own, px_code, p_off, protos, pr_code, m_off, n_problems, D, kappa, mode, nll, stats,
+                     nullptr, nullptr, nullptr, ws, ws_bytes, (hipStream_t)stream);
+}
+
+extern "C" int spml_segsort_nll_batched_bwd_f32(const float* emb, const int64_t* own, const int64_t* px_code,
+                                                const int64_t* p_off, const float* protos, const int64_t* pr_code,
+                                                const int64_t* m_off, int n_problems, int D, float kappa, int mode,
+                                                const float* stats, const float* d_nll, float* d_emb, float* d_protos,
+                                                void* ws, size_t ws_bytes, void* stream) {
+  return nll_batched(true, emb, own, px_code, p_off, protos, pr_code, m_off, n_problems, D, kappa, mode, nullptr,
+                     const_cast<float*>(stats), d_nll, d_emb, d_protos, ws, ws_bytes, (hipStream_t)stream);
+}
diff --git a/spml_amd/csrc/nll_common.hpp b/spml_amd/csrc/nll_common.hpp
--- a/spml_amd/csrc/nll_common.hpp
+++ b/spml_amd/csrc/nll_common.hpp
@@ -75,6 +75,7 @@
   float* partial;
   int skip_de;
   float* partial_de;
+  int64_t own_base;
 };
 
 __device__ __forceinline__ void dpr_add(const NllArgs& a, size_t idx, float v, float inv_gscale) {
diff --git a/spml_amd/models/predictions/segsort.py b/spml_amd/models/predictions/segsort.py
--- a/spml_amd/models/predictions/segsort.py
+++ b/spml_amd/models/predictions/segsort.py
@@ -127,7 +127,7 @@
       uniq, pair = segsort_common._unique_inverse((img_of_px * (clu.max() + 1) + clu) * off + ins,
                                                   with_uniq=False, padded=True)
       bounds = torch.arange(1, n_img + 1, device=uniq.device) * stride
-      sim = (sizes, off, uniq, pair, torch.searchsorted(uniq, bounds) - 1)
+      sim = (sizes, off, uniq, pair, torch.searchsorted(uniq, bounds) - 1, img_of_px)
     last = None
 
     if self.sem_ann_loss is not None or self.sem_occ_loss is not None:
@@ -170,7 +170,7 @@
       acc = parallel.sharded_retrieval_accuracy(segsort_eval.top_k_ranking, protos, p_sem, 5)
 
     if sim is not None:
-      sizes, off, uniq, pair, last_dev = sim
+      sizes, off, uniq, pair, last_dev, img_of_px = sim
       emb = datas[self.img_sim_embedding_key]
       ins = datas['cluster_instance_label']
       if last is None:
@@ -178,40 +178,50 @@
       last = [int(v) for v in last]
       pair_lab = uniq[:last[-1] + 1] % off
       terms, lo, first = [], 0, 0
-      pr_all = e_all = None
+      pr_all = e_all = nll_all = None
       if os.environ.get('SPML_IMG_SIM_BATCHED_PROTOS') != '0' and sum(sizes) == int(emb.shape[0]):
         counts = [end + 1 - (last[i - 1] + 1 if i else 0) for i, end in enumerate(last)]
-        pr_all = torch.split(segsort_common.calculate_prototypes_from_labels(emb, pair, last[-1] + 1), counts)
-        e_all = torch.split(emb, sizes)
-      streams = _side_streams(emb.device, int(os.environ.get('SPML_IMG_SIM_STREAMS', '4'))) if emb.is_cuda else []
-      cur = torch.cuda.current_stream(emb.device) if streams else None
-      for st in streams:
-        st.wait_stream(cur)
-      for i, (n_px, end) in enumerate(zip(sizes, last)):
-        lab, c_abs, first_i = ins[lo:lo + n_px], pair[lo:lo + n_px], first
-        e = e_all[i] if e_all is not None else emb[lo:lo + n_px]
-        p_lab = pair_lab[first:end + 1]
-        lo, first = lo + n_px, end + 1
-        if streams:
-          side = streams[i % len(streams)]
-          if os.environ.get('SPML_IMG_SIM_RECORD_STREAM') != '0':
-            for t_ in (e, lab, c_abs, p_lab) + ((pr_all[i],) if pr_all is not None else ()):
-              t_.record_stream(side)
-          with torch.cuda.stream(side):
-            c = c_abs - first_i
-            pr_img = pr_all[i] if pr_all is not None else \
-                segsort_common.calculate_prototypes_from_labels(e, c, p_lab.shape[0])
-            term = self.img_sim_loss(e, lab, c, pr_img, p_lab, codes32=True)
-            term.record_stream(cur)
-          terms.append(term)
-          continue
-        c = c_abs - first_i
-        pr_img = pr_all[i] if pr_all is not None else \
-            segsort_common.calculate_prototypes_from_labels(e, c, p_lab.shape[0])
-        terms.append(self.img_sim_loss(e, lab, c, pr_img, p_lab, codes32=True))
-      for st in streams:
-        cur.wait_stream(st)
-      img_sim = sum(terms) / len(terms) * self.img_sim_loss_weight
+        protos_all = segsort_common.calculate_prototypes_from_labels(emb, pair, last[-1] + 1)
+        nll_all = self.img_sim_loss.batched_nll(emb, ins, pair, sizes, protos_all, pair_lab, counts) \
+            if (emb.is_cuda and os.environ.get('SPML_IMG_SIM_BATCHED') != '0' and
+                'SPML_IMG_SIM_STREAMS' not in os.environ) else None
+        if nll_all is None:
+          pr_all = torch.split(protos_all, counts)
+          e_all = torch.split(emb, sizes)
+      if nll_all is not None:
+        n_px = torch.zeros(len(sizes), dtype=torch.float32, device=emb.device)
+        n_px.index_add_(0, img_of_px, torch.ones_like(nll_all))
+        img_sim = (nll_all / n_px[img_of_px]).sum() / len(sizes) * self.img_sim_loss_weight
+      else:
+        streams = _side_streams(emb.device, int(os.environ.get('SPML_IMG_SIM_STREAMS', '4'))) if emb.is_cuda else []
+        cur = torch.cuda.current_stream(emb.device) if streams else None
+        for st in streams:
+          st.wait_stream(cur)
+        for i, (n_px, end) in enumerate(zip(sizes, last)):
+          lab, c_abs, first_i = ins[lo:lo + n_px], pair[lo:lo + n_px], first
+          e = e_all[i] if e_all is not None else emb[lo:lo + n_px]
+          p_lab = pair_lab[first:end + 1]
+          lo, first = lo + n_px, end + 1
+          if streams:
+            side = streams[i % len(streams)]
+            if os.environ.get('SPML_IMG_SIM_RECORD_STREAM') != '0':
+              for t_ in (e, lab, c_abs, p_lab) + ((pr_all[i],) if pr_all is not None else ()):
+                t_.record_stream(side)
+            with torch.cuda.stream(side):
+              c = c_abs - first_i
+              pr_img = pr_all[i] if pr_all is not None else \
+                  segsort_common.calculate_prototypes_from_labels(e, c, p_lab.shape[0])
+              term = self.img_sim_loss(e, lab, c, pr_img, p_lab, codes32=True)
+              term.record_stream(cur)
+            terms.append(term)
+            continue
+          c = c_abs - first_i
+          pr_img = pr_all[i] if pr_all is not None else \
+              segsort_common.calculate_prototypes_from_labels(e, c, p_lab.shape[0])
+          terms.append(self.img_sim_loss(e, lab, c, pr_img, p_lab, codes32=True))
+        for st in streams:
+          cur.wait_stream(st)
+        img_sim = sum(terms) / len(terms) * self.img_sim_loss_weight
 
     return sem_ann, sem_occ, img_sim, acc
 
diff --git a/spml_amd/ops.py b/spml_amd/ops.py
--- a/spml_amd/ops.py
+++ b/spml_amd/ops.py
@@ -107,6 +107,44 @@
     return emb.new_zeros((0,))
   m_grad = -1 if proto_grad_rows is None else int(proto_grad_rows)
   return _SegSortNLL.apply(emb, own, px_code, protos, pr_code, float(kappa), int(mode), m_grad)
+
+
+class _SegSortNLLBatched(torch.autograd.Function):
+
+  @staticmethod
+  def forward(ctx, emb, own_abs, px_code, protos, pr_code, p_sizes, m_sizes, kappa, mode):
+    emb, protos = _f32c(emb), _f32c(protos)
+    own_abs, px_code, pr_code = _i64c(own_abs), _i64c(px_code), _i64c(pr_code)
+    nll, stats = _ffi.segsort_nll_batched_fwd(emb, own_abs, px_code, p_sizes, protos, pr_code, m_sizes, kappa, mode)
+    ctx.save_for_backward(emb, own_abs, px_code, protos, pr_code, stats)
+    ctx.p_sizes, ctx.m_sizes, ctx.kappa, ctx.mode = p_sizes, m_sizes, kappa, mode
+    return nll
+
+  @staticmethod
+  def backward(ctx, d_nll):
+    emb, own_abs, px_code, protos, pr_code, stats = ctx.saved_tensors
+    d_emb, d_protos = _ffi.segsort_nll_batched_bwd(emb, own_abs, px_code, ctx.p_sizes, protos, pr_code, ctx.m_sizes,
+                                                   ctx.kappa, ctx.mode, stats, _f32c(d_nll))
+    return d_emb, None, None, d_protos, None, None, None, None, None
+
+
+def segsort_nll_batched_supported(d, mode):
+  return _ffi.segsort_nll_batched_supported(d, mode)
+
+
+def segsort_nll_batched(emb, own_abs, px_code, p_sizes, protos, pr_code, m_sizes, kappa, mode=NLL_LABEL):
+  p_sizes, m_sizes = [int(v) for v in p_sizes], [int(v) for v in m_sizes]
+  if emb.shape[0] == 0:
+    return emb.new_zeros((0,))
+  if segsort_nll_batched_supported(emb.shape[1], mode):
+    return _SegSortNLLBatched.apply(emb, own_abs, px_code, protos, pr_code, tuple(p_sizes), tuple(m_sizes),
+                                    float(kappa), int(mode))
+  out, lo, first = [], 0, 0
+  for n_px, n_pr in zip(p_sizes, m_sizes):
+    out.append(segsort_nll(emb[lo:lo + n_px], own_abs[lo:lo + n_px] - first, px_code[lo:lo + n_px],
+                           protos[first:first + n_pr], pr_code[first:first + n_pr], kappa, mode))
+    lo, first = lo + n_px, first + n_pr
+  return torch.cat(out)
 
 
 def kmeans(x, seg_offsets, max_seg_len, k, labels_init, iterations, want_centroids=False):
diff --git a/spml_amd/utils/segsort/loss.py b/spml_amd/utils/segsort/loss.py
--- a/spml_amd/utils/segsort/loss.py
+++ b/spml_amd/utils/segsort/loss.py
@@ -92,10 +92,24 @@
       return torch.sum(nll)
     return nll
 
+  _batched_mode = None
+
+  def batched_nll(self, embeddings, semantic_labels, instance_labels, pixel_counts, prototypes,
+                  prototype_semantic_labels, prototype_counts):
+    base = type(self)._batched_mode
+    if base is None or self.reduction != 'mean' or embeddings.dim() != 2 or semantic_labels.dim() != 1:
+      return None
+    mode = _mode(self.group_mode, base, True)
+    if not ops.segsort_nll_batched_supported(embeddings.shape[-1], mode):
+      return None
+    return ops.segsort_nll_batched(embeddings, instance_labels, semantic_labels, pixel_counts, prototypes,
+                                   prototype_semantic_labels, prototype_counts, self.concentration, mode)
+
 
 class SegSortLoss(_NcaLoss):
   _kernel = staticmethod(_calculate_log_likelihood)
   _name = 'SegSortLoss'
+  _batched_mode = ops.NLL_LABEL
 
 
 class SetSegSortLoss(_NcaLoss):
```
